# leo-stan/torch-points3d

Hardware: AMD Instinct MI355X
Metric: point-clouds/sec fwd+bwd PointNet++SSG B=32 N=16384 (higher is better)
Workload: dtype f32; 1 GPU; PointNet++ SSG (unet_3_ss) train step fwd+bwd+Adam, B=32 per GPU, N=16384, FEAT=3, 10 classes, pos~U[-1,1]^3 (BASELINE configs[1]); launch=hip-graph replay; geometry of step i+1 on a 2nd stream during step i, global_batch=32, points=16384, parallelism=dp1, whole clouds per rank, one flat gradient all-reduce (RCCL) per step

## Files before the change

include/tp3d_hip.h:

```cpp
#ifndef TP3D_HIP_H
#define TP3D_HIP_H

#include <stddef.h>
#include <stdint.h>

#ifdef __cplusplus
extern "C" {
#endif

#define TP3D_OK 0
#define TP3D_E_BADARG (-1)
#define TP3D_E_LAUNCH (-2)
#define TP3D_E_UNSORTED (-3)
#define TP3D_E_TOOBIG (-4)

#define TP3D_ABI_VERSION 39

int tp3d_abi_version(void);
const char *tp3d_strerror(int code);
int tp3d_last_hip_error(void);

#define TP3D_FPS_MAX_REG_POINTS 32768
int tp3d_fps_f32(const float *xyz, int B, int N, int npoint, float *scratch, int64_t *out_idx, void *stream);

int tp3d_fps_ragged_f32(const float *pos, const int64_t *seg_in, const int64_t *seg_out, int64_t M, int clouds,
                        int max_cloud_points, float *scratch, int64_t *out_idx, void *stream);

int tp3d_ball_query_dense_f32(const float *x, const float *y, int B, int N, int np, float radius, int nsample,
                              int sort, int64_t *idx, float *dist2, void *workspace, size_t workspace_bytes,
                              void *stream);
size_t tp3d_ball_query_workspace_bytes(int num_clouds, int64_t rows, int max_cloud_points);

int tp3d_ball_query_partial_dense_f32(const float *x, const float *y, const int64_t *batch_x,
                                      const int64_t *batch_y, int64_t M, int64_t Nq, float radius, int nsample,
                                      int sort, int64_t *idx, float *dist2, const int64_t *seg_x, int num_clouds,
                                      int max_cloud_points, void *workspace, size_t workspace_bytes, int reuse_grid,
                                      void *stream);

int tp3d_three_nn_f32(const float *unknown, const float *known, int B, int n, int m, float *dist, int64_t *idx,
                      void *stream);

int tp3d_three_interpolate_fwd_f32(const float *features, const int64_t *idx, const float *weight, int B, int C,
                                   int m, int n, float *out, void *stream);
int tp3d_three_interpolate_bwd_f32(const float *grad_out, const int64_t *idx, const float *weight, int B, int C,
                                   int m, int n, float *grad_features, void *workspace, size_t workspace_bytes,
                                   void *stream);

size_t tp3d_scatter_workspace_bytes(int B, int L, int nbins, int with_weights);

int tp3d_group_fwd_f32(const float *features, const int64_t *idx, int B, int C, int N, int np, int ns, float *out,
                       void *stream);
int tp3d_group_bwd_f32(const float *grad_out, const int64_t *idx, int B, int C, int N, int np, int ns,
                       float *grad_features, void *workspace, size_t workspace_bytes, void *stream);


int tp3d_group_concat_fwd_f32(const float *pos, const float *new_pos, const float *x_cl, const int64_t *idx, int B,
                              int N, int np, int ns, int C, int ld, float radius, int normalize, float *out,
                              void *stream);

int tp3d_rows_scatter_bwd_f32(const float *grad_rows, const int64_t *idx, const float *weight, int B, int L, int div,
                              int nbins, int ld, int col0, int C, float *grad_x_cl, void *workspace,
                              size_t workspace_bytes, void *stream);
int tp3d_rows_scatter_invert(const int64_t *idx, const float *weight, int B, int L, int div, int nbins, void *workspace,
                             size_t workspace_bytes, void *stream);
int tp3d_rows_scatter_apply_f32(const float *grad_rows, int B, int L, int div, int nbins, int ld, int col0, int C,
                                int with_weights, float *grad_x_cl, void *table, size_t table_bytes, void *stream);

size_t tp3d_bn_workspace_floats(int64_t M, int C);
int tp3d_bn_stats_f32(const float *Y, int64_t M, int C, float eps, float momentum, const float *gamma,
                      const float *beta, float *running_mean, float *running_var, int64_t *num_batches_tracked,
                      int training, float *mean, float *invstd, float *scale, float *shift, float *workspace,
                      void *stream);

int tp3d_bn_act_f32(const float *Y, const float *mean, const float *scale, const float *shift, float slope, int64_t M,
                    int C, float *out, void *stream);
int tp3d_bn_act_maxpool_f32(const float *Y, const float *mean, const float *scale, const float *shift, float slope,
                            int64_t G, int ns, int C, float *out, int *argmax, void *stream);

int tp3d_bn_act_bwd_f32(const float *dA, const int *argmax, const float *Y, const float *scale, const float *shift,
                        const float *mean, const float *invstd, float slope, int64_t M, int ns, int C, int training,
                        float *dbeta, float *dgamma, float *dY, float *workspace, void *stream);
int tp3d_bn_bwd_reduce_f32(const float *dA, const int *argmax, const float *Y, const float *scale, const float *shift,
                           const float *mean, const float *invstd, float slope, int64_t M, int ns, int C, int training,
                           float *dbeta, float *dgamma, float *c1, float *c2, float *workspace, int reverse,
                           void *stream);

int tp3d_interp_concat_fwd_f32(const float *feat_cl, const int64_t *idx, const float *weight, const float *skip_cl,
                               int B, int m, int n, int C1, int C2, int ld, float *out, void *stream);

size_t tp3d_gemm_rows_stat_floats(int64_t M, int N);
int tp3d_gemm_rows_stat_chunks(int64_t M, int N);
size_t tp3d_gemm_rows_workspace_floats(int64_t M, int N, int K);
int tp3d_gemm_rows_f32(const float *A, const float *Bt, int64_t M, int N, int K, float *C, float *stat_partial,
                       float *workspace, void *stream);
int tp3d_gemm_rows_epi_f32(const float *A, const float *Bt, int64_t M, int N, int K, const float *mean, const float *scale,
                           const float *beta, float slope, float *C, float *workspace, void *stream);
int tp3d_gemm_rows_sp_chunks(int64_t M, int N, int K, int with_act_out);
int tp3d_gemm_rows_bnact_sp_f32(const float *Y, const float *mean, const float *scale, const float *beta, float slope,
                                const float *Bt, int64_t M, int N, int K, float *C, float *stat_partial, float *act_out,
                                int reverse, void *stream);
int tp3d_gemm_rows_x3_chunks(int64_t M, int N, int K, int with_act_out);
int tp3d_gemm_rows_bnact_x3_f32(const float *Y, const float *mean, const float *scale, const float *beta, float slope,
                                const float *Bt, int64_t M, int N, int K, float *C, float *stat_partial, float *act_out,
                                int reverse, void *stream);

int tp3d_gemm_rows_bnbwd_sp_serves(int64_t M, int N, int K);
int tp3d_gemm_rows_bnbwd_sp_f32(const float *Y, const float *dA, const float *mean, const float *scale, const float *beta,
                                const float *c1, const float *c2, float slope, const float *Bt, int64_t M, int N, int K,
                                float *C, int ldc, int pad_lo, int pad_hi, float *dY_out, const int *argmax, int ns,
                                int reverse, void *stream);
int tp3d_bn_finalize_f32(float *partial, int chunks, int64_t M, int C, float eps, float momentum, const float *gamma,
                         const float *beta, float *running_mean, float *running_var, int64_t *num_batches_tracked,
                         float *mean, float *invstd, float *scale, float *shift, void *stream);

int tp3d_gemm_tn_bn_narrow_serves(int64_t M, int N, int K);
int tp3d_gemm_rows_narrow_chunks(int64_t M);
int tp3d_gemm_rows_narrow_f32(const float *A, const float *W, int64_t M, int N, int K, float *Y, float *stat_partial,
                              int reverse, void *stream);
size_t tp3d_gemm_tn_bn_narrow_workspace_floats(int64_t M, int N, int K);
int tp3d_gemm_tn_bn_narrow_f32(const float *Y, const float *dA, const float *mean_n, const float *scale_n,
                               const float *beta_n, const float *c1_n, const float *c2_n, float slope_n, const float *A,
                               int64_t M, int N, int K, float *out, float *workspace, int reverse, void *stream);

size_t tp3d_gemm_tn_workspace_floats(int64_t M, int N, int K);
int tp3d_gemm_tn_f32(const float *dY, const float *A, int64_t M, int N, int K, float *out, float *workspace,
                     void *stream);

int tp3d_gemm_tn_x3_serves(int64_t M, int N, int K);
size_t tp3d_gemm_tn_x3_workspace_floats(int64_t M, int N, int K);
int tp3d_gemm_tn_x3_f32(const float *dY, const float *A, int64_t M, int N, int K, int terms, float *out, float *workspace,
                        int reverse, void *stream);
int tp3d_gemm_tn_x3_act_f32(const float *dY, const float *Yp, const float *mean_k, const float *scale_k, const float *beta_k,
                            float slope_k, int64_t M, int N, int K, int terms, float *out, float *workspace, int reverse, void *stream);
int tp3d_gemm_tn_x3_red_chunks(int64_t M, int N, int K);
int tp3d_gemm_tn_x3_act_red_f32(const float *dY, const float *Yp, const float *mean_k, const float *scale_k,
                                const float *beta_k, const float *invstd_k, float slope_k, const float *dA_k, int training,
                                int64_t M, int N, int K, int terms, float *out, float *workspace, float *red_out,
                                float *red_workspace, int reverse, void *stream);

int tp3d_kpconv_weighted_f32(const float *query, const float *support, const int64_t *neighbors,
                             const float *features, const float *k_points, int64_t Nq, int64_t M, int Mn, int Cin,
                             int KP, float extent, int influence, int closest, float *weighted, void *stream);

size_t tp3d_kpconv_bwd_workspace_bytes(int64_t M, int64_t slots);
size_t tp3d_kpconv_grad_workspace_bytes(int64_t M, int64_t slots, int Cin);
int tp3d_kpconv_bwd_features_f32(const float *query, const float *support, const int64_t *neighbors,
                                 const float *k_points, const float *d_weighted, int64_t Nq, int64_t M, int Mn,
                                 int Cin, int KP, float extent, int influence, int closest, float *d_features,
                                 void *inverse, size_t inverse_bytes, int inverse_ready, void *workspace,
                                 size_t workspace_bytes, void *stream);

int tp3d_kpconv_deform_weighted_f32(const float *query, const float *support, const int64_t *neighbors,
                                    const float *features, const float *k_points, const float *offsets,
                                    const float *modulations, int64_t Nq, int64_t M, int Mn, int Cin, int KP, float extent,
                                    int influence, float *weighted, float *kp_min_d2, int32_t *kp_argmin, void *stream);

int tp3d_kpconv_deform_bwd_f32(const float *query, const float *support, const int64_t *neighbors, const float *features,
                               const float *k_points, const float *offsets, const float *modulations,
                               const float *d_weighted, const float *d_kp_min_d2, const int32_t *kp_argmin, int64_t Nq,
                               int64_t M, int Mn, int Cin, int KP, float extent, int influence, float *d_features,
                               float *d_offsets, float *d_modulations, void *inverse, size_t inverse_bytes,
                               int inverse_ready, void *workspace, size_t workspace_bytes, void *stream);

int tp3d_relation_rows_f32(const float *pos, const float *new_pos, const int64_t *idx, int B, int N, int np, int ns,
                           int ld, float *out, void *stream);

int tp3d_idw_weights_f32(const float *dist, int64_t rows, float *weight, void *stream);

int tp3d_voxel_bounds_f32(const float *pos, const int64_t *batch, int64_t N, float size, int32_t *bounds, void *stream);
size_t tp3d_voxel_workspace_bytes(int64_t N);
int tp3d_voxel_cluster_f32(const float *pos, const int64_t *batch, int64_t N, float size, const int32_t *bounds_host,
                           int64_t *cluster, int64_t *order, int64_t *cluster_start, int64_t *last, int64_t *meta,
                           void *workspace, size_t workspace_bytes, void *stream);
int tp3d_cluster_mean_f32(const float *x, const int64_t *order, const int64_t *cluster_start, int64_t K, int C,
                          float *out, void *stream);
int tp3d_cluster_majority_i64(const int64_t *labels, const int64_t *order, const int64_t *cluster_start, int64_t K,
                              int64_t min_label, int64_t num_classes, int64_t *out, void *stream);

size_t tp3d_knn_workspace_bytes(int num_clouds, int64_t rows, int max_cloud_points);
int tp3d_knn_partial_dense_f32(const float *x, const float *y, const int64_t *batch_y, const int64_t *seg_x,
                               int num_clouds, int max_cloud_points, int64_t M, int64_t Nq, int k, float cell,
                               int64_t *idx, float *dist2, void *workspace, size_t workspace_bytes, void *stream);
int tp3d_knn_dense_f32(const float *x, const float *y, int B, int N, int np, int k, float cell, int64_t *idx,
                       float *dist2, void *workspace, size_t workspace_bytes, void *stream);

int tp3d_knn_interpolate_fwd_f32(const float *x, const int64_t *idx, const float *dist2, const float *skip, int64_t Nq,
                                 int k, int C, int C2, int ld, float *out, float *wnorm, void *stream);

int tp3d_randla_relpos_f32(const float *q_pos, const float *s_pos, const int64_t *nbr, int64_t Nq, int k, int64_t M,
                           float *out, void *stream);

int tp3d_attn_pool_fwd_f32(const float *g, const float *f, const int64_t *nbr, int64_t Nq, int k, int C, int ldg, int ldf,
                           float *out, void *stream);
int tp3d_attn_pool_bwd_f32(const float *g, const float *f, const float *dout, const int64_t *nbr, int64_t Nq, int k, int C,
                           int ldg, int ldf, float *dg, float *df, void *stream);

int tp3d_gemm_skinny_f32(const float *A, const float *W, int64_t M, int N, int K, int lda, float *Y, void *stream);
int tp3d_gemm_skinny_bnact_f32(const float *A, const float *W, int64_t M, int N, int K, int lda, const float *mean,
                               const float *scale, const float *beta, float slope, float *out, void *stream);

int tp3d_nbr_maxpool_fwd_f32(const float *x, const int64_t *neighbors, int64_t Nq, int64_t M, int Mn, int C, float *out,
                             int32_t *argmax, void *stream);
int tp3d_nbr_maxpool_bwd_f32(const float *grad_out, const int32_t *argmax, const int64_t *neighbors, int64_t Nq,
                             int64_t M, int Mn, int C, float *d_x, void *inverse, size_t inverse_bytes,
                             int inverse_ready, void *stream);

int tp3d_pospool_padding_i64(const int64_t *neighbors, int64_t slots, int64_t M, int64_t *padding, void *stream);
int tp3d_pospool_fwd_f32(const float *query, const float *support, const int64_t *neighbors, const float *features,
                         const int64_t *padding, const float *dim_mat, int64_t Nq, int64_t M, int Mn, int C, float radius,
                         int embedding, int reduction, float *out, float *counts, void *stream);
int tp3d_pospool_bwd_f32(const float *query, const float *support, const int64_t *neighbors, const float *grad_out,
                         const float *counts, const float *dim_mat, int64_t Nq, int64_t M, int Mn, int C, float radius,
                         int embedding, int reduction, float *d_features, void *inverse, size_t inverse_bytes,
                         int inverse_ready, void *stream);


int tp3d_table_edge_start_i64(const int64_t *table, int64_t Nq, int max_num, int64_t *edge_start, void *stream);
int tp3d_table_edge_col_i64(const int64_t *table, const int64_t *edge_start, int64_t Nq, int max_num, int64_t E,
                            int64_t *col, void *stream);

int tp3d_pointconv_rows_f32(const float *x, const float *pos_s, const float *pos_q, const int64_t *edge_start,
                            const int64_t *col, int64_t Nq, int64_t M, int64_t E, int C, int ld, float *out,
                            void *stream);

int tp3d_segment_max_fwd_f32(const float *rows, const int64_t *seg, int64_t S, int64_t E, int C, int ld, float *out,
                             int64_t *argmax, void *stream);
int tp3d_segment_max_bwd_f32(const float *dout, const int64_t *argmax, const int64_t *seg, int64_t S, int64_t E, int C,
                             int ld, float *d_rows, void *stream);


int tp3d_rsconv_relation_rows_f32(const float *pos_s, const float *pos_q, const int64_t *edge_start, const int64_t *col,
                                  int64_t Nq, int64_t M, int64_t E, int ld, float *out, void *stream);

int tp3d_rsconv_msgmax_fwd_f32(const float *w, int ldw, const float *x, int ldx, const int64_t *col,
                               const int64_t *edge_start, int64_t Nq, int64_t M, int64_t E, int C, float *out,
                               int64_t *arg, void *stream);
int tp3d_rsconv_msgmax_bwd_f32(const float *dout, const int64_t *arg, const float *w, int ldw, const float *x, int ldx,
                               const int64_t *col, const int64_t *edge_start, int64_t Nq, int64_t M, int64_t E, int C,
                               float *d_w, float *g_x, void *stream);

int tp3d_gemm_tn_plan(int64_t M, int N, int K, int64_t *plan);
int tp3d_gemm_tn_x3_plan(int64_t M, int N, int K, int64_t *plan);
int tp3d_gemm_rows_plan(int64_t M, int N, int K, int64_t *plan);
int tp3d_bn_plan(int64_t M, int C, int pooled_ns, int64_t *plan);
int tp3d_scatter_plan(int B, int L, int nbins, int with_weights, int64_t *plan);

#ifdef __cplusplus
}
#endif
#endif
```

torch_points3d_amd/_lib.py:

```python
import collections
import ctypes
import os

import torch

from . import build as _build

_p = ctypes.c_void_p
_i = ctypes.c_int
_l = ctypes.c_int64
_f = ctypes.c_float

SIGNATURES = {
    "tp3d_fps_f32": [_p, _i, _i, _i, _p, _p, _p],
    "tp3d_ball_query_dense_f32": [_p, _p, _i, _i, _i, _f, _i, _i, _p, _p, _p, ctypes.c_size_t, _p],
    "tp3d_ball_query_partial_dense_f32": [_p, _p, _p, _p, _l, _l, _f, _i, _i, _p, _p, _p, _i, _i, _p, ctypes.c_size_t,
                                          _i, _p],
    "tp3d_three_nn_f32": [_p, _p, _i, _i, _i, _p, _p, _p],
    "tp3d_three_interpolate_fwd_f32": [_p, _p, _p, _i, _i, _i, _i, _p, _p],
    "tp3d_three_interpolate_bwd_f32": [_p, _p, _p, _i, _i, _i, _i, _p, _p, ctypes.c_size_t, _p],
    "tp3d_group_fwd_f32": [_p, _p, _i, _i, _i, _i, _i, _p, _p],
    "tp3d_group_bwd_f32": [_p, _p, _i, _i, _i, _i, _i, _p, _p, ctypes.c_size_t, _p],
    "tp3d_group_concat_fwd_f32": [_p, _p, _p, _p, _i, _i, _i, _i, _i, _i, _f, _i, _p, _p],
    "tp3d_rows_scatter_bwd_f32": [_p, _p, _p, _i, _i, _i, _i, _i, _i, _i, _p, _p, ctypes.c_size_t, _p],
    "tp3d_rows_scatter_invert": [_p, _p, _i, _i, _i, _i, _p, ctypes.c_size_t, _p],
    "tp3d_rows_scatter_apply_f32": [_p, _i, _i, _i, _i, _i, _i, _i, _i, _p, _p, ctypes.c_size_t, _p],
    "tp3d_bn_stats_f32": [_p, _l, _i, _f, _f, _p, _p, _p, _p, _p, _i, _p, _p, _p, _p, _p, _p],
    "tp3d_bn_act_f32": [_p, _p, _p, _p, _f, _l, _i, _p, _p],
    "tp3d_bn_act_maxpool_f32": [_p, _p, _p, _p, _f, _l, _i, _i, _p, _p, _p],
    "tp3d_bn_act_bwd_f32": [_p, _p, _p, _p, _p, _p, _p, _f, _l, _i, _i, _i, _p, _p, _p, _p, _p],
    "tp3d_interp_concat_fwd_f32": [_p, _p, _p, _p, _i, _i, _i, _i, _i, _i, _p, _p],
    "tp3d_idw_weights_f32": [_p, _l, _p, _p],
    "tp3d_gemm_tn_f32": [_p, _p, _l, _i, _i, _p, _p, _p],
    "tp3d_gemm_tn_x3_f32": [_p, _p, _l, _i, _i, _i, _p, _p, _i, _p],
    "tp3d_gemm_tn_x3_act_f32": [_p, _p, _p, _p, _p, _f, _l, _i, _i, _i, _p, _p, _i, _p],
    "tp3d_gemm_tn_x3_act_red_f32": [_p, _p, _p, _p, _p, _p, _f, _p, _i, _l, _i, _i, _i, _p, _p, _p, _p, _i, _p],
    "tp3d_gemm_rows_narrow_f32": [_p, _p, _l, _i, _i, _p, _p, _i, _p],
    "tp3d_gemm_tn_bn_narrow_f32": [_p, _p, _p, _p, _p, _p, _p, _f, _p, _l, _i, _i, _p, _p, _i, _p],
    "tp3d_bn_bwd_reduce_f32": [_p, _p, _p, _p, _p, _p, _p, _f, _l, _i, _i, _i, _p, _p, _p, _p, _p, _i, _p],
    "tp3d_gemm_rows_f32": [_p, _p, _l, _i, _i, _p, _p, _p, _p],
    "tp3d_gemm_rows_epi_f32": [_p, _p, _l, _i, _i, _p, _p, _p, _f, _p, _p, _p],
    "tp3d_gemm_rows_bnact_sp_f32": [_p, _p, _p, _p, _f, _p, _l, _i, _i, _p, _p, _p, _i, _p],
    "tp3d_gemm_rows_bnact_x3_f32": [_p, _p, _p, _p, _f, _p, _l, _i, _i, _p, _p, _p, _i, _p],
    "tp3d_gemm_rows_bnbwd_sp_f32": [_p, _p, _p, _p, _p, _p, _p, _f, _p, _l, _i, _i, _p, _i, _i, _i, _p, _p, _i, _i, _p],
    "tp3d_bn_finalize_f32": [_p, _i, _l, _i, _f, _f, _p, _p, _p, _p, _p, _p, _p, _p, _p, _p],
    "tp3d_kpconv_bwd_features_f32": [_p, _p, _p, _p, _p, _l, _l, _i, _i, _i, _f, _i, _i, _p, _p, ctypes.c_size_t, _i, _p,
                                     ctypes.c_size_t, _p],
    "tp3d_knn_partial_dense_f32": [_p, _p, _p, _p, _i, _i, _l, _l, _i, _f, _p, _p, _p, ctypes.c_size_t, _p],
    "tp3d_knn_dense_f32": [_p, _p, _i, _i, _i, _i, _f, _p, _p, _p, ctypes.c_size_t, _p],
    "tp3d_knn_interpolate_fwd_f32": [_p, _p, _p, _p, _l, _i, _i, _i, _i, _p, _p, _p],
    "tp3d_nbr_maxpool_fwd_f32": [_p, _p, _l, _l, _i, _i, _p, _p, _p],
    "tp3d_nbr_maxpool_bwd_f32": [_p, _p, _p, _l, _l, _i, _i, _p, _p, ctypes.c_size_t, _i, _p],
    "tp3d_pospool_padding_i64": [_p, _l, _l, _p, _p],
    "tp3d_pospool_fwd_f32": [_p, _p, _p, _p, _p, _p, _l, _l, _i, _i, _f, _i, _i, _p, _p, _p],
    "tp3d_pospool_bwd_f32": [_p, _p, _p, _p, _p, _p, _l, _l, _i, _i, _f, _i, _i, _p, _p, ctypes.c_size_t, _i, _p],
    "tp3d_voxel_bounds_f32": [_p, _p, _l, _f, _p, _p],
    "tp3d_voxel_cluster_f32": [_p, _p, _l, _f, _p, _p, _p, _p, _p, _p, _p, ctypes.c_size_t, _p],
    "tp3d_cluster_mean_f32": [_p, _p, _p, _l, _i, _p, _p],
    "tp3d_cluster_majority_i64": [_p, _p, _p, _l, _l, _l, _p, _p],
    "tp3d_kpconv_weighted_f32": [_p, _p, _p, _p, _p, _l, _l, _i, _i, _i, _f, _i, _i, _p, _p],
    "tp3d_kpconv_deform_weighted_f32": [_p, _p, _p, _p, _p, _p, _p, _l, _l, _i, _i, _i, _f, _i, _p, _p, _p, _p],
    "tp3d_kpconv_deform_bwd_f32": [_p, _p, _p, _p, _p, _p, _p, _p, _p, _p, _l, _l, _i, _i, _i, _f, _i, _p, _p, _p, _p,
                                   ctypes.c_size_t, _i, _p, ctypes.c_size_t, _p],
    "tp3d_gemm_skinny_f32": [_p, _p, _l, _i, _i, _i, _p, _p],
    "tp3d_gemm_skinny_bnact_f32": [_p, _p, _l, _i, _i, _i, _p, _p, _p, _f, _p, _p],
    "tp3d_randla_relpos_f32": [_p, _p, _p, _l, _i, _l, _p, _p],
    "tp3d_attn_pool_fwd_f32": [_p, _p, _p, _l, _i, _i, _i, _i, _p, _p],
    "tp3d_attn_pool_bwd_f32": [_p, _p, _p, _p, _l, _i, _i, _i, _i, _p, _p, _p],
    "tp3d_relation_rows_f32": [_p, _p, _p, _i, _i, _i, _i, _i, _p, _p],
    "tp3d_fps_ragged_f32": [_p, _p, _p, _l, _i, _i, _p, _p, _p],
    "tp3d_table_edge_start_i64": [_p, _l, _i, _p, _p],
    "tp3d_table_edge_col_i64": [_p, _p, _l, _i, _l, _p, _p],
    "tp3d_pointconv_rows_f32": [_p, _p, _p, _p, _p, _l, _l, _l, _i, _i, _p, _p],
    "tp3d_segment_max_fwd_f32": [_p, _p, _l, _l, _i, _i, _p, _p, _p],
    "tp3d_segment_max_bwd_f32": [_p, _p, _p, _l, _l, _i, _i, _p, _p],
    "tp3d_rsconv_relation_rows_f32": [_p, _p, _p, _p, _l, _l, _l, _i, _p, _p],
    "tp3d_rsconv_msgmax_fwd_f32": [_p, _i, _p, _i, _p, _p, _l, _l, _l, _i, _p, _p, _p],
    "tp3d_rsconv_msgmax_bwd_f32": [_p, _p, _p, _i, _p, _i, _p, _p, _l, _l, _l, _i, _p, _p, _p],
    "tp3d_gemm_tn_plan": [_l, _i, _i, _p],
    "tp3d_gemm_tn_x3_plan": [_l, _i, _i, _p],
    "tp3d_gemm_rows_plan": [_l, _i, _i, _p],
    "tp3d_bn_plan": [_l, _i, _i, _p],
    "tp3d_scatter_plan": [_i, _i, _i, _i, _p],
}
_z = ctypes.c_size_t
MISC = {
    "tp3d_abi_version": (_i, []),
    "tp3d_strerror": (ctypes.c_char_p, [_i]),
    "tp3d_last_hip_error": (_i, []),
    "tp3d_scatter_workspace_bytes": (_z, [_i, _i, _i, _i]),
    "tp3d_bn_workspace_floats": (_z, [_l, _i]),
    "tp3d_gemm_tn_workspace_floats": (_z, [_l, _i, _i]),
    "tp3d_gemm_tn_x3_workspace_floats": (_z, [_l, _i, _i]),
    "tp3d_gemm_tn_x3_serves": (_i, [_l, _i, _i]),
    "tp3d_gemm_tn_x3_red_chunks": (_i, [_l, _i, _i]),
    "tp3d_kpconv_bwd_workspace_bytes": (_z, [_l, _l]),
    "tp3d_gemm_rows_stat_floats": (_z, [_l, _i]),
    "tp3d_gemm_rows_stat_chunks": (_i, [_l, _i]),
    "tp3d_gemm_rows_narrow_chunks": (_i, [_l]),
    "tp3d_gemm_tn_bn_narrow_serves": (_i, [_l, _i, _i]),
    "tp3d_gemm_tn_bn_narrow_workspace_floats": (_z, [_l, _i, _i]),
    "tp3d_gemm_rows_bnbwd_sp_serves": (_i, [_l, _i, _i]),
    "tp3d_gemm_rows_x3_chunks": (_i, [_l, _i, _i, _i]),
    "tp3d_gemm_rows_sp_chunks": (_i, [_l, _i, _i, _i]),
    "tp3d_gemm_rows_workspace_floats": (_z, [_l, _i, _i]),
    "tp3d_kpconv_grad_workspace_bytes": (_z, [_l, _l, _i]),
    "tp3d_knn_workspace_bytes": (_z, [_i, _l, _i]),
    "tp3d_voxel_workspace_bytes": (_z, [_l]),
    "tp3d_ball_query_workspace_bytes": (_z, [_i, _l, _i]),
}
ABI_VERSION = 39

_handle = None


class Tp3dError(RuntimeError):
    pass


def library_path():
    return _build.LIB_PATH


def load():
    global _handle
    if _handle is not None:
        return _handle
    path = _build.LIB_PATH
    if not os.path.exists(path):
        _build.build_library()
    if not os.path.exists(path):
        raise Tp3dError("libtp3d_hip.so is missing at %s and could not be built" % path)
    h = ctypes.CDLL(path)
    for name, argtypes in SIGNATURES.items():
        fn = getattr(h, name)
        fn.argtypes = argtypes
        fn.restype = _i
    for name, (restype, argtypes) in MISC.items():
        fn = getattr(h, name)
        fn.restype = restype
        fn.argtypes = argtypes
    if h.tp3d_abi_version() != ABI_VERSION:
        raise Tp3dError("libtp3d_hip.so ABI %d != binding ABI %d" % (h.tp3d_abi_version(), ABI_VERSION))
    _handle = h
    return h


class KernelTimer(object):

    def __init__(self):
        self.records = []

    def summary(self):
        out = {}
        for tag, a, b in self.records:
            n, t = out.get(tag, (0, 0.0))
            out[tag] = (n + 1, t + a.elapsed_time(b))
        return out


_timer = None


def set_timer(timer):
    global _timer
    prev, _timer = _timer, timer
    return prev


_fn_cache = {}
_post_call_hook = None


def set_post_call_hook(hook):
    global _post_call_hook
    prev, _post_call_hook = _post_call_hook, hook
    return prev


def call(name, *args):
    fn = _fn_cache.get(name)
    if fn is None:
        fn = _fn_cache[name] = getattr(load(), name)
    if _timer is not None:
        a = torch.cuda.Event(enable_timing=True)
        b = torch.cuda.Event(enable_timing=True)
        torch.cuda.current_stream().synchronize()
        a.record()
        rc = fn(*args)
        b.record()
        _timer.records.append(((name, tuple(v for v in args if type(v) is int and v < (1 << 40))), a, b))
    else:
        rc = fn(*args)
    if rc != 0:
        h = load()
        raise Tp3dError("%s failed: %s (code %d, hipError %d)" % (
            name, h.tp3d_strerror(rc).decode(), rc, h.tp3d_last_hip_error()))
    if _post_call_hook is not None:
        _post_call_hook(name, args)


class on_device(object):

    __slots__ = ("idx", "prev")

    def __init__(self, dev):
        self.idx = dev.index if dev.index is not None else torch.cuda.current_device()
        self.prev = -1

    def __enter__(self):
        cur = torch.cuda.current_device()
        if cur != self.idx:
            self.prev = cur
            torch.cuda.set_device(self.idx)

    def __exit__(self, *exc):
        if self.prev >= 0:
            torch.cuda.set_device(self.prev)
        return False


_ws_cache = {}
_ws_retired = []


def workspace(tag, nbytes, device):
    key = (device.index, _raw_stream(device), tag)
    capturing = device.type == "cuda" and torch.cuda.is_current_stream_capturing()
    slot = _ws_cache.get(key)
    if slot is None or slot[0].numel() < nbytes:
        if slot is not None and slot[1]:
            _ws_retired.append(slot[0])
        slot = _ws_cache[key] = [torch.empty(max(int(nbytes), 256), dtype=torch.uint8, device=device), False]
    if capturing:
        slot[1] = True
    return slot[0]


def _raw_stream(device):
    idx = device.index if device.index is not None else torch.cuda.current_device()
    return torch._C._cuda_getCurrentRawStream(idx)


def scatter_workspace(B, L, nbins, with_weights, device):
    nbytes = load().tp3d_scatter_workspace_bytes(B, L, nbins, int(with_weights))
    return workspace("scatter", nbytes, device), nbytes


GRID_MIN_POINTS = 2048


def ball_query_workspace(num_clouds, rows, max_cloud_points, device):
    if max_cloud_points < GRID_MIN_POINTS:
        return None, 0
    nbytes = load().tp3d_ball_query_workspace_bytes(num_clouds, rows, max_cloud_points)
    if nbytes == 0:
        return None, 0
    return workspace("grid", nbytes, device), nbytes


_inverse_cache = collections.OrderedDict()
INVERSE_CACHE_ENTRIES = 48


def _evict_inverse():
    if len(_inverse_cache) < INVERSE_CACHE_ENTRIES:
        return
    for key in list(_inverse_cache):
        if len(_inverse_cache) < INVERSE_CACHE_ENTRIES:
            break
        if not _inverse_cache[key][5]:
            del _inverse_cache[key]


def neighbour_inverse(nbr, M, device):
    key = (nbr.data_ptr(), nbr._version, tuple(nbr.shape), int(M), device.index)
    hit = _inverse_cache.get(key)
    cur = _raw_stream(device)
    capturing = torch.cuda.is_current_stream_capturing()
    if hit is not None and hit[3] is not None:
        _inverse_cache.move_to_end(key)
        if capturing:
            hit[5] = True
        elif hit[4] != cur:
            torch.cuda.current_stream(device).wait_event(hit[3])
        return hit[1], hit[2], 1, None
    nbytes = load().tp3d_kpconv_bwd_workspace_bytes(int(M), nbr.numel())
    if capturing:
        return workspace("nbr_inverse", nbytes, device), nbytes, 0, None
    buf = torch.empty(max(int(nbytes), 256), dtype=torch.uint8, device=device)
    _evict_inverse()
    _inverse_cache[key] = [nbr, buf, nbytes, None, cur, False]
    return buf, nbytes, 0, key


def inverse_built(token, device):
    if token is None:
        return
    entry = _inverse_cache.get(token)
    if entry is not None:
        ev = torch.cuda.Event()
        ev.record(torch.cuda.current_stream(device))
        entry[3] = ev


def bn_workspace(M, C, device):
    n = load().tp3d_bn_workspace_floats(M, C)
    return workspace("bn", 4 * n, device)


def gemm_tn_workspace(M, N, K, device, x3=False):
    h = load()
    n = h.tp3d_gemm_tn_x3_workspace_floats(M, N, K) if x3 else h.tp3d_gemm_tn_workspace_floats(M, N, K)
    return workspace("gemm_tn", 4 * n, device)


def ptr(t):
    return None if t is None else t.data_ptr()


def stream_ptr(device):
    return _raw_stream(device)
```

torch_points3d_amd/csrc/gemm_tn.hip:

```cpp
#include <type_traits>

#include "tp3d_common.h"

namespace tp3d {

typedef float f32x16 __attribute__((ext_vector_type(16)));

constexpr int TN_BLOCK = 256;
constexpr int TN_BR_MAX = 64;

template <int WM, int WN, bool VECY, bool VECA, int GN = 2>
__global__ __launch_bounds__(TN_BLOCK) void gemm_tn_partial_kernel(const float *__restrict__ dY,
                                                                    const float *__restrict__ A, int64_t M, int N,
                                                                    int K, int64_t rows_per_split, int tiles_k,
                                                                    float *__restrict__ partial )
{
    constexpr int GK = 4 / GN;
    constexpr int TN = GN * WM * 32, TK = GK * WN * 32;
    constexpr int TN_BR = (WM * WN) % 3 == 0 ? 16 : 64 / (WM * WN);
    constexpr int LDN = TN + 4, LDK = TK + 4;
    __shared__ __attribute__((aligned(16))) float sY[TN_BR * LDN];
    __shared__ __attribute__((aligned(16))) float sA[TN_BR * LDK];

    const int tile = blockIdx.x;
    const int n0 = (tile / tiles_k) * TN, k0 = (tile % tiles_k) * TK;
    const int split = blockIdx.y;
    const int64_t r_begin = (int64_t)split * rows_per_split;
    const int64_t r_end = min(r_begin + rows_per_split, M);
    const int tid = threadIdx.x, lane = tid & 63, wave = tid >> 6;
    const int wr = wave / GK, wc = wave % GK;
    const int l31 = lane & 31, lh = lane >> 5;
    f32x16 acc[WM][WN];
#pragma unroll
    for (int i = 0; i < WM; ++i)
#pragma unroll
        for (int j = 0; j < WN; ++j)
#pragma unroll
            for (int e = 0; e < 16; ++e) acc[i][j][e] = 0.0f;


    auto load4 = [&](const float *base, int64_t r, int c, int ld, auto aligned_tag) __attribute__((always_inline)) -> float4 {
        constexpr bool aligned = decltype(aligned_tag)::value;
        float4 v = make_float4(0.f, 0.f, 0.f, 0.f);
        if (r < r_end) {
            const float *src = base + r * ld + c;
            if (aligned) {
                if (c < ld) v = *reinterpret_cast<const float4 *>(src);
            } else {
                if (c + 0 < ld) v.x = src[0];
                if (c + 1 < ld) v.y = src[1];
                if (c + 2 < ld) v.z = src[2];
                if (c + 3 < ld) v.w = src[3];
            }
        }
        return v;
    };

    constexpr int PY = TN_BR * (TN / 4) / TN_BLOCK, PA = TN_BR * (TK / 4) / TN_BLOCK;
    static_assert(PY >= 1 && PA >= 1 && PY * TN_BLOCK == TN_BR * (TN / 4) && PA * TN_BLOCK == TN_BR * (TK / 4),
                  "staged tile must be a whole number of float4 slots per thread");
    float4 ry[PY], ra[PA];
    auto fetch = [&](int64_t r0) __attribute__((always_inline)) {
#pragma unroll
        for (int i = 0; i < PY; ++i) {
            const int e = tid + i * TN_BLOCK;
            const int64_t r = r0 + e / (TN / 4);
            const int c = n0 + (e % (TN / 4)) * 4;
            ry[i] = load4(dY, r, c, N, std::integral_constant<bool, VECY>());
        }
#pragma unroll
        for (int i = 0; i < PA; ++i) {
            const int e = tid + i * TN_BLOCK;
            ra[i] = load4(A, r0 + e / (TK / 4), k0 + (e % (TK / 4)) * 4, K, std::integral_constant<bool, VECA>());
        }
    };
    if (r_begin < r_end) fetch(r_begin);
    for (int64_t r0 = r_begin; r0 < r_end; r0 += TN_BR) {
#pragma unroll
        for (int i = 0; i < PY; ++i) {
            const int e = tid + i * TN_BLOCK;
            *reinterpret_cast<float4 *>(&sY[(e / (TN / 4)) * LDN + (e % (TN / 4)) * 4]) = ry[i];
        }
#pragma unroll
        for (int i = 0; i < PA; ++i) {
            const int e = tid + i * TN_BLOCK;
            *reinterpret_cast<float4 *>(&sA[(e / (TK / 4)) * LDK + (e % (TK / 4)) * 4]) = ra[i];
        }
        __syncthreads();
        if (r0 + TN_BR < r_end) fetch(r0 + TN_BR);
#pragma unroll
        for (int rr = 0; rr < TN_BR; rr += 2) {
            float a[WM], b[WN];
#pragma unroll
            for (int i = 0; i < WM; ++i) a[i] = sY[(rr + lh) * LDN + (wr * WM + i) * 32 + l31];
#pragma unroll
            for (int j = 0; j < WN; ++j) b[j] = sA[(rr + lh) * LDK + (wc * WN + j) * 32 + l31];
#pragma unroll
            for (int i = 0; i < WM; ++i)
#pragma unroll
                for (int j = 0; j < WN; ++j) acc[i][j] = __builtin_amdgcn_mfma_f32_32x32x2f32(a[i], b[j], acc[i][j], 0, 0, 0);
        }
        __syncthreads();
    }

    float *out = partial + (size_t)split * N * K;
#pragma unroll
    for (int i = 0; i < WM; ++i)
#pragma unroll
        for (int j = 0; j < WN; ++j)
#pragma unroll
            for (int e = 0; e < 16; ++e) {
                const int n = n0 + (wr * WM + i) * 32 + (e & 3) + 8 * (e >> 2) + 4 * lh;
                const int k = k0 + (wc * WN + j) * 32 + l31;
                if (n < N && k < K) out[(size_t)n * K + k] = acc[i][j][e];
            }
}

constexpr int RD_E = 64, RD_S = 16;
__global__ __launch_bounds__(RD_E *RD_S) void gemm_tn_reduce_kernel(const float *__restrict__ partial, int S,
                                                                     int64_t NK, float *__restrict__ out)
{
    __shared__ float sm[RD_S][RD_E];
    const int tx = threadIdx.x % RD_E, ty = threadIdx.x / RD_E;
    const int64_t e = (int64_t)blockIdx.x * RD_E + tx;
    float acc = 0.0f;
    if (e < NK)
        for (int s = ty; s < S; s += RD_S) acc += partial[(size_t)s * NK + e];
    sm[ty][tx] = acc;
    __syncthreads();
    if (ty == 0 && e < NK) {
        float t = 0.0f;
#pragma unroll
        for (int k = 0; k < RD_S; ++k) t += sm[k][tx];
        out[e] = t;
    }
}

int tn_reduce_splits(const float *partial, int splits, int64_t NK, float *out, hipStream_t s)
{
    hipLaunchKernelGGL(gemm_tn_reduce_kernel, dim3((unsigned)((NK + RD_E - 1) / RD_E)), dim3(RD_E * RD_S), 0, s, partial, splits,
                       NK, out);
    return check_launch();
}

struct TnPlan {
    int wm, wn, gn, tn, tk, tiles_n, tiles_k, splits;
    int64_t rows_per_split;
};

static TnPlan plan_tn(int64_t M, int N, int K)
{
    TnPlan p;
    p.wm = N > 64 ? 2 : 1;
    if (K <= 64) p.wn = 1;
    else if (K <= 128) p.wn = 2;
    else if (K <= 192) p.wn = 3;
    else p.wn = ((K + 191) / 192) * 192 < ((K + 127) / 128) * 128 ? 3 : 2;
    p.gn = 2;
    if (N <= 32 && K >= 128) {
        p.gn = 1;
        p.wm = 1;
        p.wn = 1;
    }
    p.tn = 32 * p.gn * p.wm;
    p.tk = 32 * (4 / p.gn) * p.wn;
    p.tiles_n = (N + p.tn - 1) / p.tn;
    p.tiles_k = (K + p.tk - 1) / p.tk;
    const int tiles = p.tiles_n * p.tiles_k;
    int64_t want = (1024 + tiles - 1) / tiles;
    const int min_rows = 256;
    int64_t max_by_rows = (M + min_rows - 1) / min_rows;
    int64_t s = want < max_by_rows ? want : max_by_rows;
    if (s < 1) s = 1;
    if (s > 512) s = 512;
    p.rows_per_split = ((M + s - 1) / s + TN_BR_MAX - 1) / TN_BR_MAX * TN_BR_MAX;
    p.splits = (int)((M + p.rows_per_split - 1) / p.rows_per_split);
    return p;
}

static int launch_tn(const float *dY, const float *A, int64_t M, int N, int K, float *out, float *workspace, hipStream_t s)
{
    const TnPlan p = plan_tn(M, N, K);
    if (p.splits > 65535) return TP3D_E_TOOBIG;
    dim3 grid(p.tiles_n * p.tiles_k, p.splits);
    const bool vy = (N & 3) == 0, va = (K & 3) == 0;
#define TP3D_TN_LAUNCH(WM_, WN_, VY_, VA_)                                                                          \
    hipLaunchKernelGGL((gemm_tn_partial_kernel<WM_, WN_, VY_, VA_>), grid, dim3(TN_BLOCK), 0, s, dY, A, M, N, K,        \
                       p.rows_per_split, p.tiles_k, workspace)
#define TP3D_TN_ALIGN(WM_, WN_)                                                                                     \
    do {                                                                                                            \
        if (vy && va) TP3D_TN_LAUNCH(WM_, WN_, true, true);                                                         \
        else if (vy) TP3D_TN_LAUNCH(WM_, WN_, true, false);                                                         \
        else if (va) TP3D_TN_LAUNCH(WM_, WN_, false, true);                                                         \
        else TP3D_TN_LAUNCH(WM_, WN_, false, false);                                                                \
    } while (0)
    if (p.gn == 1) {
        if (vy && va) hipLaunchKernelGGL((gemm_tn_partial_kernel<1, 1, true, true, 1>), grid, dim3(TN_BLOCK), 0, s, dY, A, M, N, K,
                                         p.rows_per_split, p.tiles_k, workspace);
        else if (va) hipLaunchKernelGGL((gemm_tn_partial_kernel<1, 1, false, true, 1>), grid, dim3(TN_BLOCK), 0, s, dY, A, M, N, K,
                                        p.rows_per_split, p.tiles_k, workspace);
        else if (vy) hipLaunchKernelGGL((gemm_tn_partial_kernel<1, 1, true, false, 1>), grid, dim3(TN_BLOCK), 0, s, dY, A, M, N, K,
                                        p.rows_per_split, p.tiles_k, workspace);
        else hipLaunchKernelGGL((gemm_tn_partial_kernel<1, 1, false, false, 1>), grid, dim3(TN_BLOCK), 0, s, dY, A, M, N, K,
                                p.rows_per_split, p.tiles_k, workspace);
    } else if (p.wm == 2 && p.wn == 3) TP3D_TN_ALIGN(2, 3);
    else if (p.wn == 3) TP3D_TN_ALIGN(1, 3);
    else if (p.wm == 2 && p.wn == 2) TP3D_TN_ALIGN(2, 2);
    else if (p.wm == 2) TP3D_TN_ALIGN(2, 1);
    else if (p.wn == 2) TP3D_TN_ALIGN(1, 2);
    else TP3D_TN_ALIGN(1, 1);
#undef TP3D_TN_ALIGN
#undef TP3D_TN_LAUNCH
    if (int rc = check_launch()) return rc;
    return tn_reduce_splits(workspace, p.splits, (int64_t)N * K, out, s);
}

}

using namespace tp3d;

TP3D_EXPORT size_t tp3d_gemm_tn_workspace_floats(int64_t M, int N, int K)
{
    if (M <= 0 || N <= 0 || K <= 0) return 0;
    const TnPlan p = plan_tn(M, N, K);
    return (size_t)p.splits * (size_t)N * (size_t)K;
}

TP3D_EXPORT int tp3d_gemm_tn_plan(int64_t M, int N, int K, int64_t *plan)
{
    if (M <= 0 || N <= 0 || K <= 0 || !plan) return TP3D_E_BADARG;
    const TnPlan p = plan_tn(M, N, K);
    plan[0] = p.splits;
    plan[1] = p.rows_per_split;
    plan[2] = p.tn;
    plan[3] = p.tk;
    plan[4] = (int64_t)p.tiles_n * p.tiles_k;
    plan[5] = (p.wm * p.wn) % 3 == 0 ? 16 : 64 / (p.wm * p.wn);
    plan[6] = (int64_t)p.splits * N * K;
    plan[7] = (int64_t)(p.splits - 1) * p.rows_per_split;
    return TP3D_OK;
}

TP3D_EXPORT int tp3d_gemm_tn_f32(const float *dY, const float *A, int64_t M, int N, int K, float *out,
                                 float *workspace, void *stream)
{
    if (M < 0 || N <= 0 || K <= 0 || !out) return TP3D_E_BADARG;
    hipStream_t s = (hipStream_t)stream;
    if (M == 0) return zero_async(out, (size_t)N * K * sizeof(float), s);
    if (!dY || !A || !workspace) return TP3D_E_BADARG;
    return launch_tn(dY, A, M, N, K, out, workspace, s);
}
```

torch_points3d_amd/csrc/gemm_tn_x3.hip:

```cpp
#include "tp3d_common.h"
#include "x3_split.h"

namespace tp3d {

typedef float f32x16 __attribute__((ext_vector_type(16)));
typedef __bf16 bf16x8 __attribute__((ext_vector_type(8)));
typedef short s16x4 __attribute__((ext_vector_type(4)));
typedef short s16x8 __attribute__((ext_vector_type(8)));

constexpr int X3_BLOCK = 512;

__host__ __device__ constexpr int x3_pitch(int cols) { return cols % 64 == 0 ? cols + 32 : cols; }

__device__ __forceinline__ bf16x8 x3_frag(const unsigned short *plane, int pitch, int row0, int col0, int lane)
{
    const int grp = lane >> 4, q = (lane & 15) >> 2, p = lane & 3;
    const unsigned short *a = plane + (row0 + 8 * (grp >> 1) + q) * pitch + col0 + 16 * (grp & 1) + 4 * p;
    typedef s16x4 __attribute__((address_space(3))) *lds_ptr;
    const s16x4 lo = __builtin_amdgcn_ds_read_tr16_b64_v4i16((lds_ptr)(a));
    const s16x4 hi = __builtin_amdgcn_ds_read_tr16_b64_v4i16((lds_ptr)(a + 4 * pitch));
    const s16x8 both = {lo[0], lo[1], lo[2], lo[3], hi[0], hi[1], hi[2], hi[3]};
    return __builtin_bit_cast(bf16x8, both);
}

struct X3Prologue {
    const float *mean, *scale, *beta;
    float slope;
    int reverse;
    const float *dA, *invstd;
    float *red_partial;
};

template <int WM, int WN, bool STRIP, int BR, int TERMS, bool RED = false>
__global__ __launch_bounds__(X3_BLOCK) void gemm_tn_x3_kernel(const float *__restrict__ dY, const float *__restrict__ A,
                                                              int64_t M, int N, int K, int64_t rows_per_split,
                                                              int tiles_k, float *__restrict__ partial ,
                                                              X3Prologue pro)
{
    static_assert(!STRIP || WM == 2, "the strip is one block per wave of a 128-row tile");
    static_assert(!(RED && STRIP), "the reductions ride on the plain tiles (one tile column: every workgroup sees all K columns)");
    constexpr int TN = 64 * WM, TK = 64 * WN, TKS = TK + (STRIP ? 32 : 0);
    constexpr int PN = x3_pitch(TN), PK = x3_pitch(TKS);
    constexpr int PLANE_N = BR * PN, PLANE_K = BR * PK;
    constexpr int BUF = 3 * PLANE_N + 3 * PLANE_K;
    extern __shared__ __attribute__((aligned(16))) unsigned short smem[];
    __shared__ __attribute__((aligned(16))) float sK[RED ? 4 : 3][TKS];

    const int tid = threadIdx.x, lane = tid & 63, wave = tid >> 6;
    const int tile = blockIdx.x;
    const int n0 = (tile / tiles_k) * TN, k0 = (tile % tiles_k) * TK;
    const bool prologue = pro.mean != nullptr;
    if (prologue) {
        for (int c = tid; c < TKS; c += X3_BLOCK) {
            const bool in = k0 + c < K;
            sK[0][c] = in ? pro.mean[k0 + c] : 0.0f;
            sK[1][c] = in ? pro.scale[k0 + c] : 0.0f;
            sK[2][c] = in ? pro.beta[k0 + c] : 0.0f;
            if (RED) sK[3][c] = in ? pro.invstd[k0 + c] : 0.0f;
        }
        __syncthreads();
    }
    const int64_t r_end = M;
    const int64_t blocks = (M + BR - 1) / BR;
    const int S = gridDim.y;
    const int steps = (int)(((int64_t)blocks - blockIdx.y + S - 1) / S);
    (void)rows_per_split;

    if (__builtin_amdgcn_readfirstlane(tid) >= 256) {
        __builtin_amdgcn_s_setprio(3);
        const int lt = tid - 256;
        constexpr int SY = BR * (TN / 4) / 256, SA = BR * (TK / 4) / 256, SS = STRIP ? BR * 8 / 256 : 0;
        static_assert(SY >= 1 && SA >= 1 && SY * 256 == BR * (TN / 4) && SA * 256 == BR * (TK / 4), "whole float4 slots per thread");
        static_assert(!STRIP || SS * 256 == BR * 8, "whole strip slots per thread");
        float4 ry0[SY], ra0[SA], rs0[STRIP ? SS : 1], ry1[SY], ra1[SA], rs1[STRIP ? SS : 1], ry2[SY], ra2[SA], rs2[STRIP ? SS : 1];
        float4 rd0[RED ? SA : 1], rd1[RED ? SA : 1], rd2[RED ? SA : 1];
        float red1[4] = {0.f, 0.f, 0.f, 0.f}, red2[4] = {0.f, 0.f, 0.f, 0.f};
        const int red_tiles = (int)gridDim.x;
        auto mine = [&](int t) __attribute__((always_inline)) -> bool { return RED && (t % red_tiles) == tile; };
        const float4 zero = make_float4(0.f, 0.f, 0.f, 0.f);
        const bool cols_full = n0 + TN <= N && k0 + TK <= K;
        unsigned oy[SY], oa[SA], os[STRIP ? SS : 1];
#pragma unroll
        for (int i = 0; i < SY; ++i) oy[i] = (unsigned)((((lt + i * 256) / (TN / 4)) * N + n0 + ((lt + i * 256) % (TN / 4)) * 4) * 4);
#pragma unroll
        for (int i = 0; i < SA; ++i) oa[i] = (unsigned)((((lt + i * 256) / (TK / 4)) * K + k0 + ((lt + i * 256) % (TK / 4)) * 4) * 4);
        if (STRIP) {
#pragma unroll
            for (int i = 0; i < SS; ++i) os[i] = (unsigned)((((lt + i * 256) / 8) * K + k0 + TK + ((lt + i * 256) % 8) * 4) * 4);
        }
        auto fetch = [&](int t, float4 *ry, float4 *ra, float4 *rs, float4 *rd) __attribute__((always_inline)) {
            const int64_t r0 = ((int64_t)(pro.reverse ? steps - 1 - t : t) * S + blockIdx.y) * BR;
            const char *by_ = reinterpret_cast<const char *>(dY) + r0 * N * 4;
            const char *ba_ = reinterpret_cast<const char *>(A) + r0 * K * 4;
            if (r0 + BR <= M && cols_full) {
#pragma unroll
                for (int i = 0; i < SY; ++i) ry[i] = *reinterpret_cast<const float4 *>(by_ + oy[i]);
#pragma unroll
                for (int i = 0; i < SA; ++i) ra[i] = *reinterpret_cast<const float4 *>(ba_ + oa[i]);
                if (mine(t)) {
                    const char *bd_ = reinterpret_cast<const char *>(pro.dA) + r0 * K * 4;
#pragma unroll
                    for (int i = 0; i < SA; ++i) rd[i] = *reinterpret_cast<const float4 *>(bd_ + oa[i]);
                }
                if (STRIP) {
#pragma unroll
                    for (int i = 0; i < SS; ++i) {
                        rs[i] = zero;
                        if (k0 + TK + ((lt + i * 256) % 8) * 4 < K) rs[i] = *reinterpret_cast<const float4 *>(ba_ + os[i]);
                    }
                }
                return;
            }
#pragma unroll
            for (int i = 0; i < SY; ++i) {
                const int e = lt + i * 256;
                const int64_t r = r0 + e / (TN / 4);
                const int c = n0 + (e % (TN / 4)) * 4;
                ry[i] = zero;
                if (r < r_end && c < N) ry[i] = *reinterpret_cast<const float4 *>(dY + r * N + c);
            }
#pragma unroll
            for (int i = 0; i < SA; ++i) {
                const int e = lt + i * 256;
                const int64_t r = r0 + e / (TK / 4);
                const int c = k0 + (e % (TK / 4)) * 4;
                ra[i] = zero;
                if (r < r_end && c < K) ra[i] = *reinterpret_cast<const float4 *>(A + r * K + c);
                if (mine(t)) {
                    rd[i] = zero;
                    if (r < r_end && c < K) rd[i] = *reinterpret_cast<const float4 *>(pro.dA + r * K + c);
                }
            }
            if (STRIP) {
#pragma unroll
                for (int i = 0; i < SS; ++i) {
                    const int e = lt + i * 256;
                    const int64_t r = r0 + e / 8;
                    const int c = k0 + TK + (e % 8) * 4;
                    rs[i] = zero;
                    if (r < r_end && c < K) rs[i] = *reinterpret_cast<const float4 *>(A + r * K + c);
                }
            }
        };
        auto put = [&](unsigned short *plane0, int plane_len, int pitch, int row, int col, float4 v) __attribute__((always_inline)) {
            uint2 h, m, l;
            x3_split(v, h, m, l);
            unsigned short *dst = plane0 + row * pitch + col;
            *reinterpret_cast<uint2 *>(dst) = h;
            *reinterpret_cast<uint2 *>(dst + plane_len) = m;
            *reinterpret_cast<uint2 *>(dst + 2 * plane_len) = l;
        };
        auto act4 = [&](float4 v, int col) __attribute__((always_inline)) -> float4 {
            const float4 mu = *reinterpret_cast<const float4 *>(&sK[0][col]);
            const float4 sc = *reinterpret_cast<const float4 *>(&sK[1][col]);
            const float4 be = *reinterpret_cast<const float4 *>(&sK[2][col]);
            const float z0 = (v.x - mu.x) * sc.x + be.x, z1 = (v.y - mu.y) * sc.y + be.y;
            const float z2 = (v.z - mu.z) * sc.z + be.z, z3 = (v.w - mu.w) * sc.w + be.w;
            return make_float4(z0 > 0.0f ? z0 : z0 * pro.slope, z1 > 0.0f ? z1 : z1 * pro.slope, z2 > 0.0f ? z2 : z2 * pro.slope,
                               z3 > 0.0f ? z3 : z3 * pro.slope);
        };
        auto store = [&](int t, const float4 *ry, const float4 *ra, const float4 *rs, const float4 *rd) __attribute__((always_inline)) {
            unsigned short *by = smem + (t & 1) * BUF, *ba = by + 3 * PLANE_N;
            if (mine(t)) {
                const int col = ((lt % (TK / 4))) * 4;
                const float4 mu = *reinterpret_cast<const float4 *>(&sK[0][col]), sc = *reinterpret_cast<const float4 *>(&sK[1][col]);
                const float4 be = *reinterpret_cast<const float4 *>(&sK[2][col]), is = *reinterpret_cast<const float4 *>(&sK[3][col]);
#pragma unroll
                for (int i = 0; i < SA; ++i) {
                    const float y[4] = {ra[i].x, ra[i].y, ra[i].z, ra[i].w}, d[4] = {rd[i].x, rd[i].y, rd[i].z, rd[i].w};
                    const float m4[4] = {mu.x, mu.y, mu.z, mu.w}, s4[4] = {sc.x, sc.y, sc.z, sc.w};
                    const float b4[4] = {be.x, be.y, be.z, be.w}, i4[4] = {is.x, is.y, is.z, is.w};
#pragma unroll
                    for (int c = 0; c < 4; ++c) {
                        const float yc = y[c] - m4[c];
                        const float dz = d[c] * (yc * s4[c] + b4[c] > 0.0f ? 1.0f : pro.slope);
                        red1[c] += dz;
                        red2[c] += dz * (yc * i4[c]);
                    }
                }
            }
#pragma unroll
            for (int i = 0; i < SY; ++i) {
                const int e = lt + i * 256;
                put(by, PLANE_N, PN, e / (TN / 4), (e % (TN / 4)) * 4, ry[i]);
            }
#pragma unroll
            for (int i = 0; i < SA; ++i) {
                const int e = lt + i * 256;
                const int col = (e % (TK / 4)) * 4;
                put(ba, PLANE_K, PK, e / (TK / 4), col, prologue ? act4(ra[i], col) : ra[i]);
            }
            if (STRIP) {
#pragma unroll
                for (int i = 0; i < SS; ++i) {
                    const int e = lt + i * 256;
                    const int col = TK + (e % 8) * 4;
                    put(ba, PLANE_K, PK, e / 8, col, prologue ? act4(rs[i], col) : rs[i]);
                }
            }
        };
        if (steps > 0) fetch(0, ry0, ra0, rs0, rd0);
        if (steps > 1) fetch(1, ry1, ra1, rs1, rd1);
        if (steps > 2) fetch(2, ry2, ra2, rs2, rd2);
        auto iter = [&](int t, float4 *ry, float4 *ra, float4 *rs, float4 *rd) __attribute__((always_inline)) {
            store(t, ry, ra, rs, rd);
            if (t + 3 < steps) fetch(t + 3, ry, ra, rs, rd);
            __syncthreads();
        };
        for (int t = 0; t < steps; t += 3) {
            iter(t, ry0, ra0, rs0, rd0);
            if (t + 1 < steps) iter(t + 1, ry1, ra1, rs1, rd1);
            if (t + 2 < steps) iter(t + 2, ry2, ra2, rs2, rd2);
        }
        if (RED) {
            float *scr = reinterpret_cast<float *>(smem + (steps & 1) * BUF);
#pragma unroll
            for (int c = 0; c < 4; ++c) {
                scr[lt * 8 + c] = red1[c];
                scr[lt * 8 + 4 + c] = red2[c];
            }
            __syncthreads();
            constexpr int CG = TK / 4, PER = 256 / CG;
            if (lt < CG) {
                float a1[4] = {0.f, 0.f, 0.f, 0.f}, a2[4] = {0.f, 0.f, 0.f, 0.f};
                for (int x = 0; x < PER; ++x)
#pragma unroll
                    for (int c = 0; c < 4; ++c) {
                        a1[c] += scr[(lt + x * CG) * 8 + c];
                        a2[c] += scr[(lt + x * CG) * 8 + 4 + c];
                    }
                float *pr = pro.red_partial + ((size_t)blockIdx.y * gridDim.x + blockIdx.x) * 2 * K;
#pragma unroll
                for (int c = 0; c < 4; ++c) {
                    const int k = k0 + lt * 4 + c;
                    if (k < K) {
                        pr[k] = a1[c];
                        pr[K + k] = a2[c];
                    }
                }
            }
        }
        return;
    }

    const int wr = wave >> 1, wc = wave & 1;
    const int l31 = lane & 31, lh = lane >> 5;
    f32x16 acc[WM][WN], low[WM][WN], accs, lows;
#pragma unroll
    for (int i = 0; i < WM; ++i)
#pragma unroll
        for (int j = 0; j < WN; ++j)
#pragma unroll
            for (int e = 0; e < 16; ++e) acc[i][j][e] = low[i][j][e] = 0.0f;
#pragma unroll
    for (int e = 0; e < 16; ++e) accs[e] = lows[e] = 0.0f;

    for (int t = 0; t < steps; ++t) {
        __syncthreads();
        const unsigned short *by = smem + (t & 1) * BUF, *ba = by + 3 * PLANE_N;
#pragma unroll
        for (int s = 0; s < BR; s += 16) {
            bf16x8 a[WM][3], b[WN][3], bs[3], as[3];
#pragma unroll
            for (int p = 0; p < 3; ++p) {
#pragma unroll
                for (int i = 0; i < WM; ++i) a[i][p] = x3_frag(by + p * PLANE_N, PN, s, (wr * WM + i) * 32, lane);
#pragma unroll
                for (int j = 0; j < WN; ++j) b[j][p] = x3_frag(ba + p * PLANE_K, PK, s, (wc * WN + j) * 32, lane);
                if (STRIP) {
                    bs[p] = x3_frag(ba + p * PLANE_K, PK, s, TK, lane);
                    as[p] = x3_frag(by + p * PLANE_N, PN, s, (wr * WM + wc) * 32, lane);
                }
            }
            constexpr int PA_[9] = {2, 2, 1, 2, 0, 1, 1, 0, 0};
            constexpr int PB_[9] = {2, 1, 2, 0, 2, 1, 0, 1, 0};
#pragma unroll
            for (int u = 9 - TERMS; u < 8; ++u) {
#pragma unroll
                for (int i = 0; i < WM; ++i)
#pragma unroll
                    for (int j = 0; j < WN; ++j)
                        low[i][j] = __builtin_amdgcn_mfma_f32_32x32x16_bf16(a[i][PA_[u]], b[j][PB_[u]], low[i][j], 0, 0, 0);
                if (STRIP) lows = __builtin_amdgcn_mfma_f32_32x32x16_bf16(as[PA_[u]], bs[PB_[u]], lows, 0, 0, 0);
            }
#pragma unroll
            for (int i = 0; i < WM; ++i)
#pragma unroll
                for (int j = 0; j < WN; ++j)
                    acc[i][j] = __builtin_amdgcn_mfma_f32_32x32x16_bf16(a[i][0], b[j][0], acc[i][j], 0, 0, 0);
            if (STRIP) accs = __builtin_amdgcn_mfma_f32_32x32x16_bf16(as[0], bs[0], accs, 0, 0, 0);
        }
    }
    if (RED) __syncthreads();

    float *out = partial + (size_t)blockIdx.y * N * K;
#pragma unroll
    for (int i = 0; i < WM; ++i)
#pragma unroll
        for (int j = 0; j < WN; ++j)
#pragma unroll
            for (int e = 0; e < 16; ++e) {
                const int n = n0 + (wr * WM + i) * 32 + (e & 3) + 8 * (e >> 2) + 4 * lh;
                const int k = k0 + (wc * WN + j) * 32 + l31;
                if (n < N && k < K) out[(size_t)n * K + k] = acc[i][j][e] + low[i][j][e];
            }
    if (STRIP) {
#pragma unroll
        for (int e = 0; e < 16; ++e) {
            const int n = n0 + (wr * WM + wc) * 32 + (e & 3) + 8 * (e >> 2) + 4 * lh;
            const int k = k0 + TK + l31;
            if (n < N && k < K) out[(size_t)n * K + k] = accs[e] + lows[e];
        }
    }
}

struct X3Plan {
    int wm, wn, strip, br, tiles_n, tiles_k, splits, lds_bytes;
    int64_t rows_per_split;
};

static X3Plan x3_plan(int64_t M, int N, int K);

static bool x3_serves(int64_t M, int N, int K)
{
    if (!(M >= 131072 && N >= 64 && K >= 64 && (N & 3) == 0 && (K & 3) == 0 &&
          M * (int64_t)(N > K ? N : K) < ((int64_t)1 << 30)))
        return false;
    const X3Plan p = x3_plan(M, N, K);
    const int tiles = p.tiles_n * p.tiles_k;
    const int64_t padded = (int64_t)p.tiles_n * 64 * p.wm * ((int64_t)p.tiles_k * 64 * p.wn + (p.strip ? 32 : 0));
    return tiles <= 2 && (int64_t)N * K * 5 >= padded * 4;
}

static X3Plan x3_plan(int64_t M, int N, int K)
{
    X3Plan p;
    p.wm = N <= 64 ? 1 : 2;
    const int rem128 = K % 128, rem64 = K % 64;
    p.strip = 0;
    if (K <= 64) p.wn = 1;
    else if (K > 128 && K <= 160 && p.wm == 2) p.wn = 2, p.strip = 1;
    else if (K <= 128) p.wn = 2;
    else p.wn = 2;
    (void)rem128;
    (void)rem64;
    p.br = (p.wm == 1 && p.wn == 1) ? 64 : 32;
    const int tn = 64 * p.wm, tk = 64 * p.wn;
    p.tiles_n = (N + tn - 1) / tn;
    p.tiles_k = p.strip ? 1 : (K + tk - 1) / tk;
    const int tiles = p.tiles_n * p.tiles_k;
    int64_t s = (256 + tiles - 1) / tiles;
    const int64_t max_by_rows = (M + 1023) / 1024;
    if (s > max_by_rows) s = max_by_rows;
    if (s < 1) s = 1;
    p.rows_per_split = ((M + s - 1) / s + p.br - 1) / p.br * p.br;
    p.splits = (int)((M + p.rows_per_split - 1) / p.rows_per_split);
    const int pn = x3_pitch(tn), pk = x3_pitch(tk + (p.strip ? 32 : 0));
    p.lds_bytes = 2 * 3 * p.br * (pn + pk) * 2;
    return p;
}

template <int WM, int WN, bool STRIP, int BR, int TERMS, bool RED = false>
static void x3_launch(const X3Plan &p, const float *dY, const float *A, int64_t M, int N, int K, float *ws, X3Prologue pro,
                      hipStream_t s)
{
    static bool allowed[64] = {};
    auto kern = gemm_tn_x3_kernel<WM, WN, STRIP, BR, TERMS, RED>;
    allow_large_dynamic_lds(reinterpret_cast<const void *>(kern), p.lds_bytes, allowed);
    hipLaunchKernelGGL(kern, dim3(p.tiles_n * p.tiles_k, p.splits), dim3(X3_BLOCK), p.lds_bytes, s, dY, A, M, N, K,
                       p.rows_per_split, p.tiles_k, ws, pro);
}

}

using namespace tp3d;

TP3D_EXPORT int tp3d_gemm_tn_x3_serves(int64_t M, int N, int K) { return x3_serves(M, N, K) ? 1 : 0; }

TP3D_EXPORT size_t tp3d_gemm_tn_x3_workspace_floats(int64_t M, int N, int K)
{
    if (!x3_serves(M, N, K)) return 0;
    return (size_t)x3_plan(M, N, K).splits * (size_t)N * (size_t)K;
}

TP3D_EXPORT int tp3d_gemm_tn_x3_plan(int64_t M, int N, int K, int64_t *plan)
{
    if (!plan || !x3_serves(M, N, K)) return TP3D_E_BADARG;
    const X3Plan p = x3_plan(M, N, K);
    plan[0] = p.splits;
    plan[1] = p.rows_per_split;
    plan[2] = 64 * p.wm;
    plan[3] = 64 * p.wn + (p.strip ? 32 : 0);
    plan[4] = (int64_t)p.tiles_n * p.tiles_k;
    plan[5] = p.br;
    plan[6] = (int64_t)p.splits * N * K;
    plan[7] = p.lds_bytes;
    return TP3D_OK;
}

static int x3_run(const float *dY, const float *A, int64_t M, int N, int K, int terms, float *out, float *workspace,
                  X3Prologue pro, void *stream)
{
    if (!x3_serves(M, N, K) || !dY || !A || !out || !workspace || (terms != 9 && terms != 6 && terms != 1)) return TP3D_E_BADARG;
    hipStream_t s = (hipStream_t)stream;
    const X3Plan p = x3_plan(M, N, K);
    if (p.splits > 65535) return TP3D_E_TOOBIG;
#define TP3D_X3(WM_, WN_, ST_, BR_)                                                                 \
    do {                                                                                            \
        if (terms == 9) x3_launch<WM_, WN_, ST_, BR_, 9>(p, dY, A, M, N, K, workspace, pro, s);     \
        else if (terms == 6) x3_launch<WM_, WN_, ST_, BR_, 6>(p, dY, A, M, N, K, workspace, pro, s); \
        else x3_launch<WM_, WN_, ST_, BR_, 1>(p, dY, A, M, N, K, workspace, pro, s);                \
    } while (0)
    if (p.wm == 2 && p.wn == 2 && p.strip) TP3D_X3(2, 2, true, 32);
    else if (p.wm == 2 && p.wn == 2) TP3D_X3(2, 2, false, 32);
    else if (p.wm == 2) TP3D_X3(2, 1, false, 32);
    else if (p.wn == 2) TP3D_X3(1, 2, false, 32);
    else TP3D_X3(1, 1, false, 64);
#undef TP3D_X3
    if (int rc = check_launch()) return rc;
    return tn_reduce_splits(workspace, p.splits, (int64_t)N * K, out, s);
}

TP3D_EXPORT int tp3d_gemm_tn_x3_f32(const float *dY, const float *A, int64_t M, int N, int K, int terms, float *out,
                                    float *workspace, int reverse, void *stream)
{
    const X3Prologue none = {nullptr, nullptr, nullptr, 1.0f, reverse, nullptr, nullptr, nullptr};
    return x3_run(dY, A, M, N, K, terms, out, workspace, none, stream);
}

TP3D_EXPORT int tp3d_gemm_tn_x3_act_f32(const float *dY, const float *Yp, const float *mean_k, const float *scale_k,
                                        const float *beta_k, float slope_k, int64_t M, int N, int K, int terms, float *out,
                                        float *workspace, int reverse, void *stream)
{
    if (!mean_k || !scale_k || !beta_k) return TP3D_E_BADARG;
    const X3Prologue pro = {mean_k, scale_k, beta_k, slope_k, reverse, nullptr, nullptr, nullptr};
    return x3_run(dY, Yp, M, N, K, terms, out, workspace, pro, stream);
}

static bool x3_red_serves(int64_t M, int N, int K)
{
    if (!x3_serves(M, N, K)) return false;
    const X3Plan p = x3_plan(M, N, K);
    return p.tiles_k == 1 && !p.strip && (p.wm == 2 || p.wn == 1);
}

TP3D_EXPORT int tp3d_gemm_tn_x3_red_chunks(int64_t M, int N, int K)
{
    if (!x3_red_serves(M, N, K)) return 0;
    const X3Plan p = x3_plan(M, N, K);
    return p.tiles_n * p.splits;
}

TP3D_EXPORT int tp3d_gemm_tn_x3_act_red_f32(const float *dY, const float *Yp, const float *mean_k, const float *scale_k,
                                            const float *beta_k, const float *invstd_k, float slope_k, const float *dA_k,
                                            int training, int64_t M, int N, int K, int terms, float *out, float *workspace,
                                            float *red_out, float *red_workspace, int reverse, void *stream)
{
    if (!mean_k || !scale_k || !beta_k || !invstd_k || !dA_k || !red_out || !red_workspace || terms != 6) return TP3D_E_BADARG;
    if (!x3_red_serves(M, N, K) || !dY || !Yp || !out || !workspace) return TP3D_E_BADARG;
    hipStream_t s = (hipStream_t)stream;
    const X3Plan p = x3_plan(M, N, K);
    if (p.splits > 65535) return TP3D_E_TOOBIG;
    const X3Prologue pro = {mean_k, scale_k, beta_k, slope_k, reverse, dA_k, invstd_k, red_workspace};
    if (p.wm == 2 && p.wn == 2) x3_launch<2, 2, false, 32, 6, true>(p, dY, Yp, M, N, K, workspace, pro, s);
    else if (p.wm == 2) x3_launch<2, 1, false, 32, 6, true>(p, dY, Yp, M, N, K, workspace, pro, s);
    else x3_launch<1, 1, false, 64, 6, true>(p, dY, Yp, M, N, K, workspace, pro, s);
    if (int rc = check_launch()) return rc;
    if (int rc = tn_reduce_splits(workspace, p.splits, (int64_t)N * K, out, s)) return rc;
    return bn_bwd_finalize_launch(red_workspace, p.tiles_n * p.splits, K, red_out, red_out + K, invstd_k, M, training,
                                  red_out + 2 * (size_t)K, red_out + 3 * (size_t)K, s);
}
```

torch_points3d_amd/csrc/rows.hip:

```cpp
#include <type_traits>

#include "tp3d_common.h"

namespace tp3d {

constexpr int RW_BLOCK = 256;

__global__ __launch_bounds__(RW_BLOCK) void group_concat_fwd_kernel(const float *__restrict__ pos,
                                                                     const float *__restrict__ new_pos,
                                                                     const float *__restrict__ x_cl,
                                                                     const int64_t *__restrict__ idx, int N, int np,
                                                                     int ns, int C, int ld, float radius,
                                                                     int normalize, int64_t total,
                                                                     float *__restrict__ out)
{
    const int Cw = C + 3;
    for (int64_t e = (int64_t)blockIdx.x * RW_BLOCK + threadIdx.x; e < total; e += (int64_t)gridDim.x * RW_BLOCK) {
        const int64_t row = e / ld;
        const int c = (int)(e - row * ld);
        if (c >= Cw) {
            out[e] = 0.0f;
            continue;
        }
        const int64_t bj = row / ns;
        const int b = (int)(bj / np);
        const int k = min(max((int)idx[row], 0), N - 1);
        float v;
        if (c < 3) {
            v = pos[((size_t)b * N + k) * 3 + c] - new_pos[bj * 3 + c];
            if (normalize) v = v / radius;
        } else {
            v = x_cl[((size_t)b * N + k) * C + (c - 3)];
        }
        out[e] = v;
    }
}

struct __attribute__((packed, aligned(4))) f4u {
    float v[4];
};
__global__ __launch_bounds__(RW_BLOCK) void group_concat_fwd4_kernel(const float *__restrict__ pos,
                                                                      const float *__restrict__ new_pos,
                                                                      const float *__restrict__ x_cl,
                                                                      const int64_t *__restrict__ idx, int N, int np,
                                                                      int ns, int C, int ld, float radius,
                                                                      int normalize, int64_t total4,
                                                                      float *__restrict__ out)
{
    const int Cw = C + 3, q = ld >> 2;
    for (int64_t e4 = (int64_t)blockIdx.x * RW_BLOCK + threadIdx.x; e4 < total4; e4 += (int64_t)gridDim.x * RW_BLOCK) {
        const int64_t row = e4 / q;
        const int c = (int)(e4 - row * q) * 4;
        const int64_t bj = row / ns;
        const int b = (int)(bj / np);
        const int k = min(max((int)idx[row], 0), N - 1);
        float t[4];
        if (c == 0) {
#pragma unroll
            for (int j = 0; j < 3; ++j) {
                float v = pos[((size_t)b * N + k) * 3 + j] - new_pos[bj * 3 + j];
                if (normalize) v = v / radius;
                t[j] = v;
            }
            t[3] = C > 0 ? x_cl[((size_t)b * N + k) * C] : 0.0f;
        } else if (c + 3 < Cw) {
            const f4u f = *reinterpret_cast<const f4u *>(x_cl + ((size_t)b * N + k) * C + (c - 3));
#pragma unroll
            for (int j = 0; j < 4; ++j) t[j] = f.v[j];
        } else {
#pragma unroll
            for (int j = 0; j < 4; ++j) t[j] = (c + j < Cw) ? x_cl[((size_t)b * N + k) * C + (c + j - 3)] : 0.0f;
        }
        *reinterpret_cast<float4 *>(out + e4 * 4) = make_float4(t[0], t[1], t[2], t[3]);
    }
}

__device__ __forceinline__ float rl_f(float x, int lane)
{
    return __builtin_bit_cast(float, __builtin_amdgcn_readlane(__builtin_bit_cast(int, x), lane));
}

template <int NP>
__device__ __forceinline__ void gather_run(const float *__restrict__ base, const int *__restrict__ od,
                                           const float *__restrict__ ws, int lo, int hi, int ld, const int (&c)[NP],
                                           float (&acc)[NP], int lane)
{
    for (int j0 = lo; j0 < hi; j0 += 64) {
        const int cnt = min(64, hi - j0);
        const int my_r = (lane < cnt) ? od[j0 + lane] : 0;
        const float my_w = (ws && lane < cnt) ? ws[j0 + lane] : 1.0f;
        int t = 0;
        auto take = [&](auto utag) {
            constexpr int U = decltype(utag)::value;
            int r[U];
            float wv[U], v[U][NP];
#pragma unroll
            for (int u = 0; u < U; ++u) {
                r[u] = __builtin_amdgcn_readlane(my_r, t + u);
                wv[u] = ws ? rl_f(my_w, t + u) : 1.0f;
            }
#pragma unroll
            for (int u = 0; u < U; ++u)
#pragma unroll
                for (int p = 0; p < NP; ++p) v[u][p] = base[(size_t)r[u] * ld + c[p]];
#pragma unroll
            for (int u = 0; u < U; ++u)
#pragma unroll
                for (int p = 0; p < NP; ++p) acc[p] = acc[p] + (ws ? wv[u] * v[u][p] : v[u][p]);
            t += U;
        };
        while (t + 8 <= cnt) take(std::integral_constant<int, 8>());
        if (t + 4 <= cnt) take(std::integral_constant<int, 4>());
        const int rem = cnt - t;
        if (rem > 0) {
            const int r0 = __builtin_amdgcn_readlane(my_r, t);
            const int r1 = __builtin_amdgcn_readlane(my_r, min(t + 1, cnt - 1));
            const int r2 = __builtin_amdgcn_readlane(my_r, min(t + 2, cnt - 1));
            const float w0 = ws ? rl_f(my_w, t) : 1.0f, w1 = ws ? rl_f(my_w, min(t + 1, cnt - 1)) : 1.0f,
                        w2 = ws ? rl_f(my_w, min(t + 2, cnt - 1)) : 1.0f;
#pragma unroll
            for (int p = 0; p < NP; ++p) {
                const float v0 = base[(size_t)r0 * ld + c[p]], v1 = base[(size_t)r1 * ld + c[p]],
                            v2 = base[(size_t)r2 * ld + c[p]];
                acc[p] = acc[p] + (ws ? w0 * v0 : v0);
                if (rem > 1) acc[p] = acc[p] + (ws ? w1 * v1 : v1);
                if (rem > 2) acc[p] = acc[p] + (ws ? w2 * v2 : v2);
            }
        }
    }
}

constexpr int HUB_MIN = 128;
constexpr int HUB_BLOCK = 1024;

template <int NP>
__global__ __launch_bounds__(RW_BLOCK) void rows_gather_sum_kernel(const float *__restrict__ grad_rows,
                                                                    const int *__restrict__ start,
                                                                    const int *__restrict__ order,
                                                                    const float *__restrict__ wsorted, int nbins,
                                                                    int L, int rows_per_cloud, int ld, int col0,
                                                                    int C, float *__restrict__ out, int flat, int hub_min)
{
    const int lane = threadIdx.x & 63;
    const int64_t dest = (int64_t)blockIdx.x * (RW_BLOCK / 64) + (threadIdx.x >> 6);
    const int b = blockIdx.y;
    if (dest >= nbins) return;
    const int *st = flat ? start + (size_t)b * nbins : start + (size_t)b * (nbins + 1);
    const int *od = flat ? order : order + (size_t)b * L;
    const float *ws = wsorted ? (flat ? wsorted : wsorted + (size_t)b * L) : nullptr;
    const int lo = st[dest], hi = st[dest + 1];
    if (hub_min > 0 && hi - lo > hub_min) return;
    const float *base = grad_rows + (flat ? (size_t)0 : (size_t)b * rows_per_cloud * ld) + col0;
    for (int c0 = 0; c0 < C; c0 += 64 * NP) {
        int c[NP];
        float acc[NP];
#pragma unroll
        for (int p = 0; p < NP; ++p) {
            c[p] = min(c0 + p * 64 + lane, C - 1);
            acc[p] = 0.0f;
        }
        gather_run<NP>(base, od, ws, lo, hi, ld, c, acc, lane);
#pragma unroll
        for (int p = 0; p < NP; ++p)
            if (c0 + p * 64 + lane < C) out[((size_t)b * nbins + dest) * C + c0 + p * 64 + lane] = acc[p];
    }
}

__global__ __launch_bounds__(256) void find_hubs_kernel(const int *__restrict__ start, int B, int nbins, int flat,
                                                        int *__restrict__ hubs)
{
    const int64_t e = (int64_t)blockIdx.x * 256 + threadIdx.x;
    if (e >= (int64_t)B * nbins) return;
    const int b = (int)(e / nbins), k = (int)(e - (int64_t)b * nbins);
    const int *st = flat ? start + (size_t)b * nbins : start + (size_t)b * (nbins + 1);
    if (st[k + 1] - st[k] > HUB_MIN) hubs[1 + atomicAdd(&hubs[0], 1)] = (int)e;
}

template <int NP>
__global__ __launch_bounds__(HUB_BLOCK) void rows_gather_hub_kernel(const float *__restrict__ grad_rows,
                                                                     const int *__restrict__ start,
                                                                     const int *__restrict__ order,
                                                                     const float *__restrict__ wsorted,
                                                                     const int *__restrict__ hubs, int nbins, int L,
                                                                     int rows_per_cloud, int ld, int col0, int C,
                                                                     float *__restrict__ out, int flat)
{
    constexpr int NW = HUB_BLOCK / 64;
    __shared__ float part[NW][64 * NP];
    const int lane = threadIdx.x & 63, wave = threadIdx.x >> 6;
    const int count = hubs[0];
    for (int h = blockIdx.x; h < count; h += gridDim.x) {
        const int e = hubs[1 + h];
        const int b = e / nbins, dest = e - b * nbins;
        const int *st = flat ? start + (size_t)b * nbins : start + (size_t)b * (nbins + 1);
        const int *od = flat ? order : order + (size_t)b * L;
        const float *ws = wsorted ? (flat ? wsorted : wsorted + (size_t)b * L) : nullptr;
        const int lo = st[dest], hi = st[dest + 1];
        const int per = ((hi - lo + NW - 1) / NW + 7) & ~7;
        const int wlo = min(lo + wave * per, hi), whi = min(wlo + per, hi);
        const float *base = grad_rows + (flat ? (size_t)0 : (size_t)b * rows_per_cloud * ld) + col0;
        for (int c0 = 0; c0 < C; c0 += 64 * NP) {
            int c[NP];
            float acc[NP];
#pragma unroll
            for (int p = 0; p < NP; ++p) {
                c[p] = min(c0 + p * 64 + lane, C - 1);
                acc[p] = 0.0f;
            }
            gather_run<NP>(base, od, ws, wlo, whi, ld, c, acc, lane);
#pragma unroll
            for (int p = 0; p < NP; ++p) part[wave][p * 64 + lane] = acc[p];
            __syncthreads();
            for (int x = threadIdx.x; x < 64 * NP; x += HUB_BLOCK) {
                float sum = part[0][x];
                for (int w = 1; w < NW; ++w) sum = sum + part[w][x];
                const int cc = c0 + x;
                if (cc < C) out[((size_t)b * nbins + dest) * C + cc] = sum;
            }
            __syncthreads();
        }
    }
}

constexpr int ST_ROWS = 256;
constexpr int ST_ROWS_SMALL = 32;
constexpr int64_t ST_SMALL_BELOW = 131072;
static inline int stat_rows(int64_t R) { return R >= ST_SMALL_BELOW ? ST_ROWS : ST_ROWS_SMALL; }

struct StatTile {
    int colthreads, rowlanes, gridx;
};
static inline StatTile stat_tile(int C, int V)
{
    int cols = (C + V - 1) / V;
    int ct = 1;
    while (ct < cols && ct < 64) ct <<= 1;
    StatTile t;
    t.colthreads = ct;
    t.rowlanes = RW_BLOCK / ct;
    t.gridx = (cols + ct - 1) / ct;
    return t;
}

template <int V, int MODE>
__global__ __launch_bounds__(RW_BLOCK) void colreduce_partial_kernel(
    const float *__restrict__ Y, const float *__restrict__ dA, const float *__restrict__ scale,
    const float *__restrict__ shift, const float *__restrict__ mean, const float *__restrict__ invstd, float slope,
    int64_t M, int C, int colthreads, int chunk_rows, float *__restrict__ partial , int reverse = 0)
{
    __shared__ float s1[RW_BLOCK * V], s2[RW_BLOCK * V];
    const int ct = threadIdx.x % colthreads, rl = threadIdx.x / colthreads;
    const int rowlanes = RW_BLOCK / colthreads;
    const int c = (blockIdx.x * colthreads + ct) * V;
    const int chunk = (MODE == 1 && reverse) ? (int)(gridDim.y - 1 - blockIdx.y) : (int)blockIdx.y;
    const int64_t r0 = (int64_t)chunk * chunk_rows;
    const int64_t r1 = min(r0 + chunk_rows, M);
    float a[V], q[V], sc[V], sh[V], mu[V], is[V];
#pragma unroll
    for (int v = 0; v < V; ++v) {
        a[v] = 0.0f;
        q[v] = 0.0f;
        if (MODE == 0) mu[v] = (c + v < C && r0 < M) ? Y[r0 * C + c + v] : 0.0f;
        if (MODE == 1 && c + v < C) {
            sc[v] = scale[c + v];
            sh[v] = shift[c + v];
            mu[v] = mean[c + v];
            is[v] = invstd[c + v];
        }
    }
    if (c < C) {
        constexpr int U = 4;
        for (int64_t r = r0 + rl; r < r1; r += (int64_t)rowlanes * U) {
            float y[U][V], d[U][V];
#pragma unroll
            for (int u = 0; u < U; ++u) {
                const int64_t rr = r + (int64_t)u * rowlanes;
                if (rr < r1) {
                    if (V == 4) {
                        *reinterpret_cast<float4 *>(y[u]) = *reinterpret_cast<const float4 *>(Y + rr * C + c);
                        if (MODE == 1) *reinterpret_cast<float4 *>(d[u]) = *reinterpret_cast<const float4 *>(dA + rr * C + c);
                    } else {
                        y[u][0] = Y[rr * C + c];
                        if (MODE == 1) d[u][0] = dA[rr * C + c];
                    }
                } else {
#pragma unroll
                    for (int v = 0; v < V; ++v) {
                        y[u][v] = mu[v];
                        d[u][v] = 0.0f;
                    }
                }
            }
#pragma unroll
            for (int u = 0; u < U; ++u)
#pragma unroll
                for (int v = 0; v < V; ++v) {
                    if (MODE == 0) {
                        const float dd = y[u][v] - mu[v];
                        a[v] += dd;
                        q[v] += dd * dd;
                    } else {
                        const float z = (y[u][v] - mu[v]) * sc[v] + sh[v];
                        const float dz = d[u][v] * (z > 0.0f ? 1.0f : slope);
                        a[v] += dz;
                        q[v] += dz * ((y[u][v] - mu[v]) * is[v]);
                    }
                }
        }
    }
#pragma unroll
    for (int v = 0; v < V; ++v) {
        s1[(rl * colthreads + ct) * V + v] = a[v];
        s2[(rl * colthreads + ct) * V + v] = q[v];
    }
    __syncthreads();
    if (rl == 0 && c < C) {
#pragma unroll
        for (int v = 0; v < V; ++v) {
            if (c + v < C) {
                float sa = 0.0f, sq = 0.0f;
                for (int k = 0; k < rowlanes; ++k) {
                    sa += s1[(k * colthreads + ct) * V + v];
                    sq += s2[(k * colthreads + ct) * V + v];
                }
                if (MODE == 0) {
                    partial[((size_t)chunk * 4 + 0) * C + c + v] = sa;
                    partial[((size_t)chunk * 4 + 1) * C + c + v] = sq;
                    partial[((size_t)chunk * 4 + 2) * C + c + v] = mu[v];
                    partial[((size_t)chunk * 4 + 3) * C + c + v] = (float)(r1 - r0);
                } else {
                    partial[((size_t)chunk * 2 + 0) * C + c + v] = sa;
                    partial[((size_t)chunk * 2 + 1) * C + c + v] = sq;
                }
            }
        }
    }
}

__device__ __forceinline__ void sum_partials(const float *__restrict__ partial, int chunks, int C, int c, double &a,
                                             double &q)
{
    __shared__ double r1[RW_BLOCK], r2[RW_BLOCK];
    double la = 0.0, lq = 0.0;
    for (int k = threadIdx.x; k < chunks; k += RW_BLOCK) {
        la += (double)partial[((size_t)k * 2 + 0) * C + c];
        lq += (double)partial[((size_t)k * 2 + 1) * C + c];
    }
    r1[threadIdx.x] = la;
    r2[threadIdx.x] = lq;
    __syncthreads();
    for (int off = RW_BLOCK / 2; off > 0; off >>= 1) {
        if ((int)threadIdx.x < off) {
            r1[threadIdx.x] += r1[threadIdx.x + off];
            r2[threadIdx.x] += r2[threadIdx.x + off];
        }
        __syncthreads();
    }
    a = r1[0];
    q = r2[0];
}

constexpr int BM_COLS = 32, BM_LANES = RW_BLOCK / BM_COLS;
__global__ __launch_bounds__(RW_BLOCK) void bn_merge_slices_kernel(float *__restrict__ partial, int chunks, int per, int C)
{
    __shared__ double rn[BM_LANES][BM_COLS], rm[BM_LANES][BM_COLS], r2[BM_LANES][BM_COLS];
    const int cx = threadIdx.x % BM_COLS, ry = threadIdx.x / BM_COLS;
    const int c = blockIdx.x * BM_COLS + cx;
    const int k0 = blockIdx.y * per, k1 = min(k0 + per, chunks);
    double n = 0.0, mu = 0.0, m2 = 0.0;
    if (c < C)
        for (int k = k0 + ry; k < k1; k += BM_LANES) {
            const float *pk = partial + (size_t)k * 4 * C + c;
            const double nb = (double)pk[(size_t)3 * C];
            if (nb > 0.0) {
                const double S = (double)pk[0], Q = (double)pk[(size_t)C];
                const double mb = (double)pk[(size_t)2 * C] + S / nb, m2b = Q - S * S / nb;
                const double tot = n + nb, dm = mb - mu;
                mu += dm * (nb / tot);
                m2 += m2b + dm * dm * (n * nb / tot);
                n = tot;
            }
        }
    rn[ry][cx] = n;
    rm[ry][cx] = mu;
    r2[ry][cx] = m2;
    __syncthreads();
    for (int off = BM_LANES / 2; off > 0; off >>= 1) {
        if (ry < off) {
            const double na = rn[ry][cx], nb = rn[ry + off][cx];
            const double tot = na + nb;
            if (nb > 0.0) {
                const double dm = rm[ry + off][cx] - rm[ry][cx];
                rm[ry][cx] += dm * (nb / tot);
                r2[ry][cx] += r2[ry + off][cx] + dm * dm * (na * nb / tot);
                rn[ry][cx] = tot;
            }
        }
        __syncthreads();
    }
    if (ry == 0 && c < C && k0 < k1) {
        float *pk = partial + (size_t)k0 * 4 * C + c;
        const double nn = rn[0][cx];
        const float kf = (float)rm[0][cx];
        const double sres = nn * (rm[0][cx] - (double)kf);
        pk[0] = (float)sres;
        pk[(size_t)C] = (float)(r2[0][cx] + (nn > 0.0 ? sres * sres / nn : 0.0));
        pk[(size_t)2 * C] = kf;
        pk[(size_t)3 * C] = (float)nn;
    }
}

__global__ __launch_bounds__(RW_BLOCK) void bn_finalize_kernel(
    const float *__restrict__ partial, int chunks, int chunk_stride, int64_t M, int C, float eps, float momentum,
    const float *__restrict__ gamma, const float *__restrict__ beta, float *__restrict__ running_mean,
    float *__restrict__ running_var, int64_t *__restrict__ batches, int training, float *__restrict__ mean_out,
    float *__restrict__ invstd_out, float *__restrict__ scale_out, float *__restrict__ shift_out)
{
    __shared__ double rn[RW_BLOCK], rm[RW_BLOCK], r2[RW_BLOCK];
    const int c = blockIdx.x;
    float mean, var;
    if (training) {
        if (batches && c == 0 && threadIdx.x == 0) *batches += 1;
        double n = 0.0, mu = 0.0, m2 = 0.0;
        for (int k = threadIdx.x; k < chunks; k += RW_BLOCK) {
            const float *pk = partial + (size_t)k * chunk_stride * 4 * C + c;
            const double nb = (double)pk[(size_t)3 * C];
            if (nb > 0.0) {
                const double S = (double)pk[0], Q = (double)pk[(size_t)C];
                const double mb = (double)pk[(size_t)2 * C] + S / nb, m2b = Q - S * S / nb;
                const double tot = n + nb, dm = mb - mu;
                mu += dm * (nb / tot);
                m2 += m2b + dm * dm * (n * nb / tot);
                n = tot;
            }
        }
        rn[threadIdx.x] = n;
        rm[threadIdx.x] = mu;
        r2[threadIdx.x] = m2;
        __syncthreads();
        for (int off = RW_BLOCK / 2; off > 0; off >>= 1) {
            if ((int)threadIdx.x < off) {
                const double na = rn[threadIdx.x], nb = rn[threadIdx.x + off];
                const double tot = na + nb;
                if (nb > 0.0) {
                    const double dm = rm[threadIdx.x + off] - rm[threadIdx.x];
                    rm[threadIdx.x] += dm * (nb / tot);
                    r2[threadIdx.x] += r2[threadIdx.x + off] + dm * dm * (na * nb / tot);
                    rn[threadIdx.x] = tot;
                }
            }
            __syncthreads();
        }
        double v = r2[0] / (double)M;
        if (v < 0.0) v = 0.0;
        mean = (float)rm[0];
        var = (float)v;
        if (running_mean && threadIdx.x == 0) {
            const double unb = M > 1 ? v * ((double)M / (double)(M - 1)) : v;
            running_mean[c] = (1.0f - momentum) * running_mean[c] + momentum * mean;
            running_var[c] = (1.0f - momentum) * running_var[c] + momentum * (float)unb;
        }
    } else {
        mean = running_mean[c];
        var = running_var[c];
    }
    if (threadIdx.x != 0) return;
    const float invstd = 1.0f / sqrtf(var + eps);
    const float g = gamma ? gamma[c] : 1.0f;
    mean_out[c] = mean;
    invstd_out[c] = invstd;
    scale_out[c] = g * invstd;
    shift_out[c] = beta ? beta[c] : 0.0f;
}

struct ChanWalk {
    int c, step, C;
    __device__ ChanWalk(int64_t e0, int64_t stride, int C_) : C(C_)
    {
        c = (int)(e0 % C_);
        step = (int)(stride % C_);
    }
    __device__ __forceinline__ void next()
    {
        c += step;
        if (c >= C) c -= C;
    }
};

__device__ __forceinline__ float leaky(float z, float slope) { return z > 0.0f ? z : z * slope; }

template <int V>
__global__ __launch_bounds__(RW_BLOCK) void bn_act_kernel(const float *__restrict__ Y, const float *__restrict__ mean,
                                                           const float *__restrict__ scale,
                                                           const float *__restrict__ shift, float slope,
                                                           int64_t total, int C, float *__restrict__ out)
{
    const int64_t stride = (int64_t)gridDim.x * RW_BLOCK * V;
    int64_t e = ((int64_t)blockIdx.x * RW_BLOCK + threadIdx.x) * V;
    ChanWalk cw(e, stride, C);
    for (; e < total; e += stride, cw.next()) {
        if (V == 4) {
            const float4 y = *reinterpret_cast<const float4 *>(Y + e);
            const float4 mu = *reinterpret_cast<const float4 *>(mean + cw.c);
            const float4 sc = *reinterpret_cast<const float4 *>(scale + cw.c);
            const float4 sh = *reinterpret_cast<const float4 *>(shift + cw.c);
            float4 o;
            o.x = leaky((y.x - mu.x) * sc.x + sh.x, slope);
            o.y = leaky((y.y - mu.y) * sc.y + sh.y, slope);
            o.z = leaky((y.z - mu.z) * sc.z + sh.z, slope);
            o.w = leaky((y.w - mu.w) * sc.w + sh.w, slope);
            *reinterpret_cast<float4 *>(out + e) = o;
        } else {
            out[e] = leaky((Y[e] - mean[cw.c]) * scale[cw.c] + shift[cw.c], slope);
        }
    }
}

__global__ __launch_bounds__(RW_BLOCK) void bn_act_maxpool_kernel(const float *__restrict__ Y,
                                                                   const float *__restrict__ mean,
                                                                   const float *__restrict__ scale,
                                                                   const float *__restrict__ shift, float slope,
                                                                   int64_t G, int ns, int C,
                                                                   float *__restrict__ out, int *__restrict__ arg)
{
    const int64_t total = G * C;
    for (int64_t e = (int64_t)blockIdx.x * RW_BLOCK + threadIdx.x; e < total; e += (int64_t)gridDim.x * RW_BLOCK) {
        const int64_t g = e / C;
        const int c = (int)(e - g * C);
        const float mu = mean[c], sc = scale[c], sh = shift[c];
        const float *y = Y + (size_t)g * ns * C + c;
        float best = -INFINITY;
        int bs = 0;
        int s = 0;
        auto take = [&](float a, int row) {
            const bool is_nan = (__float_as_uint(a) & 0x7fffffffu) > 0x7f800000u;
            const bool have_nan = (__float_as_uint(best) & 0x7fffffffu) > 0x7f800000u;
            if (!have_nan && (is_nan || a > best)) {
                best = a;
                bs = row;
            }
        };
        for (; s + 8 <= ns; s += 8) {
            float v[8];
#pragma unroll
            for (int u = 0; u < 8; ++u) v[u] = y[(size_t)(s + u) * C];
#pragma unroll
            for (int u = 0; u < 8; ++u) {
                const float z = (v[u] - mu) * sc + sh;
                take(z > 0.0f ? z : z * slope, s + u);
            }
        }
        for (; s < ns; ++s) {
            const float z = (y[(size_t)s * C] - mu) * sc + sh;
            take(z > 0.0f ? z : z * slope, s);
        }
        out[e] = best;
        arg[e] = bs;
    }
}

__global__ __launch_bounds__(RW_BLOCK) void bn_pool_bwd_partial_kernel(const float *__restrict__ dP,
                                                                        const int *__restrict__ arg,
                                                                        const float *__restrict__ Y,
                                                                        const float *__restrict__ scale,
                                                                        const float *__restrict__ shift,
                                                                        const float *__restrict__ mean,
                                                                        const float *__restrict__ invstd, float slope,
                                                                        int64_t G, int ns, int C, int chunk_rows,
                                                                        float *__restrict__ partial)
{
    __shared__ float s1[4][64], s2[4][64];
    const int tc = threadIdx.x & 63, tr = threadIdx.x >> 6;
    const int c = blockIdx.x * 64 + tc;
    const int64_t g0 = (int64_t)blockIdx.y * chunk_rows;
    const int64_t g1 = min(g0 + chunk_rows, G);
    float a = 0.0f, q = 0.0f;
    if (c < C) {
        const float sc = scale[c], sh = shift[c], mu = mean[c], is = invstd[c];
        for (int64_t g = g0 + tr; g < g1; g += 4) {
            const int s = arg[g * C + c];
            const float y = Y[((size_t)g * ns + s) * C + c];
            const float z = (y - mu) * sc + sh;
            const float dz = dP[g * C + c] * (z > 0.0f ? 1.0f : slope);
            a += dz;
            q += dz * ((y - mu) * is);
        }
    }
    s1[tr][tc] = a;
    s2[tr][tc] = q;
    __syncthreads();
    if (tr == 0 && c < C) {
        a = (s1[0][tc] + s1[1][tc]) + (s1[2][tc] + s1[3][tc]);
        q = (s2[0][tc] + s2[1][tc]) + (s2[2][tc] + s2[3][tc]);
        partial[((size_t)blockIdx.y * 2 + 0) * C + c] = a;
        partial[((size_t)blockIdx.y * 2 + 1) * C + c] = q;
    }
}

__global__ __launch_bounds__(RW_BLOCK) void bn_bwd_finalize_kernel(const float *__restrict__ partial, int chunks,
                                                                    int C, float *__restrict__ dbeta,
                                                                    float *__restrict__ dgamma,
                                                                    const float *__restrict__ invstd, int64_t M,
                                                                    int training, float *__restrict__ c1,
                                                                    float *__restrict__ c2)
{
    double a, q;
    sum_partials(partial, chunks, C, blockIdx.x, a, q);
    if (threadIdx.x == 0) {
        dbeta[blockIdx.x] = (float)a;
        dgamma[blockIdx.x] = (float)q;
        if (c1) {
            const float invM = 1.0f / (float)M;
            c1[blockIdx.x] = training ? (float)a * invM : 0.0f;
            c2[blockIdx.x] = training ? invstd[blockIdx.x] * ((float)q * invM) : 0.0f;
        }
    }
}

__device__ __forceinline__ float bn_bwd_elem(float da, float y, float sc, float sh, float mu, float is, float db,
                                             float dg, float slope, float invM, int training)
{
    const float z = (y - mu) * sc + sh;
    const float dz = da * (z > 0.0f ? 1.0f : slope);
    float v = dz;
    if (training) v = dz - db * invM - ((y - mu) * is) * (dg * invM);
    return sc * v;
}

template <int V>
__global__ __launch_bounds__(RW_BLOCK) void bn_act_bwd_apply_kernel(
    const float *__restrict__ dA, const float *__restrict__ Y, const float *__restrict__ scale,
    const float *__restrict__ shift, const float *__restrict__ mean, const float *__restrict__ invstd,
    const float *__restrict__ dbeta, const float *__restrict__ dgamma, float slope, int64_t M, int C, int training,
    float *__restrict__ dY)
{
    const int64_t total = M * C;
    const float invM = 1.0f / (float)M;
    const int64_t stride = (int64_t)gridDim.x * RW_BLOCK * V;
    int64_t e = ((int64_t)blockIdx.x * RW_BLOCK + threadIdx.x) * V;
    ChanWalk cw(e, stride, C);
    if (cw.step == 0 && e < total) {
        float sc[V], sh[V], mu[V], is[V], k1[V], k2[V];
#pragma unroll
        for (int v = 0; v < V; ++v) {
            const int c = cw.c + v;
            sc[v] = scale[c], sh[v] = shift[c], mu[v] = mean[c], is[v] = invstd[c];
            k1[v] = dbeta[c] * invM, k2[v] = dgamma[c] * invM;
        }
        for (; e < total; e += stride) {
            float y[V], d[V], o[V];
            if (V == 4) {
                *reinterpret_cast<float4 *>(y) = *reinterpret_cast<const float4 *>(Y + e);
                *reinterpret_cast<float4 *>(d) = *reinterpret_cast<const float4 *>(dA + e);
            } else {
                y[0] = Y[e];
                d[0] = dA[e];
            }
#pragma unroll
            for (int v = 0; v < V; ++v) {
                const float z = (y[v] - mu[v]) * sc[v] + sh[v];
                const float dz = d[v] * (z > 0.0f ? 1.0f : slope);
                float t = dz;
                if (training) t = dz - k1[v] - ((y[v] - mu[v]) * is[v]) * k2[v];
                o[v] = sc[v] * t;
            }
            if (V == 4) *reinterpret_cast<float4 *>(dY + e) = *reinterpret_cast<float4 *>(o);
            else dY[e] = o[0];
        }
        return;
    }
    for (; e < total; e += stride, cw.next()) {
        float y[V], d[V], o[V];
        if (V == 4) {
            *reinterpret_cast<float4 *>(y) = *reinterpret_cast<const float4 *>(Y + e);
            *reinterpret_cast<float4 *>(d) = *reinterpret_cast<const float4 *>(dA + e);
        } else {
            y[0] = Y[e];
            d[0] = dA[e];
        }
#pragma unroll
        for (int v = 0; v < V; ++v) {
            const int c = cw.c + v;
            o[v] = bn_bwd_elem(d[v], y[v], scale[c], shift[c], mean[c], invstd[c], dbeta[c], dgamma[c], slope, invM,
                               training);
        }
        if (V == 4) *reinterpret_cast<float4 *>(dY + e) = *reinterpret_cast<float4 *>(o);
        else dY[e] = o[0];
    }
}

__global__ __launch_bounds__(RW_BLOCK) void bn_pool_bwd_apply_kernel(
    const float *__restrict__ dP, const int *__restrict__ arg, const float *__restrict__ Y,
    const float *__restrict__ scale, const float *__restrict__ shift, const float *__restrict__ mean,
    const float *__restrict__ invstd, const float *__restrict__ dbeta, const float *__restrict__ dgamma, float slope,
    int64_t G, int ns, int C, int split, int training, float *__restrict__ dY)
{
    const int64_t GC = G * C, total = GC * split;
    const int seg_len = (ns + split - 1) / split;
    const float invM = 1.0f / (float)(G * ns);
    for (int64_t w = (int64_t)blockIdx.x * RW_BLOCK + threadIdx.x; w < total; w += (int64_t)gridDim.x * RW_BLOCK) {
        const int seg = (int)(w / GC);
        const int64_t e = w - (int64_t)seg * GC;
        const int64_t g = e / C;
        const int c = (int)(e - g * C);
        const float sc = scale[c], sh = shift[c], mu = mean[c], is = invstd[c], db = dbeta[c], dg = dgamma[c];
        const float dp = dP[e];
        const int sa = arg[e];
        const size_t base = (size_t)g * ns * C + c;
        const int s_end = min(ns, (seg + 1) * seg_len);
        int s = seg * seg_len;
        for (; s + 8 <= s_end; s += 8) {
            float y[8];
#pragma unroll
            for (int u = 0; u < 8; ++u) y[u] = Y[base + (size_t)(s + u) * C];
#pragma unroll
            for (int u = 0; u < 8; ++u)
                dY[base + (size_t)(s + u) * C] =
                    bn_bwd_elem(s + u == sa ? dp : 0.0f, y[u], sc, sh, mu, is, db, dg, slope, invM, training);
        }
        for (; s < s_end; ++s) {
            const float y = Y[base + (size_t)s * C];
            dY[base + (size_t)s * C] = bn_bwd_elem(s == sa ? dp : 0.0f, y, sc, sh, mu, is, db, dg, slope, invM, training);
        }
    }
}

__global__ __launch_bounds__(RW_BLOCK) void interp_concat_fwd_kernel(const float *__restrict__ feat_cl,
                                                                      const int64_t *__restrict__ idx,
                                                                      const float *__restrict__ w,
                                                                      const float *__restrict__ skip_cl, int m, int n,
                                                                      int C1, int C2, int ld, int64_t total,
                                                                      float *__restrict__ out)
{
    const int Cw = C1 + C2;
    for (int64_t e = (int64_t)blockIdx.x * RW_BLOCK + threadIdx.x; e < total; e += (int64_t)gridDim.x * RW_BLOCK) {
        const int64_t row = e / ld;
        const int c = (int)(e - row * ld);
        if (c >= Cw) {
            out[e] = 0.0f;
            continue;
        }
        float v;
        if (c < C1) {
            const int b = (int)(row / n);
            const int64_t *ip = idx + row * 3;
            const float *wp = w + row * 3;
            const int k0 = min(max((int)ip[0], 0), m - 1), k1 = min(max((int)ip[1], 0), m - 1),
                      k2 = min(max((int)ip[2], 0), m - 1);
            const float *fb = feat_cl + (size_t)b * m * C1 + c;
            const float a0 = wp[0] * fb[(size_t)k0 * C1];
            const float a1 = wp[1] * fb[(size_t)k1 * C1];
            const float a2 = wp[2] * fb[(size_t)k2 * C1];
            v = (a0 + a1) + a2;
        } else {
            v = skip_cl[row * C2 + (c - C1)];
        }
        out[e] = v;
    }
}

__global__ __launch_bounds__(RW_BLOCK) void interp_concat_fwd4_kernel(const float *__restrict__ feat_cl,
                                                                       const int64_t *__restrict__ idx,
                                                                       const float *__restrict__ w,
                                                                       const float *__restrict__ skip_cl, int m, int n,
                                                                       int C1, int C2, int ld, int64_t total4,
                                                                       float *__restrict__ out)
{
    const int Cw = C1 + C2, q = ld >> 2;
    for (int64_t e4 = (int64_t)blockIdx.x * RW_BLOCK + threadIdx.x; e4 < total4; e4 += (int64_t)gridDim.x * RW_BLOCK) {
        const int64_t row = e4 / q;
        const int c = (int)(e4 - row * q) * 4;
        float4 v;
        if (c < C1) {
            const int b = (int)(row / n);
            const int64_t *ip = idx + row * 3;
            const float *wp = w + row * 3;
            const int k0 = min(max((int)ip[0], 0), m - 1), k1 = min(max((int)ip[1], 0), m - 1),
                      k2 = min(max((int)ip[2], 0), m - 1);
            const float w0 = wp[0], w1 = wp[1], w2 = wp[2];
            const float *fb = feat_cl + (size_t)b * m * C1 + c;
            const float4 f0 = *reinterpret_cast<const float4 *>(fb + (size_t)k0 * C1);
            const float4 f1 = *reinterpret_cast<const float4 *>(fb + (size_t)k1 * C1);
            const float4 f2 = *reinterpret_cast<const float4 *>(fb + (size_t)k2 * C1);
            v.x = (w0 * f0.x + w1 * f1.x) + w2 * f2.x;
            v.y = (w0 * f0.y + w1 * f1.y) + w2 * f2.y;
            v.z = (w0 * f0.z + w1 * f1.z) + w2 * f2.z;
            v.w = (w0 * f0.w + w1 * f1.w) + w2 * f2.w;
        } else {
            float t[4];
#pragma unroll
            for (int j = 0; j < 4; ++j) t[j] = (c + j < Cw) ? skip_cl[row * C2 + (c + j - C1)] : 0.0f;
            v = make_float4(t[0], t[1], t[2], t[3]);
        }
        *reinterpret_cast<float4 *>(out + e4 * 4) = v;
    }
}

__global__ void idw_weights_kernel(const float *__restrict__ dist, int64_t rows, float *__restrict__ w)
{
    const int64_t r = (int64_t)blockIdx.x * blockDim.x + threadIdx.x;
    if (r >= rows) return;
    const float r0 = 1.0f / (dist[r * 3 + 0] + 1e-8f);
    const float r1 = 1.0f / (dist[r * 3 + 1] + 1e-8f);
    const float r2 = 1.0f / (dist[r * 3 + 2] + 1e-8f);
    const float norm = (r0 + r1) + r2;
    w[r * 3 + 0] = r0 / norm;
    w[r * 3 + 1] = r1 / norm;
    w[r * 3 + 2] = r2 / norm;
}

static inline unsigned grid_for(int64_t total)
{
    int64_t g = (total + RW_BLOCK - 1) / RW_BLOCK;
    return (unsigned)(g < 1 ? 1 : (g > 8192 ? 8192 : g));
}

}

using namespace tp3d;

TP3D_EXPORT int tp3d_group_concat_fwd_f32(const float *pos, const float *new_pos, const float *x_cl,
                                          const int64_t *idx, int B, int N, int np, int ns, int C, int ld,
                                          float radius, int normalize, float *out, void *stream)
{
    if (B < 0 || N <= 0 || np < 0 || ns < 0 || C < 0 || ld < C + 3) return TP3D_E_BADARG;
    const int64_t total = (int64_t)B * np * ns * ld;
    if (total == 0) return TP3D_OK;
    if (!pos || !new_pos || !idx || !out || (C > 0 && !x_cl)) return TP3D_E_BADARG;
    if ((ld & 3) == 0 && ((uintptr_t)out & 15) == 0)
        hipLaunchKernelGGL(group_concat_fwd4_kernel, dim3(grid_for(total / 4)), dim3(RW_BLOCK), 0, (hipStream_t)stream,
                           pos, new_pos, x_cl, idx, N, np, ns, C, ld, radius, normalize, total / 4, out);
    else
        hipLaunchKernelGGL(group_concat_fwd_kernel, dim3(grid_for(total)), dim3(RW_BLOCK), 0, (hipStream_t)stream, pos,
                           new_pos, x_cl, idx, N, np, ns, C, ld, radius, normalize, total, out);
    return check_launch();
}

namespace tp3d {
__global__ void slots_to_rows_kernel(int *__restrict__ order, const float *__restrict__ weight, int div, int L,
                                     const int *__restrict__ start, int nbins, float *__restrict__ wsorted)
{
    const int j = blockIdx.x * blockDim.x + threadIdx.x;
    if (j >= L || j >= start[nbins]) return;
    const int slot = order[j];
    if (wsorted) wsorted[j] = weight[slot];
    order[j] = slot / div;
}
}

namespace tp3d {
static bool scatter_goes_flat(int B, int L, int nbins)
{
    return L >= 2 * nbins && (int64_t)B * L < 0x7fffffff && (int64_t)B * nbins < 0x3fffffff &&
           ((B == 1 && L >= 16384) || !csr_fits_lds(L, nbins));
}
}

TP3D_EXPORT int tp3d_scatter_plan(int B, int L, int nbins, int with_weights, int64_t *plan)
{
    if (B <= 0 || L <= 0 || nbins <= 0 || !plan) return TP3D_E_BADARG;
    const ScatterWorkspace w = carve_scatter_workspace(nullptr, B, L, nbins, with_weights != 0);
    plan[0] = (char *)w.start - (char *)nullptr;
    plan[1] = (char *)w.order - (char *)nullptr;
    plan[2] = (char *)w.scratch - (char *)nullptr;
    plan[3] = w.wsorted ? (char *)w.wsorted - (char *)nullptr : -1;
    plan[4] = (char *)w.merge_tmp - (char *)nullptr;
    plan[5] = (int64_t)w.bytes;
    plan[6] = scatter_goes_flat(B, L, nbins) ? 1 : 0;
    plan[7] = plan[6] ? 2 * (int64_t)B * nbins : 0;
    plan[8] = (char *)w.hubs - (char *)nullptr;
    return TP3D_OK;
}

TP3D_EXPORT int tp3d_rows_scatter_invert(const int64_t *idx, const float *weight, int B, int L, int div, int nbins,
                                         void *workspace, size_t workspace_bytes, void *stream)
{
    if (B < 0 || L < 0 || div <= 0 || nbins <= 0) return TP3D_E_BADARG;
    if (B == 0 || L == 0) return TP3D_OK;
    if (!idx || !workspace || B > 65535) return TP3D_E_BADARG;
    hipStream_t s = (hipStream_t)stream;
    ScatterWorkspace w = carve_scatter_workspace(workspace, B, L, nbins, weight != nullptr);
    if (workspace_bytes < w.bytes) return TP3D_E_BADARG;
    const bool flat = scatter_goes_flat(B, L, nbins);
    if (flat) {
        const int64_t slots = (int64_t)B * L, bins = (int64_t)B * nbins;
        if (int rc = invert_table(idx, slots, bins, w.scratch, w.start, w.scratch + bins, w.order, s, L, nbins, w.merge_tmp))
            return rc;
        hipLaunchKernelGGL(slots_to_rows_kernel, dim3((unsigned)((slots + 255) / 256)), dim3(256), 0, s, w.order, weight, div,
                           (int)slots, w.start, (int)bins, w.wsorted);
        if (int rc = check_launch()) return rc;
    } else if (int rc = csr_transpose(idx, B, L, nbins, div, weight, w.start, w.order, w.wsorted, w.scratch, s)) {
        return rc;
    }
    if (int rc = zero_async(w.hubs, sizeof(int), s)) return rc;
    hipLaunchKernelGGL(find_hubs_kernel, dim3((unsigned)(((int64_t)B * nbins + 255) / 256)), dim3(256), 0, s, w.start, B, nbins,
                       flat ? 1 : 0, w.hubs);
    return check_launch();
}

TP3D_EXPORT int tp3d_rows_scatter_apply_f32(const float *grad_rows, int B, int L, int div, int nbins, int ld, int col0,
                                            int C, int with_weights, float *grad_x_cl, void *table, size_t table_bytes,
                                            void *stream)
{
    if (B < 0 || L < 0 || div <= 0 || nbins <= 0 || ld <= 0 || col0 < 0 || C < 0 || col0 + C > ld) return TP3D_E_BADARG;
    if (B == 0 || C == 0) return TP3D_OK;
    if (!grad_x_cl) return TP3D_E_BADARG;
    hipStream_t s = (hipStream_t)stream;
    if (L == 0) return zero_async(grad_x_cl, (size_t)B * nbins * C * sizeof(float), s);
    if (!grad_rows || !table || B > 65535) return TP3D_E_BADARG;
    ScatterWorkspace w = carve_scatter_workspace(table, B, L, nbins, with_weights != 0);
    if (table_bytes < w.bytes) return TP3D_E_BADARG;
    const bool flat = scatter_goes_flat(B, L, nbins);
    dim3 grid((nbins + RW_BLOCK / 64 - 1) / (RW_BLOCK / 64), B);
    const dim3 hub_grid(256);
    const int fl = flat ? 1 : 0;
    if (C > 128) {
        hipLaunchKernelGGL(rows_gather_sum_kernel<4>, grid, dim3(RW_BLOCK), 0, s, grad_rows, w.start, w.order, w.wsorted,
                           nbins, L, L / div, ld, col0, C, grad_x_cl, fl, HUB_MIN);
        hipLaunchKernelGGL(rows_gather_hub_kernel<4>, hub_grid, dim3(HUB_BLOCK), 0, s, grad_rows, w.start, w.order, w.wsorted,
                           w.hubs, nbins, L, L / div, ld, col0, C, grad_x_cl, fl);
    } else if (C > 64) {
        hipLaunchKernelGGL(rows_gather_sum_kernel<2>, grid, dim3(RW_BLOCK), 0, s, grad_rows, w.start, w.order, w.wsorted,
                           nbins, L, L / div, ld, col0, C, grad_x_cl, fl, HUB_MIN);
        hipLaunchKernelGGL(rows_gather_hub_kernel<2>, hub_grid, dim3(HUB_BLOCK), 0, s, grad_rows, w.start, w.order, w.wsorted,
                           w.hubs, nbins, L, L / div, ld, col0, C, grad_x_cl, fl);
    } else {
        hipLaunchKernelGGL(rows_gather_sum_kernel<1>, grid, dim3(RW_BLOCK), 0, s, grad_rows, w.start, w.order, w.wsorted,
                           nbins, L, L / div, ld, col0, C, grad_x_cl, fl, HUB_MIN);
        hipLaunchKernelGGL(rows_gather_hub_kernel<1>, hub_grid, dim3(HUB_BLOCK), 0, s, grad_rows, w.start, w.order, w.wsorted,
                           w.hubs, nbins, L, L / div, ld, col0, C, grad_x_cl, fl);
    }
    return check_launch();
}

TP3D_EXPORT int tp3d_rows_scatter_bwd_f32(const float *grad_rows, const int64_t *idx, const float *weight, int B,
                                          int L, int div, int nbins, int ld, int col0, int C, float *grad_x_cl,
                                          void *workspace, size_t workspace_bytes, void *stream)
{
    if (B < 0 || L < 0 || div <= 0 || nbins <= 0 || ld <= 0 || col0 < 0 || C < 0 || col0 + C > ld) return TP3D_E_BADARG;
    if (B == 0 || C == 0) return TP3D_OK;
    if (!grad_x_cl) return TP3D_E_BADARG;
    if (L == 0) return zero_async(grad_x_cl, (size_t)B * nbins * C * sizeof(float), (hipStream_t)stream);
    if (!grad_rows || !idx || !workspace || B > 65535) return TP3D_E_BADARG;
    if (int rc = tp3d_rows_scatter_invert(idx, weight, B, L, div, nbins, workspace, workspace_bytes, stream)) return rc;
    return tp3d_rows_scatter_apply_f32(grad_rows, B, L, div, nbins, ld, col0, C, weight != nullptr, grad_x_cl, workspace,
                                       workspace_bytes, stream);
}

TP3D_EXPORT size_t tp3d_bn_workspace_floats(int64_t M, int C)
{
    if (M < 0 || C < 0) return 0;
    int64_t chunks = M >= ST_SMALL_BELOW ? (M + ST_ROWS - 1) / ST_ROWS : (M + ST_ROWS_SMALL - 1) / ST_ROWS_SMALL;
    if (M >= ST_SMALL_BELOW && chunks < ST_SMALL_BELOW / ST_ROWS_SMALL) chunks = ST_SMALL_BELOW / ST_ROWS_SMALL;
    return (size_t)chunks * 4 * (size_t)C;
}

TP3D_EXPORT int tp3d_bn_plan(int64_t M, int C, int pooled_ns, int64_t *plan)
{
    if (M <= 0 || C <= 0 || pooled_ns < 0 || !plan) return TP3D_E_BADARG;
    const int64_t R = pooled_ns > 1 ? M / pooled_ns : M;
    const int crow = stat_rows(R);
    plan[0] = crow;
    plan[1] = (R + crow - 1) / crow;
    plan[2] = plan[1] * (pooled_ns == 0 ? 4 : 2) * C;
    return TP3D_OK;
}

constexpr int BN_DIRECT_CHUNKS = 64, BN_SLICES = 32;
static int launch_bn_finalize(float *partial, int chunks, int64_t M, int C, float eps, float momentum, const float *gamma,
                              const float *beta, float *running_mean, float *running_var, int64_t *batches, int training,
                              float *mean, float *invstd, float *scale, float *shift, hipStream_t s)
{
    int n = chunks, stride = 1;
    if (training && chunks > BN_DIRECT_CHUNKS) {
        stride = (chunks + BN_SLICES - 1) / BN_SLICES;
        n = (chunks + stride - 1) / stride;
        hipLaunchKernelGGL(bn_merge_slices_kernel, dim3((C + BM_COLS - 1) / BM_COLS, n), dim3(RW_BLOCK), 0, s, partial, chunks,
                           stride, C);
        if (int rc = check_launch()) return rc;
    }
    hipLaunchKernelGGL(bn_finalize_kernel, dim3(C), dim3(RW_BLOCK), 0, s, partial, n, stride, M, C, eps, momentum, gamma, beta,
                       running_mean, running_var, batches, training, mean, invstd, scale, shift);
    return check_launch();
}

TP3D_EXPORT int tp3d_bn_stats_f32(const float *Y, int64_t M, int C, float eps, float momentum, const float *gamma,
                                  const float *beta, float *running_mean, float *running_var,
                                  int64_t *num_batches_tracked, int training, float *mean, float *invstd, float *scale,
                                  float *shift, float *workspace, void *stream)
{
    if (M <= 0 || C <= 0 || !mean || !invstd || !scale || !shift) return TP3D_E_BADARG;
    if (!training && (!running_mean || !running_var)) return TP3D_E_BADARG;
    hipStream_t s = (hipStream_t)stream;
    const int crow = stat_rows(M);
    const int chunks = (int)((M + crow - 1) / crow);
    if (training) {
        if (!Y || !workspace) return TP3D_E_BADARG;
        if (chunks > 65535) return TP3D_E_TOOBIG;
        if ((C & 3) == 0) {
            const StatTile t = stat_tile(C, 4);
            hipLaunchKernelGGL((colreduce_partial_kernel<4, 0>), dim3(t.gridx, chunks), dim3(RW_BLOCK), 0, s, Y,
                               (const float *)nullptr, (const float *)nullptr, (const float *)nullptr,
                               (const float *)nullptr, (const float *)nullptr, 0.0f, M, C, t.colthreads, crow, workspace);
        } else {
            const StatTile t = stat_tile(C, 1);
            hipLaunchKernelGGL((colreduce_partial_kernel<1, 0>), dim3(t.gridx, chunks), dim3(RW_BLOCK), 0, s, Y,
                               (const float *)nullptr, (const float *)nullptr, (const float *)nullptr,
                               (const float *)nullptr, (const float *)nullptr, 0.0f, M, C, t.colthreads, crow, workspace);
        }
        if (int rc = check_launch()) return rc;
    }
    return launch_bn_finalize(workspace, chunks, M, C, eps, momentum, gamma, beta, running_mean, running_var,
                              num_batches_tracked, training, mean, invstd, scale, shift, s);
}

TP3D_EXPORT int tp3d_bn_finalize_f32(float *partial, int chunks, int64_t M, int C, float eps, float momentum,
                                     const float *gamma, const float *beta, float *running_mean, float *running_var,
                                     int64_t *num_batches_tracked, float *mean, float *invstd, float *scale, float *shift,
                                     void *stream)
{
    if (M <= 0 || C <= 0 || chunks <= 0 || !partial || !mean || !invstd || !scale || !shift) return TP3D_E_BADARG;
    return launch_bn_finalize(partial, chunks, M, C, eps, momentum, gamma, beta, running_mean, running_var,
                              num_batches_tracked, 1, mean, invstd, scale, shift, (hipStream_t)stream);
}

TP3D_EXPORT int tp3d_bn_act_f32(const float *Y, const float *mean, const float *scale, const float *shift, float slope,
                                int64_t M, int C, float *out, void *stream)
{
    if (M < 0 || C <= 0) return TP3D_E_BADARG;
    if (M == 0) return TP3D_OK;
    if (!Y || !mean || !scale || !shift || !out) return TP3D_E_BADARG;
    const int64_t total = M * C;
    if ((C & 3) == 0)
        hipLaunchKernelGGL(bn_act_kernel<4>, dim3(grid_for(total / 4)), dim3(RW_BLOCK), 0, (hipStream_t)stream, Y, mean,
                           scale, shift, slope, total, C, out);
    else
        hipLaunchKernelGGL(bn_act_kernel<1>, dim3(grid_for(total)), dim3(RW_BLOCK), 0, (hipStream_t)stream, Y, mean,
                           scale, shift, slope, total, C, out);
    return check_launch();
}

TP3D_EXPORT int tp3d_bn_act_maxpool_f32(const float *Y, const float *mean, const float *scale, const float *shift,
                                        float slope, int64_t G, int ns, int C, float *out, int *argmax, void *stream)
{
    if (G < 0 || ns <= 0 || C <= 0) return TP3D_E_BADARG;
    if (G == 0) return TP3D_OK;
    if (!Y || !mean || !scale || !shift || !out || !argmax) return TP3D_E_BADARG;
    hipLaunchKernelGGL(bn_act_maxpool_kernel, dim3(grid_for(G * C)), dim3(RW_BLOCK), 0, (hipStream_t)stream, Y, mean, scale,
                       shift, slope, G, ns, C, out, argmax);
    return check_launch();
}

namespace tp3d {
int bn_bwd_finalize_launch(const float *partial, int chunks, int C, float *dbeta, float *dgamma, const float *invstd, int64_t M,
                           int training, float *c1, float *c2, hipStream_t s)
{
    hipLaunchKernelGGL(bn_bwd_finalize_kernel, dim3(C), dim3(RW_BLOCK), 0, s, partial, chunks, C, dbeta, dgamma, invstd, M,
                       training, c1, c2);
    return check_launch();
}

static int bn_bwd_reduce(const float *dA, const int *argmax, const float *Y, const float *scale, const float *shift,
                         const float *mean, const float *invstd, float slope, int64_t M, int ns, int C, int training,
                         float *dbeta, float *dgamma, float *c1, float *c2, float *workspace, int reverse, hipStream_t s)
{
    const int64_t R = argmax ? M / ns : M;
    const int crow = stat_rows(R);
    const int chunks = (int)((R + crow - 1) / crow);
    if (chunks > 65535) return TP3D_E_TOOBIG;
    if (argmax) {
        hipLaunchKernelGGL(bn_pool_bwd_partial_kernel, dim3((C + 63) / 64, chunks), dim3(RW_BLOCK), 0, s, dA, argmax, Y,
                           scale, shift, mean, invstd, slope, R, ns, C, crow, workspace);
    } else if ((C & 3) == 0) {
        const StatTile t = stat_tile(C, 4);
        hipLaunchKernelGGL((colreduce_partial_kernel<4, 1>), dim3(t.gridx, chunks), dim3(RW_BLOCK), 0, s, Y, dA, scale,
                           shift, mean, invstd, slope, M, C, t.colthreads, crow, workspace, reverse);
    } else {
        const StatTile t = stat_tile(C, 1);
        hipLaunchKernelGGL((colreduce_partial_kernel<1, 1>), dim3(t.gridx, chunks), dim3(RW_BLOCK), 0, s, Y, dA, scale,
                           shift, mean, invstd, slope, M, C, t.colthreads, crow, workspace);
    }
    if (int rc = check_launch()) return rc;
    hipLaunchKernelGGL(bn_bwd_finalize_kernel, dim3(C), dim3(RW_BLOCK), 0, s, workspace, chunks, C, dbeta, dgamma, invstd, M,
                       training, c1, c2);
    return check_launch();
}
}

TP3D_EXPORT int tp3d_bn_bwd_reduce_f32(const float *dA, const int *argmax, const float *Y, const float *scale,
                                       const float *shift, const float *mean, const float *invstd, float slope,
                                       int64_t M, int ns, int C, int training, float *dbeta, float *dgamma, float *c1,
                                       float *c2, float *workspace, int reverse, void *stream)
{
    if (M <= 0 || C <= 0 || ns <= 0 || (argmax && M % ns)) return TP3D_E_BADARG;
    if (!dA || !Y || !scale || !shift || !mean || !invstd || !dbeta || !dgamma || !c1 || !c2 || !workspace)
        return TP3D_E_BADARG;
    return bn_bwd_reduce(dA, argmax, Y, scale, shift, mean, invstd, slope, M, ns, C, training, dbeta, dgamma, c1, c2,
                         workspace, reverse, (hipStream_t)stream);
}

TP3D_EXPORT int tp3d_bn_act_bwd_f32(const float *dA, const int *argmax, const float *Y, const float *scale,
                                    const float *shift, const float *mean, const float *invstd, float slope,
                                    int64_t M, int ns, int C, int training, float *dbeta, float *dgamma, float *dY,
                                    float *workspace, void *stream)
{
    if (M <= 0 || C <= 0 || ns <= 0 || (argmax && M % ns)) return TP3D_E_BADARG;
    if (!dA || !Y || !scale || !shift || !mean || !invstd || !dbeta || !dgamma || !dY || !workspace)
        return TP3D_E_BADARG;
    hipStream_t s = (hipStream_t)stream;
    const int64_t R = argmax ? M / ns : M;
    if (int rc = bn_bwd_reduce(dA, argmax, Y, scale, shift, mean, invstd, slope, M, ns, C, training, dbeta, dgamma, nullptr,
                               nullptr, workspace, 0, s))
        return rc;
    if (argmax) {
        int split = (int)((262144 + R * C - 1) / (R * C));
        split = split < 1 ? 1 : (split > ns ? ns : split);
        hipLaunchKernelGGL(bn_pool_bwd_apply_kernel, dim3(grid_for(R * C * split)), dim3(RW_BLOCK), 0, s, dA, argmax, Y,
                           scale, shift, mean, invstd, dbeta, dgamma, slope, R, ns, C, split, training, dY);
    }
    else if ((C & 3) == 0)
        hipLaunchKernelGGL(bn_act_bwd_apply_kernel<4>, dim3(grid_for(M * C / 4)), dim3(RW_BLOCK), 0, s, dA, Y, scale,
                           shift, mean, invstd, dbeta, dgamma, slope, M, C, training, dY);
    else
        hipLaunchKernelGGL(bn_act_bwd_apply_kernel<1>, dim3(grid_for(M * C)), dim3(RW_BLOCK), 0, s, dA, Y, scale,
                           shift, mean, invstd, dbeta, dgamma, slope, M, C, training, dY);
    return check_launch();
}

TP3D_EXPORT int tp3d_interp_concat_fwd_f32(const float *feat_cl, const int64_t *idx, const float *weight,
                                           const float *skip_cl, int B, int m, int n, int C1, int C2, int ld,
                                           float *out, void *stream)
{
    if (B < 0 || m <= 0 || n < 0 || C1 < 0 || C2 < 0 || ld < C1 + C2) return TP3D_E_BADARG;
    const int64_t total = (int64_t)B * n * ld;
    if (total == 0) return TP3D_OK;
    if (!out || (C1 > 0 && (!feat_cl || !idx || !weight)) || (C2 > 0 && !skip_cl)) return TP3D_E_BADARG;
    if ((ld & 3) == 0 && (C1 & 3) == 0 && (((uintptr_t)feat_cl | (uintptr_t)out) & 15) == 0)
        hipLaunchKernelGGL(interp_concat_fwd4_kernel, dim3(grid_for(total / 4)), dim3(RW_BLOCK), 0, (hipStream_t)stream,
                           feat_cl, idx, weight, skip_cl, m, n, C1, C2, ld, total / 4, out);
    else
        hipLaunchKernelGGL(interp_concat_fwd_kernel, dim3(grid_for(total)), dim3(RW_BLOCK), 0, (hipStream_t)stream,
                           feat_cl, idx, weight, skip_cl, m, n, C1, C2, ld, total, out);
    return check_launch();
}

namespace tp3d {
__global__ __launch_bounds__(RW_BLOCK) void relation_rows_kernel(const float *__restrict__ pos,
                                                                  const float *__restrict__ new_pos,
                                                                  const int64_t *__restrict__ idx, int N, int np, int ns,
                                                                  int ld, int64_t rows, float *__restrict__ out)
{
    for (int64_t row = (int64_t)blockIdx.x * RW_BLOCK + threadIdx.x; row < rows; row += (int64_t)gridDim.x * RW_BLOCK) {
        const int64_t bj = row / ns;
        const int b = (int)(bj / np);
        const int k = min(max((int)idx[row], 0), N - 1);
        const float *p = pos + ((size_t)b * N + k) * 3, *c = new_pos + bj * 3;
        const float px = p[0], py = p[1], pz = p[2], cx = c[0], cy = c[1], cz = c[2];
        const float dx = px - cx, dy = py - cy, dz = pz - cz;
        float v[12] = {sqrtf((dx * dx + dy * dy) + dz * dz), cx, cy, cz, px, py, pz, dx, dy, dz, 0.0f, 0.0f};
        float *o = out + row * ld;
        if (ld == 12 && ((uintptr_t)out & 15) == 0) {
#pragma unroll
            for (int q = 0; q < 3; ++q) reinterpret_cast<float4 *>(o)[q] = make_float4(v[4 * q], v[4 * q + 1], v[4 * q + 2], v[4 * q + 3]);
        } else {
            for (int q = 0; q < ld; ++q) o[q] = q < 10 ? v[q] : 0.0f;
        }
    }
}
}

TP3D_EXPORT int tp3d_relation_rows_f32(const float *pos, const float *new_pos, const int64_t *idx, int B, int N, int np,
                                       int ns, int ld, float *out, void *stream)
{
    if (B < 0 || N <= 0 || np < 0 || ns < 0 || ld < 10) return TP3D_E_BADARG;
    const int64_t rows = (int64_t)B * np * ns;
    if (rows == 0) return TP3D_OK;
    if (!pos || !new_pos || !idx || !out) return TP3D_E_BADARG;
    hipLaunchKernelGGL(relation_rows_kernel, dim3(grid_for(rows)), dim3(RW_BLOCK), 0, (hipStream_t)stream, pos, new_pos, idx,
                       N, np, ns, ld, rows, out);
    return check_launch();
}

TP3D_EXPORT int tp3d_idw_weights_f32(const float *dist, int64_t rows, float *weight, void *stream)
{
    if (rows < 0) return TP3D_E_BADARG;
    if (rows == 0) return TP3D_OK;
    if (!dist || !weight) return TP3D_E_BADARG;
    hipLaunchKernelGGL(idw_weights_kernel, dim3((unsigned)((rows + 255) / 256)), dim3(256), 0, (hipStream_t)stream,
                       dist, rows, weight);
    return check_launch();
}
```

torch_points3d_amd/csrc/tp3d_common.h:

```cpp
#pragma once
#include <hip/hip_runtime.h>
#include <stdint.h>

#include "tp3d_hip.h"

#define TP3D_EXPORT extern "C" __attribute__((visibility("default")))

namespace tp3d {

constexpr int kWave = 64;

void set_last_hip_error(hipError_t e);

inline int check_launch()
{
    hipError_t e = hipGetLastError();
    if (e != hipSuccess) {
        set_last_hip_error(e);
        return TP3D_E_LAUNCH;
    }
    return TP3D_OK;
}

inline void allow_large_dynamic_lds(const void *func, int bytes, bool *done_per_device )
{
    int dev = 0;
    if (hipGetDevice(&dev) != hipSuccess || dev < 0 || dev >= 64) dev = 0;
    if (!done_per_device[dev]) {
        (void)hipFuncSetAttribute(func, hipFuncAttributeMaxDynamicSharedMemorySize, bytes);
        done_per_device[dev] = true;
    }
}

inline int zero_async(void *ptr, size_t bytes, hipStream_t s)
{
    if (bytes == 0) return TP3D_OK;
    hipError_t e = hipMemsetAsync(ptr, 0, bytes, s);
    if (e != hipSuccess) {
        set_last_hip_error(e);
        return TP3D_E_LAUNCH;
    }
    return TP3D_OK;
}

__device__ __forceinline__ float sqdist3(float ax, float ay, float az, float bx, float by, float bz)
{
    float dx = ax - bx;
    float dy = ay - by;
    float dz = az - bz;
    return (dx * dx + dy * dy) + dz * dz;
}

struct ScatterWorkspace {
    int *start;
    int *order;
    int *scratch;
    float *wsorted;
    int *merge_tmp;
    int *hubs;
    size_t bytes;
};
ScatterWorkspace carve_scatter_workspace(void *ws, int B, int L, int nbins, bool with_weights);
int csr_transpose(const int64_t *idx, int B, int L, int nbins, int div, const float *weight, int *start, int *order,
                  float *wsorted, int *scratch_ord, hipStream_t s);
int gather_sum(const float *rows, const int *start, const int *order, const float *wsorted, int B, int C, int nbins,
               int Lrow, int Lslots, float *out, hipStream_t s);

int invert_table(const int64_t *idx, int64_t slots, int64_t M, int *cnt, int *start, int *cursor, int *order,
                 hipStream_t s, int64_t per_cloud_slots = 0, int64_t per_cloud_bins = 0, int *merge_tmp = nullptr);
int invert_neighbors(const int64_t *neighbors, int64_t slots, int64_t M, void *workspace, int **start_out,
                     int **order_out, hipStream_t s, bool ready = false);
int gather_slot_rows(const float *g, const int *start, const int *order, int64_t M, int Cin, float *d_x, hipStream_t s);
bool csr_fits_lds(int L, int nbins);

int bn_bwd_finalize_launch(const float *partial, int chunks, int C, float *dbeta, float *dgamma, const float *invstd, int64_t M,
                           int training, float *c1, float *c2, hipStream_t s);
int tn_reduce_splits(const float *partial, int splits, int64_t NK, float *out, hipStream_t s);

int grid_ball_query(const float *x, const float *y, const int64_t *seg, const int64_t *batch_y, int num_clouds,
                    int64_t rows, int N, int np, int64_t total_q, int Lmax, float radius, int nsample, int sort,
                    int64_t *idx, float *dist2, void *workspace, size_t workspace_bytes, bool reuse_grid, hipStream_t s);

__device__ __forceinline__ int lane_id() { return threadIdx.x & (kWave - 1); }

__device__ __forceinline__ int lanes_below(unsigned long long mask)
{
    return __builtin_amdgcn_mbcnt_hi((unsigned)(mask >> 32), __builtin_amdgcn_mbcnt_lo((unsigned)mask, 0));
}


template <int NU, typename OrdT>
__device__ __forceinline__ void wave_sort_bin(OrdT *__restrict__ bin, int n, int lane)
{
    int e[NU];
#pragma unroll
    for (int u = 0; u < NU; ++u) e[u] = (lane + 64 * u < n) ? (int)bin[lane + 64 * u] : 0x7fffffff;
#pragma unroll
    for (int size = 2; size <= 64 * NU; size <<= 1) {
#pragma unroll
        for (int stride = size >> 1; stride >= 1; stride >>= 1) {
            if (stride >= 64) {
#pragma unroll
                for (int u = 0; u < NU; ++u) {
                    const int pu = u ^ (stride >> 6);
                    if (pu > u) {
                        const bool up = (((u << 6) | lane) & size) == 0;
                        const int a = e[u], b = e[pu];
                        const bool swap = up ? a > b : a < b;
                        e[u] = swap ? b : a;
                        e[pu] = swap ? a : b;
                    }
                }
            } else {
#pragma unroll
                for (int u = 0; u < NU; ++u) {
                    const int other = __shfl_xor(e[u], stride);
                    const bool up = (((u << 6) | lane) & size) == 0;
                    const bool lower = (lane & stride) == 0;
                    e[u] = (lower == up) ? min(e[u], other) : max(e[u], other);
                }
            }
        }
    }
    __builtin_amdgcn_fence(__ATOMIC_RELEASE, "workgroup");
    __builtin_amdgcn_wave_barrier();
#pragma unroll
    for (int u = 0; u < NU; ++u)
        if (lane + 64 * u < n) bin[lane + 64 * u] = (OrdT)e[u];
}

}
```

torch_points3d_amd/fused.py:

```python
import collections

import torch
import torch.nn as nn

from . import _lib


USE_ROWS_GEMM = True


def _cl(x):
    return x.transpose(1, 2).contiguous()


def _pad4(c):
    return (c + 3) & ~3


def _slope_of(act):
    if act is None:
        return 1.0
    if isinstance(act, nn.LeakyReLU):
        return float(act.negative_slope)
    if isinstance(act, nn.ReLU):
        return 0.0
    return None


def layer_parts(block):
    mods = list(block.children())
    if not mods or not isinstance(mods[0], (nn.Conv2d, nn.Conv1d)):
        return None
    conv = mods[0]
    if conv.bias is not None or any(k != 1 for k in conv.kernel_size):
        return None
    bn, act = None, None
    for m in mods[1:]:
        if isinstance(m, (nn.BatchNorm2d, nn.BatchNorm1d)) and bn is None and act is None:
            bn = m
        elif act is None:
            act = m
        else:
            return None
    if bn is None or not bn.affine or not bn.track_running_stats or bn.momentum is None:
        return None
    slope = _slope_of(act)
    if slope is None:
        return None
    return conv, bn, slope


def mlp_parts(mlp):
    parts = [layer_parts(b) for b in mlp.children()]
    return None if (not parts or any(p is None for p in parts)) else parts


FWD_X3 = True
WGRAD_X3_ACT = True
WGRAD_X3 = 6


_ident = {}


def _identity_stats(K, dev):
    key = (dev.index, K)
    hit = _ident.get(key)
    if hit is None:
        hit = _ident[key] = (torch.zeros(K, dtype=torch.float32, device=dev), torch.ones(K, dtype=torch.float32, device=dev))
    return hit


def _chain_wgrad(b, dY, l, A0, acts, Ys, stats, slopes, dA_prev=None, training=True):
    if b.wgrad not in ("x3_act", "x3_act_red"):
        return _gemm_tn_launch(b.wgrad, dY, A0 if l == 0 else acts[l - 1], b.terms, None, b.wgrad_rev), None
    ps = stats[l - 1]
    if b.wgrad == "x3_act":
        return _gemm_tn_launch("x3_act", dY, Ys[l - 1], b.terms, (ps[0], ps[2], ps[3], slopes[l - 1]), b.wgrad_rev), None
    dev = dY.device
    M, N = dY.shape
    K = Ys[l - 1].shape[1]
    out = torch.empty((N, K), dtype=torch.float32, device=dev)
    red = torch.empty((4, K), dtype=torch.float32, device=dev)
    ws = _lib.gemm_tn_workspace(M, N, K, dev, x3=True)
    rws = _lib.workspace("gemm_tn_red", 4 * 2 * b.wgrad_chunks * K, dev)
    with _lib.on_device(dev):
        _lib.call("tp3d_gemm_tn_x3_act_red_f32", _lib.ptr(dY), _lib.ptr(Ys[l - 1]), _lib.ptr(ps[0]), _lib.ptr(ps[2]), _lib.ptr(ps[3]),
                  _lib.ptr(ps[1]), float(slopes[l - 1]), _lib.ptr(dA_prev), int(training), M, N, K, 6, _lib.ptr(out), _lib.ptr(ws),
                  _lib.ptr(red), _lib.ptr(rws), int(b.wgrad_rev), _lib.stream_ptr(dev))
    return out, red


def _chain_wgrad_narrow(dY_src, Y, ls, red, slope, A0, reverse, st):
    dev = Y.device
    M, C = Y.shape
    Kp = A0.shape[1]
    dW = torch.empty((C, Kp), dtype=torch.float32, device=dev)
    nws = _lib.workspace("gemm_tn_narrow", 4 * _lib.load().tp3d_gemm_tn_bn_narrow_workspace_floats(M, C, Kp), dev)
    _lib.call("tp3d_gemm_tn_bn_narrow_f32", _lib.ptr(Y), _lib.ptr(dY_src), _lib.ptr(ls[0]), _lib.ptr(ls[2]),
              _lib.ptr(ls[3]), _lib.ptr(red[2]), _lib.ptr(red[3]), slope, _lib.ptr(A0), M, C, Kp, _lib.ptr(dW),
              _lib.ptr(nws), reverse, st)
    return dW


def gemm_tn(dY, A, x3=None, act=None, reverse=0):
    dY, A = dY.contiguous(), A.contiguous()
    M, N = dY.shape
    K = A.shape[1]
    terms = WGRAD_X3 if x3 is None else x3
    kernel = "x3" if terms and M > 0 and _lib.load().tp3d_gemm_tn_x3_serves(M, N, K) else "tn"
    if act is not None:
        if kernel != "x3":
            raise ValueError("gemm_tn(act=): only the bf16-pipe contraction forms its A operand (shape %s x %s x %s)" % (M, N, K))
        kernel = "x3_act"
    return _gemm_tn_launch(kernel, dY, A, terms, act, reverse)


def _gemm_tn_launch(kernel, dY, A, terms, act, reverse):
    dev = dY.device
    M, N = dY.shape
    K = A.shape[1]
    out = torch.empty((N, K), dtype=torch.float32, device=dev)
    ws = _lib.gemm_tn_workspace(M, N, K, dev, x3=kernel != "tn")
    with _lib.on_device(dev):
        if kernel == "x3_act":
            _lib.call("tp3d_gemm_tn_x3_act_f32", _lib.ptr(dY), _lib.ptr(A), _lib.ptr(act[0]), _lib.ptr(act[1]), _lib.ptr(act[2]),
                      float(act[3]), M, N, K, int(terms), _lib.ptr(out), _lib.ptr(ws), int(reverse), _lib.stream_ptr(dev))
        elif kernel == "x3":
            _lib.call("tp3d_gemm_tn_x3_f32", _lib.ptr(dY), _lib.ptr(A), M, N, K, int(terms), _lib.ptr(out), _lib.ptr(ws), int(reverse),
                      _lib.stream_ptr(dev))
        else:
            _lib.call("tp3d_gemm_tn_f32", _lib.ptr(dY), _lib.ptr(A), M, N, K, _lib.ptr(out), _lib.ptr(ws),
                      _lib.stream_ptr(dev))
    return out


SKINNY_MAX = 32
SKINNY_MIN_ROWS = 32768


def gemm_skinny(A, W):
    dev = A.device
    A, W = A.contiguous(), W.contiguous()
    M, K = A.shape
    N = W.shape[0]
    Y = torch.empty((M, N), dtype=torch.float32, device=dev)
    with _lib.on_device(dev):
        _lib.call("tp3d_gemm_skinny_f32", _lib.ptr(A), _lib.ptr(W), M, N, K, K, _lib.ptr(Y), _lib.stream_ptr(dev))
    return Y


def _is_skinny(M, a, b):
    return M >= SKINNY_MIN_ROWS and a <= SKINNY_MAX and b <= SKINNY_MAX


def gemm_rows(A, Bt, want_stats=False):
    dev = A.device
    M, K = A.shape
    N = Bt.shape[0]
    Bm = Bt.contiguous()
    C = torch.empty((M, N), dtype=torch.float32, device=dev)
    part, slabs = None, None
    h = _lib.load()
    if want_stats:
        part = _lib.workspace("gemm_rows_stats", 4 * h.tp3d_gemm_rows_stat_floats(M, N), dev)
    else:
        n = h.tp3d_gemm_rows_workspace_floats(M, N, K)
        if n:
            slabs = _lib.workspace("gemm_rows_slabs", 4 * n, dev)
    with _lib.on_device(dev):
        _lib.call("tp3d_gemm_rows_f32", _lib.ptr(A), _lib.ptr(Bm), M, N, K, _lib.ptr(C), _lib.ptr(part), _lib.ptr(slabs),
                  _lib.stream_ptr(dev))
    return C, part


def _finalize_stats(part, M, C, gamma, beta, bn, dev, st, chunks=None):
    stats = torch.empty((4, C), dtype=torch.float32, device=dev)
    if chunks is None:
        chunks = _lib.load().tp3d_gemm_rows_stat_chunks(M, C)
    _lib.call("tp3d_bn_finalize_f32", _lib.ptr(part), chunks, M, C, float(bn.eps),
              float(bn.momentum), _lib.ptr(gamma), _lib.ptr(beta), _lib.ptr(bn.running_mean), _lib.ptr(bn.running_var),
              _lib.ptr(bn.num_batches_tracked), _lib.ptr(stats[0]), _lib.ptr(stats[1]), _lib.ptr(stats[2]), _lib.ptr(stats[3]), st)
    _note_training_pass(bn)
    return stats


def _note_training_pass(bn):
    bn._tp3d_train_passes = getattr(bn, "_tp3d_train_passes", 0) + 1


_replay_epoch = 0


def note_graph_replay():
    global _replay_epoch
    _replay_epoch += 1


ROWS_GEMM_MIN_COLS = 32
ROWS_GEMM_WITHOUT_STATS = True
ROWS_GEMM_EPILOGUE = True
ROWS_GEMM_NARROW = True
CHAIN_MIN_ROWS = 32768


def _rows_gemm_serves(cout):
    if not USE_ROWS_GEMM or cout < ROWS_GEMM_MIN_COLS:
        return False
    return ROWS_GEMM_NARROW or not (0 < cout % 128 <= 64)


def _bn_stats(Y, M, C, gamma, beta, bn, training, dev, st, bias=None):
    key = None
    if not training:
        key = tuple((t.data_ptr(), t._version) for t in (gamma, beta, bn.running_mean, bn.running_var)
                    + ((bias,) if bias is not None else ())) + (getattr(bn, "_tp3d_train_passes", 0), _replay_epoch)
        hit = getattr(bn, "_tp3d_eval_stats", None)
        if hit is not None and hit[0] == key:
            return hit[1]
    stats = torch.empty((4, C), dtype=torch.float32, device=dev)
    ws = _lib.bn_workspace(M, C, dev)
    _lib.call("tp3d_bn_stats_f32", _lib.ptr(Y), M, C, float(bn.eps), float(bn.momentum), _lib.ptr(gamma), _lib.ptr(beta),
              _lib.ptr(bn.running_mean), _lib.ptr(bn.running_var), _lib.ptr(bn.num_batches_tracked) if training else None,
              int(training), _lib.ptr(stats[0]), _lib.ptr(stats[1]), _lib.ptr(stats[2]), _lib.ptr(stats[3]), _lib.ptr(ws), st)
    if training:
        _note_training_pass(bn)
    if key is not None:
        if bias is not None:
            stats[0].sub_(bias.detach())
        bn._tp3d_eval_stats = (key, stats)
    return stats


def _bn_act_out(Y, stats, slope, pool_ns, st):
    dev = Y.device
    M, C = Y.shape
    if pool_ns:
        G = M // pool_ns
        out = torch.empty((G, C), dtype=torch.float32, device=dev)
        arg = torch.empty((G, C), dtype=torch.int32, device=dev)
        _lib.call("tp3d_bn_act_maxpool_f32", _lib.ptr(Y), _lib.ptr(stats[0]), _lib.ptr(stats[2]), _lib.ptr(stats[3]), slope, G,
                  pool_ns, C, _lib.ptr(out), _lib.ptr(arg), st)
        return out, arg
    out = torch.empty((M, C), dtype=torch.float32, device=dev)
    _lib.call("tp3d_bn_act_f32", _lib.ptr(Y), _lib.ptr(stats[0]), _lib.ptr(stats[2]), _lib.ptr(stats[3]), slope, M, C,
              _lib.ptr(out), st)
    return out, None


def _bn_act_bwd(grad_out, arg, Y, stats, slope, pool_ns, training, st):
    dev = Y.device
    M, C = Y.shape
    dY = torch.empty_like(Y)
    dgb = torch.empty((2, C), dtype=torch.float32, device=dev)
    ws = _lib.bn_workspace(M, C, dev)
    _lib.call("tp3d_bn_act_bwd_f32", _lib.ptr(grad_out), _lib.ptr(arg), _lib.ptr(Y), _lib.ptr(stats[2]),
              _lib.ptr(stats[3]), _lib.ptr(stats[0]), _lib.ptr(stats[1]), slope, M, max(pool_ns, 1), C,
              int(training), _lib.ptr(dgb[0]), _lib.ptr(dgb[1]), _lib.ptr(dY), _lib.ptr(ws), st)
    return dY, dgb


def _layer_route(M, Kp, Cout, training, pool_ns, want_grad):
    skinny = _is_skinny(M, Kp, Cout)
    if not training and skinny and not want_grad:
        return "skinny_bnact", False
    few_tiles = ((M + 127) // 128) * ((Cout + 127) // 128) < 128 and 512 <= Kp < 1024
    rows = _rows_gemm_serves(Cout) and Kp % 4 == 0 and not few_tiles
    want_stats = training and _lib.load().tp3d_gemm_rows_workspace_floats(M, Cout, Kp) == 0
    if rows and ROWS_GEMM_EPILOGUE and not training and not pool_ns and ROWS_GEMM_WITHOUT_STATS and not want_grad:
        return "rows_epi", False
    if rows and (want_stats or ROWS_GEMM_WITHOUT_STATS):
        return "rows", want_stats
    if skinny:
        return "skinny", False
    return "library", False


class _LinearBNAct(torch.autograd.Function):

    @staticmethod
    def forward(ctx, A, weight, gamma, beta, bn, slope, pool_ns, grad_enabled, bias=None):
        dev = A.device
        A = A.contiguous()
        M, Kp = A.shape
        Cout = weight.shape[0]
        W2 = weight.reshape(Cout, -1)
        Cin = W2.shape[1]
        if Kp != Cin:
            W2 = torch.nn.functional.pad(W2, (0, Kp - Cin))
        training = bn.training
        st = _lib.stream_ptr(dev)
        path, want_stats = _layer_route(M, Kp, Cout, training, pool_ns, grad_enabled and any(ctx.needs_input_grad))
        if path in ("skinny_bnact", "rows_epi"):
            with _lib.on_device(dev):
                stats = _bn_stats(A, M, Cout, gamma, beta, bn, False, dev, st, bias)
                out = torch.empty((M, Cout), dtype=torch.float32, device=dev)
                if path == "skinny_bnact":
                    _lib.call("tp3d_gemm_skinny_bnact_f32", _lib.ptr(A), _lib.ptr(W2.contiguous()), M, Cout, Kp, Kp,
                              _lib.ptr(stats[0]), _lib.ptr(stats[2]), _lib.ptr(stats[3]), slope, _lib.ptr(out), st)
                else:
                    n = _lib.load().tp3d_gemm_rows_workspace_floats(M, Cout, Kp)
                    slabs = _lib.workspace("gemm_rows_slabs", 4 * n, dev) if n else None
                    _lib.call("tp3d_gemm_rows_epi_f32", _lib.ptr(A), _lib.ptr(W2.contiguous()), M, Cout, Kp, _lib.ptr(stats[0]),
                              _lib.ptr(stats[2]), _lib.ptr(stats[3]), slope, _lib.ptr(out), _lib.ptr(slabs), st)
            return out.view(M // pool_ns, pool_ns, Cout).max(1)[0] if pool_ns else out
        part = None
        if path == "rows":
            Y, part = gemm_rows(A, W2, want_stats=want_stats)
        elif path == "skinny":
            Y = gemm_skinny(A, W2)
        else:
            Y = torch.mm(A, W2.t())
        with _lib.on_device(dev):
            if part is not None:
                stats = _finalize_stats(part, M, Cout, gamma, beta, bn, dev, st)
            else:
                stats = _bn_stats(Y, M, Cout, gamma, beta, bn, training, dev, st, bias)
            out, arg = _bn_act_out(Y, stats, slope, pool_ns, st)
        if training and bias is not None:
            bn.running_mean.add_(bias.detach(), alpha=float(bn.momentum))
        ctx.save_for_backward(A, W2, Y, stats, arg)
        ctx.cfg = (slope, pool_ns, training, tuple(weight.shape), Cin, bias is not None)
        return out

    @staticmethod
    def backward(ctx, grad_out):
        A, W2, Y, stats, arg = ctx.saved_tensors
        slope, pool_ns, training, wshape, Cin, has_bias = ctx.cfg
        dev = grad_out.device
        grad_out = grad_out.contiguous()
        M, Cout = Y.shape
        need_A, need_W, need_bias = ctx.needs_input_grad[0], ctx.needs_input_grad[1], ctx.needs_input_grad[-1]
        with _lib.on_device(dev):
            dY, dgb = _bn_act_bwd(grad_out, arg, Y, stats, slope, pool_ns, training, _lib.stream_ptr(dev))
        dW = None
        if need_W:
            dW = gemm_tn(dY, A)[:, :Cin].reshape(wshape)
        dA = None
        if need_A:
            if _is_skinny(M, W2.shape[1], Cout):
                dA = gemm_skinny(dY, W2.t())
            else:
                dA = torch.mm(dY, W2)
        dbias = None
        if has_bias and need_bias:
            dbias = torch.zeros(Y.shape[1], dtype=torch.float32, device=dev) if training else dY.sum(0)
        return dA, dW, dgb[1], dgb[0], None, None, None, None, dbias


class _MLPChain(torch.autograd.Function):

    @staticmethod
    def forward(ctx, A0, pool_ns, layers, grad_cols, grad_enabled, *params):
        dev = A0.device
        A0 = A0.contiguous()
        M, K0 = A0.shape
        st = _lib.stream_ptr(dev)
        L = len(layers)
        training = layers[0][0].training
        need = ctx.needs_input_grad
        first = len(need) - len(params)
        plan = _plan_chain(M, K0, [params[3 * l].shape[0] for l in range(L)], pool_ns, grad_enabled and any(need), need[0],
                           need[first::3], grad_cols)
        Ys, stats, W2s, cins, acts = [], [], [], [], [None] * (L - 1)
        with _lib.on_device(dev):
            for l, ((bn, slope), p) in enumerate(zip(layers, plan)):
                weight, gamma, beta = params[3 * l], params[3 * l + 1], params[3 * l + 2]
                Cout = weight.shape[0]
                W2 = weight.reshape(Cout, -1)
                Kp = K0 if l == 0 else Ys[-1].shape[1]
                cins.append(W2.shape[1])
                if W2.shape[1] != Kp:
                    W2 = torch.nn.functional.pad(W2, (0, Kp - W2.shape[1]))
                W2 = W2.contiguous()
                Y = torch.empty((M, Cout), dtype=torch.float32, device=dev)
                part = None
                if training:
                    nbytes = 16 * p.chunks * Cout if p.reverse is not None else 4 * _lib.load().tp3d_gemm_rows_stat_floats(M, Cout)
                    part = _lib.workspace("gemm_rows_stats", nbytes, dev)
                if p.kernel == "narrow":
                    _lib.call("tp3d_gemm_rows_narrow_f32", _lib.ptr(A0), _lib.ptr(W2), M, Cout, Kp, _lib.ptr(Y), _lib.ptr(part), p.reverse, st)
                elif p.kernel in ("rows", "bn_act_rows"):
                    src = A0
                    if l:
                        src = _bn_act_out(Ys[-1], stats[-1], layers[l - 1][1], 0, st)[0]
                        acts[l - 1] = src if p.keep_act else None
                    _lib.call("tp3d_gemm_rows_f32", _lib.ptr(src), _lib.ptr(W2), M, Cout, Kp, _lib.ptr(Y), _lib.ptr(part), None, st)
                else:
                    if l == 0:
                        ident = _identity_stats(Kp, dev)
                        src, mean, scale, shift, pslope = A0, ident[0], ident[1], ident[0], 1.0
                    else:
                        ps = stats[-1]
                        src, mean, scale, shift, pslope = Ys[-1], ps[0], ps[2], ps[3], layers[l - 1][1]
                        acts[l - 1] = torch.empty((M, Kp), dtype=torch.float32, device=dev) if p.keep_act else None
                    _lib.call("tp3d_gemm_rows_bnact_sp_f32" if p.kernel == "sp" else "tp3d_gemm_rows_bnact_x3_f32", _lib.ptr(src),
                              _lib.ptr(mean), _lib.ptr(scale), _lib.ptr(shift), pslope, _lib.ptr(W2), M, Cout, Kp, _lib.ptr(Y),
                              _lib.ptr(part), _lib.ptr(acts[l - 1]) if l else None, p.reverse, st)
                if training:
                    stats.append(_finalize_stats(part, M, Cout, gamma, beta, bn, dev, st, p.chunks))
                else:
                    stats.append(_bn_stats(Y, M, Cout, gamma, beta, bn, False, dev, st))
                Ys.append(Y)
                W2s.append(W2)
            out, arg = _bn_act_out(Ys[-1], stats[-1], layers[-1][1], pool_ns, st)
        ctx.save_for_backward(A0, arg, *Ys, *stats, *W2s, *(acts if plan[0].bwd else []))
        ctx.cfg = (L, pool_ns, training, [s_ for _, s_ in layers], [tuple(params[3 * l].shape) for l in range(L)], cins)
        ctx.plan = plan
        return out

    @staticmethod
    def backward(ctx, grad_out):
        L, pool_ns, training, slopes, wshapes, cins = ctx.cfg
        saved = ctx.saved_tensors
        A0, arg = saved[0], saved[1]
        Ys, stats, W2s = saved[2:2 + L], saved[2 + L:2 + 2 * L], saved[2 + 2 * L:2 + 3 * L]
        dev = grad_out.device
        st = _lib.stream_ptr(dev)
        M = A0.shape[0]
        dcur = grad_out.contiguous()
        grads = [None] * (3 * L)
        if not ctx.plan[0].bwd:
            raise RuntimeError("_MLPChain.backward: the forward pass ran without a gradient request (grad mode off at the call site)")
        acts = saved[2 + 3 * L:2 + 3 * L + (L - 1)]
        red_next = None
        with _lib.on_device(dev):
            for l in range(L - 1, -1, -1):
                Y, ls, W2, slope, b = Ys[l], stats[l], W2s[l], slopes[l], ctx.plan[l].bwd
                C, Kp = W2.shape
                pooled_arg, ns = (arg, pool_ns) if (pool_ns and l == L - 1) else (None, 0)
                if b.kind == "passes":
                    dY, dgb = _bn_act_bwd(dcur, pooled_arg, Y, ls, slope, ns, training, st)
                    grads[3 * l + 1], grads[3 * l + 2] = dgb[1], dgb[0]
                    if b.wgrad:
                        grads[3 * l] = _chain_wgrad(b, dY, l, A0, acts, Ys, stats, slopes)[0][:, :cins[l]].reshape(wshapes[l])
                    if b.dx:
                        dcur = torch.mm(dY, W2)
                    continue
                red, red_next = red_next, None
                if b.reduce_rev is not None:
                    red = torch.empty((4, C), dtype=torch.float32, device=dev)
                    _lib.call("tp3d_bn_bwd_reduce_f32", _lib.ptr(dcur), _lib.ptr(pooled_arg), _lib.ptr(Y), _lib.ptr(ls[2]), _lib.ptr(ls[3]),
                              _lib.ptr(ls[0]), _lib.ptr(ls[1]), slope, M, max(ns, 1), C, int(training), _lib.ptr(red[0]),
                              _lib.ptr(red[1]), _lib.ptr(red[2]), _lib.ptr(red[3]), _lib.ptr(_lib.bn_workspace(M, C, dev)), b.reduce_rev, st)
                grads[3 * l + 1], grads[3 * l + 2] = red[1], red[0]
                if b.kind == "narrow":
                    dW = _chain_wgrad_narrow(dcur, Y, ls, red, slope, A0, b.wgrad_rev, st)
                    grads[3 * l] = dW[:, :cins[l]].reshape(wshapes[l])
                    continue
                dY = torch.empty_like(Y) if b.write_dY else None
                dprev = torch.empty((M, Kp), dtype=torch.float32, device=dev)
                c0, ncol = b.cols if b.cols else (0, Kp)
                pad_hi = Kp - c0 - ncol
                Wt = W2.t()[c0:c0 + ncol].contiguous()
                pad_lo_k, pad_hi_k = c0, pad_hi
                if c0 > 32 or pad_hi > 32:
                    dprev.zero_()
                    pad_lo_k = pad_hi_k = 0
                _lib.call("tp3d_gemm_rows_bnbwd_sp_f32", _lib.ptr(Y), _lib.ptr(dcur), _lib.ptr(ls[0]), _lib.ptr(ls[2]),
                          _lib.ptr(ls[3]), _lib.ptr(red[2]), _lib.ptr(red[3]), slope, _lib.ptr(Wt), M, ncol, C,
                          _lib.ptr(dprev) + 4 * c0, Kp, pad_lo_k, pad_hi_k, _lib.ptr(dY), _lib.ptr(pooled_arg), max(ns, 1), b.dx_rev, st)
                if b.wgrad:
                    dW, red_next = _chain_wgrad(b, dY, l, A0, acts, Ys, stats, slopes, dprev, training)
                    grads[3 * l] = dW[:, :cins[l]].reshape(wshapes[l])
                dcur = dprev
        return (dcur if ctx.plan[0].bwd.dx else None, None, None, None, None) + tuple(grads)


def _chain_ok(rows, parts):
    if not USE_MLP_CHAIN or rows.shape[0] < CHAIN_MIN_ROWS or rows.shape[1] % 4:
        return False
    for conv, bn, slope in parts:
        cout = conv.weight.shape[0]
        if getattr(conv, "bias", None) is not None or cout % 4 or cout < ROWS_GEMM_MIN_COLS or cout > 1536:
            return False
    return True


USE_MLP_CHAIN = True
CHAIN_BWD_LOADER = True
CHAIN_BWD_POOLED = True
ROW_ORDER_ALTERNATE = True
WGRAD_NARROW = True
FWD_NARROW = True
WGRAD_RED = True

_ChainLayer = collections.namedtuple("_ChainLayer", "kernel chunks reverse keep_act bwd")
_ChainLayerBwd = collections.namedtuple("_ChainLayerBwd", "kind cols reduce_rev dx dx_rev write_dY wgrad wgrad_rev wgrad_chunks terms")


def _plan_chain(M, K0, widths, pool_ns, want_grad, need_in, need_w, grad_cols):
    h = _lib.load()
    L = len(widths)
    Ks = [K0] + list(widths[:-1])
    alt = bool(ROW_ORDER_ALTERNATE)
    tn = ["x3" if WGRAD_X3 and h.tp3d_gemm_tn_x3_serves(M, widths[l], Ks[l]) else "tn" for l in range(L)]
    keep = [bool(want_grad and l > 0 and not (WGRAD_X3_ACT and need_w[l] and tn[l] == "x3")) for l in range(L)]

    fwd, prev = [], 0
    for l in range(L):
        Cout, Kp, side = widths[l], Ks[l], int(keep[l])
        sp = h.tp3d_gemm_rows_sp_chunks(M, Cout, Kp, side) if l else 0
        x3 = h.tp3d_gemm_rows_x3_chunks(M, Cout, Kp, side) if (FWD_X3 and (sp or not l)) else 0
        if x3:
            kernel, chunks = "x3" if l else "x3_identity", x3
        elif sp:
            kernel, chunks = "sp", sp
        elif not l and FWD_NARROW and h.tp3d_gemm_tn_bn_narrow_serves(M, Cout, Kp):
            kernel, chunks = "narrow", h.tp3d_gemm_rows_narrow_chunks(M)
        else:
            kernel, chunks = "bn_act_rows" if l else "rows", h.tp3d_gemm_rows_stat_chunks(M, Cout)
        directed = kernel not in ("rows", "bn_act_rows")
        prev = int(directed and alt and not prev)
        fwd.append((kernel, chunks, prev if directed else None, keep[l]))
    if not want_grad:
        return tuple(_ChainLayer(*f, bwd=None) for f in fwd)

    kinds, cols = [], []
    for l in range(L):
        C, Kp = widths[l], Ks[l]
        pooled = bool(pool_ns) and l == L - 1
        want_prev = l > 0 or need_in
        cols.append(grad_cols if (l == 0 and grad_cols is not None and grad_cols[1] >= ROWS_GEMM_MIN_COLS) else None)
        pow2 = pooled and pool_ns >= 64 and (pool_ns & (pool_ns - 1)) == 0
        if (CHAIN_BWD_LOADER and (not pooled or (CHAIN_BWD_POOLED and pow2)) and want_prev
                and h.tp3d_gemm_rows_bnbwd_sp_serves(M, cols[l][1] if cols[l] else Kp, C)):
            kinds.append("loader")
        elif (WGRAD_NARROW and not pooled and not want_prev and need_w[l] and l == 0
                and h.tp3d_gemm_tn_bn_narrow_serves(M, C, Kp)):
            kinds.append("narrow")
        else:
            kinds.append("passes")

    rev = (int(alt), 0)
    bwd, turn = [None] * L, 0
    red_above = False
    for l in range(L - 1, -1, -1):
        plain = "x3_act" if (l > 0 and not keep[l]) else tn[l]
        if kinds[l] == "passes":
            wgrad = plain if need_w[l] else None
            bwd[l] = _ChainLayerBwd("passes", cols[l], None, l > 0 or need_in, None, True, wgrad, 0 if wgrad in ("x3", "x3_act") else None,
                                    0, WGRAD_X3)
            continue
        reduce_rev = None
        if not red_above:
            reduce_rev, turn = rev[turn % 2], turn + 1
        red_above = False
        if kinds[l] == "narrow":
            bwd[l] = _ChainLayerBwd("narrow", cols[l], reduce_rev, False, None, False, "narrow", rev[turn % 2], 0, WGRAD_X3)
            turn += 1
            continue
        dx_rev, turn = rev[turn % 2], turn + 1
        wgrad, wgrad_rev, chunks = None, None, 0
        if need_w[l] and WGRAD_RED and l > 0 and not keep[l] and kinds[l - 1] != "passes":
            chunks = h.tp3d_gemm_tn_x3_red_chunks(M, widths[l], Ks[l]) if WGRAD_X3 == 6 else 0
            if chunks:
                wgrad, wgrad_rev, red_above = "x3_act_red", rev[turn % 2], True
            turn += 1
        if need_w[l] and not chunks:
            wgrad, wgrad_rev, turn = plain, (rev[turn % 2] if plain != "tn" else None), turn + 1
        bwd[l] = _ChainLayerBwd("loader", cols[l], reduce_rev, True, dx_rev, need_w[l], wgrad, wgrad_rev, chunks, WGRAD_X3)
    return tuple(_ChainLayer(*f, bwd=b) for f, b in zip(fwd, bwd))


class _BNAct(torch.autograd.Function):

    @staticmethod
    def forward(ctx, Y, gamma, beta, bn, slope, pool_ns=0):
        dev = Y.device
        Y = Y.contiguous()
        M, C = Y.shape
        training = bn.training
        st = _lib.stream_ptr(dev)
        with _lib.on_device(dev):
            stats = _bn_stats(Y, M, C, gamma, beta, bn, training, dev, st)
            out, arg = _bn_act_out(Y, stats, slope, pool_ns, st)
        ctx.save_for_backward(Y, stats, arg)
        ctx.cfg = (slope, training, pool_ns)
        return out

    @staticmethod
    def backward(ctx, grad_out):
        Y, stats, arg = ctx.saved_tensors
        slope, training, pool_ns = ctx.cfg
        dev = grad_out.device
        with _lib.on_device(dev):
            dY, dgb = _bn_act_bwd(grad_out.contiguous(), arg, Y, stats, slope, pool_ns, training, _lib.stream_ptr(dev))
        return dY, dgb[1], dgb[0], None, None, None


def bn_act(Y, bn, slope, pool_ns=0):
    return _BNAct.apply(Y, bn.weight, bn.bias, bn, slope, pool_ns)


def relation_rows(pos, new_pos, idx):
    dev = pos.device
    B, N, _ = pos.shape
    _, npnt, ns = idx.shape
    out = torch.empty((B * npnt * ns, 12), dtype=torch.float32, device=dev)
    with _lib.on_device(dev):
        _lib.call("tp3d_relation_rows_f32", _lib.ptr(pos.contiguous()), _lib.ptr(new_pos.contiguous()),
                  _lib.ptr(idx.contiguous()), B, N, npnt, ns, 12, _lib.ptr(out), _lib.stream_ptr(dev))
    return out


class _NbrMaxPool(torch.autograd.Function):

    @staticmethod
    def forward(ctx, x, nbr):
        dev = x.device
        xf = x.contiguous()
        Nq, Mn = nbr.shape
        M, C = xf.shape
        out = torch.empty((Nq, C), dtype=torch.float32, device=dev)
        need = ctx.needs_input_grad[0]
        arg = torch.empty((Nq, C), dtype=torch.int32, device=dev) if need else None
        with _lib.on_device(dev):
            _lib.call("tp3d_nbr_maxpool_fwd_f32", _lib.ptr(xf), _lib.ptr(nbr), Nq, M, Mn, C, _lib.ptr(out), _lib.ptr(arg),
                      _lib.stream_ptr(dev))
        ctx.save_for_backward(nbr, arg)
        ctx.cfg = (M, C)
        return out

    @staticmethod
    def backward(ctx, g):
        nbr, arg = ctx.saved_tensors
        M, C = ctx.cfg
        dev = g.device
        g = g.contiguous()
        Nq, Mn = nbr.shape
        dx = torch.empty((M, C), dtype=torch.float32, device=dev)
        with _lib.on_device(dev):
            inv, inv_bytes, ready, token = _lib.neighbour_inverse(nbr, M, dev)
            _lib.call("tp3d_nbr_maxpool_bwd_f32", _lib.ptr(g), _lib.ptr(arg), _lib.ptr(nbr), Nq, M, Mn, C, _lib.ptr(dx),
                      _lib.ptr(inv), inv_bytes, ready, _lib.stream_ptr(dev))
            _lib.inverse_built(token, dev)
        return dx, None


def nbr_maxpool(x, nbr):
    return _NbrMaxPool.apply(x.float(), nbr)


def linear_bn_act(A, conv, bn, slope, pool_ns=0):
    return _LinearBNAct.apply(A, conv.weight, bn.weight, bn.bias, bn, slope, pool_ns, torch.is_grad_enabled(), getattr(conv, "bias", None))


def _bn1d_of(m):
    inner = getattr(m, "batch_norm", m)
    if isinstance(inner, nn.BatchNorm1d) and inner.affine and inner.track_running_stats and inner.momentum is not None:
        return inner
    return None


def seq_parts(seq):
    mods = list(seq.children()) if isinstance(seq, nn.Sequential) else []
    if len(mods) not in (2, 3) or not isinstance(mods[0], nn.Linear):
        return None
    bn = _bn1d_of(mods[1])
    slope = _slope_of(mods[2] if len(mods) == 3 else None)
    if bn is None or slope is None:
        return None
    return mods[0], bn, slope


def rows_seq(seq, x):
    parts = seq_parts(seq) if x.is_cuda else None
    if parts is None:
        return seq(x)
    lin, bn, slope = parts
    return linear_bn_act(x.float(), lin, bn, slope)


def rows_mlp(mlp, x):
    for block in mlp.children():
        x = rows_seq(block, x)
    return x


def run_mlp(rows, parts, pool_ns=0):
    if _chain_ok(rows, parts):
        flat = []
        for conv, bn, slope in parts:
            flat += [conv.weight, bn.weight, bn.bias]
        return _MLPChain.apply(rows, pool_ns, [(bn, slope) for _, bn, slope in parts], getattr(rows, "_tp3d_grad_cols", None),
                               torch.is_grad_enabled(), *flat)
    for i, (conv, bn, slope) in enumerate(parts):
        rows = linear_bn_act(rows, conv, bn, slope, pool_ns if i == len(parts) - 1 else 0)
    return rows


def scatter_table(idx, weight, nbins, div):
    dev = idx.device
    B = idx.shape[0]
    L = idx[0].numel()
    nbytes = _lib.load().tp3d_scatter_workspace_bytes(B, L, nbins, int(weight is not None))
    buf = torch.empty(nbytes, dtype=torch.uint8, device=dev)
    idx = idx.contiguous()
    w = None if weight is None else weight.contiguous()
    with _lib.on_device(dev):
        _lib.call("tp3d_rows_scatter_invert", _lib.ptr(idx), _lib.ptr(w), B, L, div, nbins, _lib.ptr(buf), nbytes,
                  _lib.stream_ptr(dev))
    return buf


class _GroupConcat(torch.autograd.Function):

    @staticmethod
    def forward(ctx, pos, new_pos, x_cl, idx, radius, normalize, table=None):
        dev = pos.device
        B, N, _ = pos.shape
        _, npnt, ns = idx.shape
        C = 0 if x_cl is None else x_cl.shape[2]
        pos, new_pos, idx = pos.contiguous(), new_pos.contiguous(), idx.contiguous()
        xc = None if x_cl is None else x_cl.contiguous()
        ld = _pad4(C + 3)
        out = torch.empty((B * npnt * ns, ld), dtype=torch.float32, device=dev)
        with _lib.on_device(dev):
            _lib.call("tp3d_group_concat_fwd_f32", _lib.ptr(pos), _lib.ptr(new_pos), _lib.ptr(xc), _lib.ptr(idx), B, N,
                      npnt, ns, C, ld, float(radius), int(bool(normalize)), _lib.ptr(out), _lib.stream_ptr(dev))
        ctx.save_for_backward(idx, table)
        ctx.dims = (B, N, npnt, ns, C, ld)
        return out

    @staticmethod
    def backward(ctx, grad_rows):
        idx, table = ctx.saved_tensors
        B, N, npnt, ns, C, ld = ctx.dims
        if C == 0 or not ctx.needs_input_grad[2]:
            return None, None, None, None, None, None, None
        dev = grad_rows.device
        grad_rows = grad_rows.contiguous()
        g = torch.empty((B, N, C), dtype=torch.float32, device=dev)
        L = npnt * ns
        with _lib.on_device(dev):
            if table is not None:
                _lib.call("tp3d_rows_scatter_apply_f32", _lib.ptr(grad_rows), B, L, 1, N, ld, 3, C, 0, _lib.ptr(g),
                          _lib.ptr(table), table.numel(), _lib.stream_ptr(dev))
            else:
                ws, ws_bytes = _lib.scatter_workspace(B, L, N, False, dev)
                _lib.call("tp3d_rows_scatter_bwd_f32", _lib.ptr(grad_rows), _lib.ptr(idx), None, B, L, 1, N, ld, 3, C,
                          _lib.ptr(g), _lib.ptr(ws), ws_bytes, _lib.stream_ptr(dev))
        return None, None, g, None, None, None, None


def group_concat(pos, new_pos, x_cl, idx, radius, normalize, table=None):
    rows = _GroupConcat.apply(pos, new_pos, x_cl, idx, radius, normalize, table)
    if x_cl is not None:
        rows._tp3d_grad_cols = (3, x_cl.shape[2])
    return rows


class _InterpConcat(torch.autograd.Function):

    @staticmethod
    def forward(ctx, feat_cl, idx, weight, skip_cl, table=None):
        dev = feat_cl.device
        B, m, C1 = feat_cl.shape
        n = idx.shape[1]
        C2 = 0 if skip_cl is None else skip_cl.shape[2]
        feat_cl, idx, weight = feat_cl.contiguous(), idx.contiguous(), weight.contiguous()
        sk = None if skip_cl is None else skip_cl.contiguous()
        ld = _pad4(C1 + C2)
        out = torch.empty((B * n, ld), dtype=torch.float32, device=dev)
        with _lib.on_device(dev):
            _lib.call("tp3d_interp_concat_fwd_f32", _lib.ptr(feat_cl), _lib.ptr(idx), _lib.ptr(weight), _lib.ptr(sk), B,
                      m, n, C1, C2, ld, _lib.ptr(out), _lib.stream_ptr(dev))
        ctx.save_for_backward(idx, weight, table)
        ctx.dims = (B, m, n, C1, C2, ld)
        return out

    @staticmethod
    def backward(ctx, grad_rows):
        idx, weight, table = ctx.saved_tensors
        B, m, n, C1, C2, ld = ctx.dims
        dev = grad_rows.device
        grad_rows = grad_rows.contiguous()
        g_feat = None
        if ctx.needs_input_grad[0]:
            g_feat = torch.empty((B, m, C1), dtype=torch.float32, device=dev)
            with _lib.on_device(dev):
                if table is not None:
                    _lib.call("tp3d_rows_scatter_apply_f32", _lib.ptr(grad_rows), B, 3 * n, 3, m, ld, 0, C1, 1,
                              _lib.ptr(g_feat), _lib.ptr(table), table.numel(), _lib.stream_ptr(dev))
                else:
                    ws, ws_bytes = _lib.scatter_workspace(B, 3 * n, m, True, dev)
                    _lib.call("tp3d_rows_scatter_bwd_f32", _lib.ptr(grad_rows), _lib.ptr(idx), _lib.ptr(weight), B, 3 * n,
                              3, m, ld, 0, C1, _lib.ptr(g_feat), _lib.ptr(ws), ws_bytes, _lib.stream_ptr(dev))
        g_skip = None
        if C2 and ctx.needs_input_grad[3]:
            g_skip = grad_rows.view(B, n, ld)[:, :, C1:C1 + C2]
        return g_feat, None, None, g_skip, None


def interp_concat(feat_cl, idx, weight, skip_cl, table=None):
    rows = _InterpConcat.apply(feat_cl, idx, weight, skip_cl, table)
    if skip_cl is not None and not (skip_cl.requires_grad and torch.is_grad_enabled()):
        rows._tp3d_grad_cols = (0, feat_cl.shape[2])
    return rows


def cat_rows(parts):
    B, n = parts[0].shape[0], parts[0].shape[1]
    width = sum(p.shape[2] for p in parts)
    if _pad4(width) != width:
        parts = list(parts) + [parts[0].new_zeros((B, n, _pad4(width) - width))]
    return torch.cat(parts, 2).reshape(B * n, -1)


def idw_weights(dist):
    dev = dist.device
    dist = dist.contiguous()
    w = torch.empty_like(dist)
    with _lib.on_device(dev):
        _lib.call("tp3d_idw_weights_f32", _lib.ptr(dist), dist.numel() // 3, _lib.ptr(w), _lib.stream_ptr(dev))
    return w
```

Baseline: 4248 point-clouds/s.

## Merge BN finalize, wgrad reduce+BN-bwd finalize, and weight packing into single launches

Adds a one-launch BN-stats finalize kernel that folds partial (sum, sumsq, shift, count) chunks per channel with a Chan-style merge. It also adds a combined kernel that does the tn split-reduction and the BN-backward finalize in one grid. A new chain-weights kernel packs padded forward weights and transposed backward weight slices into one buffer in a single launch, replacing the per-layer pad and transpose-contiguous copies. The aim is fewer small kernel launches and fewer graph nodes per MLP chain layer, at the cost of more complex finalize kernels and an extra saved pack tensor. The old two-launch paths stay available behind module flags.

```diff
diff --git a/include/tp3d_hip.h b/include/tp3d_hip.h
--- a/include/tp3d_hip.h
+++ b/include/tp3d_hip.h
@@ -112,6 +112,13 @@
 int tp3d_bn_finalize_f32(float *partial, int chunks, int64_t M, int C, float eps, float momentum, const float *gamma,
                          const float *beta, float *running_mean, float *running_var, int64_t *num_batches_tracked,
                          float *mean, float *invstd, float *scale, float *shift, void *stream);
+int tp3d_bn_finalize_two_launch_f32(float *partial, int chunks, int64_t M, int C, float eps, float momentum,
+                                    const float *gamma, const float *beta, float *running_mean, float *running_var,
+                                    int64_t *num_batches_tracked, float *mean, float *invstd, float *scale, float *shift,
+                                    void *stream);
+
+int tp3d_chain_weights_f32(const void *const *weights, const int64_t *desc, int L, float *workspace,
+                           size_t workspace_floats, void *stream);
 
 int tp3d_gemm_tn_bn_narrow_serves(int64_t M, int N, int K);
 int tp3d_gemm_rows_narrow_chunks(int64_t M);
@@ -137,6 +144,10 @@
                                 const float *beta_k, const float *invstd_k, float slope_k, const float *dA_k, int training,
                                 int64_t M, int N, int K, int terms, float *out, float *workspace, float *red_out,
                                 float *red_workspace, int reverse, void *stream);
+int tp3d_gemm_tn_x3_act_red_two_launch_f32(const float *dY, const float *Yp, const float *mean_k, const float *scale_k,
+                                           const float *beta_k, const float *invstd_k, float slope_k, const float *dA_k,
+                                           int training, int64_t M, int N, int K, int terms, float *out, float *workspace,
+                                           float *red_out, float *red_workspace, int reverse, void *stream);
 
 int tp3d_kpconv_weighted_f32(const float *query, const float *support, const int64_t *neighbors,
                              const float *features, const float *k_points, int64_t Nq, int64_t M, int Mn, int Cin,
diff --git a/torch_points3d_amd/_lib.py b/torch_points3d_amd/_lib.py
--- a/torch_points3d_amd/_lib.py
+++ b/torch_points3d_amd/_lib.py
@@ -35,6 +35,7 @@
     "tp3d_gemm_tn_x3_f32": [_p, _p, _l, _i, _i, _i, _p, _p, _i, _p],
     "tp3d_gemm_tn_x3_act_f32": [_p, _p, _p, _p, _p, _f, _l, _i, _i, _i, _p, _p, _i, _p],
     "tp3d_gemm_tn_x3_act_red_f32": [_p, _p, _p, _p, _p, _p, _f, _p, _i, _l, _i, _i, _i, _p, _p, _p, _p, _i, _p],
+    "tp3d_gemm_tn_x3_act_red_two_launch_f32": [_p, _p, _p, _p, _p, _p, _f, _p, _i, _l, _i, _i, _i, _p, _p, _p, _p, _i, _p],
     "tp3d_gemm_rows_narrow_f32": [_p, _p, _l, _i, _i, _p, _p, _i, _p],
     "tp3d_gemm_tn_bn_narrow_f32": [_p, _p, _p, _p, _p, _p, _p, _f, _p, _l, _i, _i, _p, _p, _i, _p],
     "tp3d_bn_bwd_reduce_f32": [_p, _p, _p, _p, _p, _p, _p, _f, _l, _i, _i, _i, _p, _p, _p, _p, _p, _i, _p],
@@ -44,6 +45,8 @@
     "tp3d_gemm_rows_bnact_x3_f32": [_p, _p, _p, _p, _f, _p, _l, _i, _i, _p, _p, _p, _i, _p],
     "tp3d_gemm_rows_bnbwd_sp_f32": [_p, _p, _p, _p, _p, _p, _p, _f, _p, _l, _i, _i, _p, _i, _i, _i, _p, _p, _i, _i, _p],
     "tp3d_bn_finalize_f32": [_p, _i, _l, _i, _f, _f, _p, _p, _p, _p, _p, _p, _p, _p, _p, _p],
+    "tp3d_bn_finalize_two_launch_f32": [_p, _i, _l, _i, _f, _f, _p, _p, _p, _p, _p, _p, _p, _p, _p, _p],
+    "tp3d_chain_weights_f32": [_p, _p, _i, _p, ctypes.c_size_t, _p],
     "tp3d_kpconv_bwd_features_f32": [_p, _p, _p, _p, _p, _l, _l, _i, _i, _i, _f, _i, _i, _p, _p, ctypes.c_size_t, _i, _p,
                                      ctypes.c_size_t, _p],
     "tp3d_knn_partial_dense_f32": [_p, _p, _p, _p, _i, _i, _l, _l, _i, _f, _p, _p, _p, ctypes.c_size_t, _p],
diff --git a/torch_points3d_amd/csrc/gemm_tn.hip b/torch_points3d_amd/csrc/gemm_tn.hip
--- a/torch_points3d_amd/csrc/gemm_tn.hip
+++ b/torch_points3d_amd/csrc/gemm_tn.hip
@@ -116,24 +116,10 @@
             }
 }
 
-constexpr int RD_E = 64, RD_S = 16;
 __global__ __launch_bounds__(RD_E *RD_S) void gemm_tn_reduce_kernel(const float *__restrict__ partial, int S,
                                                                      int64_t NK, float *__restrict__ out)
 {
-    __shared__ float sm[RD_S][RD_E];
-    const int tx = threadIdx.x % RD_E, ty = threadIdx.x / RD_E;
-    const int64_t e = (int64_t)blockIdx.x * RD_E + tx;
-    float acc = 0.0f;
-    if (e < NK)
-        for (int s = ty; s < S; s += RD_S) acc += partial[(size_t)s * NK + e];
-    sm[ty][tx] = acc;
-    __syncthreads();
-    if (ty == 0 && e < NK) {
-        float t = 0.0f;
-#pragma unroll
-        for (int k = 0; k < RD_S; ++k) t += sm[k][tx];
-        out[e] = t;
-    }
+    tn_reduce_block(partial, S, NK, out, (int)blockIdx.x);
 }
 
 int tn_reduce_splits(const float *partial, int splits, int64_t NK, float *out, hipStream_t s)
diff --git a/torch_points3d_amd/csrc/gemm_tn_x3.hip b/torch_points3d_amd/csrc/gemm_tn_x3.hip
--- a/torch_points3d_amd/csrc/gemm_tn_x3.hip
+++ b/torch_points3d_amd/csrc/gemm_tn_x3.hip
@@ -451,10 +451,10 @@
     return p.tiles_n * p.splits;
 }
 
-TP3D_EXPORT int tp3d_gemm_tn_x3_act_red_f32(const float *dY, const float *Yp, const float *mean_k, const float *scale_k,
-                                            const float *beta_k, const float *invstd_k, float slope_k, const float *dA_k,
-                                            int training, int64_t M, int N, int K, int terms, float *out, float *workspace,
-                                            float *red_out, float *red_workspace, int reverse, void *stream)
+static int x3_act_red_run(const float *dY, const float *Yp, const float *mean_k, const float *scale_k, const float *beta_k,
+                          const float *invstd_k, float slope_k, const float *dA_k, int training, int64_t M, int N, int K,
+                          int terms, float *out, float *workspace, float *red_out, float *red_workspace, int reverse,
+                          void *stream, bool one_launch)
 {
     if (!mean_k || !scale_k || !beta_k || !invstd_k || !dA_k || !red_out || !red_workspace || terms != 6) return TP3D_E_BADARG;
     if (!x3_red_serves(M, N, K) || !dY || !Yp || !out || !workspace) return TP3D_E_BADARG;
@@ -466,7 +466,29 @@
     else if (p.wm == 2) x3_launch<2, 1, false, 32, 6, true>(p, dY, Yp, M, N, K, workspace, pro, s);
     else x3_launch<1, 1, false, 64, 6, true>(p, dY, Yp, M, N, K, workspace, pro, s);
     if (int rc = check_launch()) return rc;
+    if (one_launch)
+        return tn_reduce_bn_bwd_finalize(workspace, p.splits, (int64_t)N * K, out, red_workspace, p.tiles_n * p.splits, K, red_out,
+                                         red_out + K, invstd_k, M, training, red_out + 2 * (size_t)K, red_out + 3 * (size_t)K, s);
     if (int rc = tn_reduce_splits(workspace, p.splits, (int64_t)N * K, out, s)) return rc;
     return bn_bwd_finalize_launch(red_workspace, p.tiles_n * p.splits, K, red_out, red_out + K, invstd_k, M, training,
                                   red_out + 2 * (size_t)K, red_out + 3 * (size_t)K, s);
 }
+
+TP3D_EXPORT int tp3d_gemm_tn_x3_act_red_f32(const float *dY, const float *Yp, const float *mean_k, const float *scale_k,
+                                            const float *beta_k, const float *invstd_k, float slope_k, const float *dA_k,
+                                            int training, int64_t M, int N, int K, int terms, float *out, float *workspace,
+                                            float *red_out, float *red_workspace, int reverse, void *stream)
+{
+    return x3_act_red_run(dY, Yp, mean_k, scale_k, beta_k, invstd_k, slope_k, dA_k, training, M, N, K, terms, out, workspace,
+                          red_out, red_workspace, reverse, stream, true);
+}
+
+TP3D_EXPORT int tp3d_gemm_tn_x3_act_red_two_launch_f32(const float *dY, const float *Yp, const float *mean_k,
+                                                       const float *scale_k, const float *beta_k, const float *invstd_k,
+                                                       float slope_k, const float *dA_k, int training, int64_t M, int N, int K,
+                                                       int terms, float *out, float *workspace, float *red_out,
+                                                       float *red_workspace, int reverse, void *stream)
+{
+    return x3_act_red_run(dY, Yp, mean_k, scale_k, beta_k, invstd_k, slope_k, dA_k, training, M, N, K, terms, out, workspace,
+                          red_out, red_workspace, reverse, stream, false);
+}
diff --git a/torch_points3d_amd/csrc/rows.hip b/torch_points3d_amd/csrc/rows.hip
--- a/torch_points3d_amd/csrc/rows.hip
+++ b/torch_points3d_amd/csrc/rows.hip
@@ -341,13 +341,15 @@
                                              double &q)
 {
     __shared__ double r1[RW_BLOCK], r2[RW_BLOCK];
-    double la = 0.0, lq = 0.0;
-    for (int k = threadIdx.x; k < chunks; k += RW_BLOCK) {
-        la += (double)partial[((size_t)k * 2 + 0) * C + c];
-        lq += (double)partial[((size_t)k * 2 + 1) * C + c];
-    }
-    r1[threadIdx.x] = la;
-    r2[threadIdx.x] = lq;
+    if (threadIdx.x < RW_BLOCK) {
+        double la = 0.0, lq = 0.0;
+        for (int k = threadIdx.x; k < chunks; k += RW_BLOCK) {
+            la += (double)partial[((size_t)k * 2 + 0) * C + c];
+            lq += (double)partial[((size_t)k * 2 + 1) * C + c];
+        }
+        r1[threadIdx.x] = la;
+        r2[threadIdx.x] = lq;
+    }
     __syncthreads();
     for (int off = RW_BLOCK / 2; off > 0; off >>= 1) {
         if ((int)threadIdx.x < off) {
@@ -471,6 +473,111 @@
     invstd_out[c] = invstd;
     scale_out[c] = g * invstd;
     shift_out[c] = beta ? beta[c] : 0.0f;
+}
+
+__device__ __forceinline__ void chan_fold(double &n, double &mu, double &m2, float fS, float fQ, float fK, float fn)
+{
+    const double nb = (double)fn;
+    if (nb > 0.0) {
+        const double S = (double)fS, Q = (double)fQ;
+        const double mb = (double)fK + S / nb, m2b = Q - S * S / nb;
+        const double tot = n + nb, dm = mb - mu;
+        mu += dm * (nb / tot);
+        m2 += m2b + dm * dm * (n * nb / tot);
+        n = tot;
+    }
+}
+__device__ __forceinline__ void chan_merge(double &na_, double &ma, double &m2a, double nb, double mb, double m2b)
+{
+    const double na = na_;
+    const double tot = na + nb;
+    if (nb > 0.0) {
+        const double dm = mb - ma;
+        ma += dm * (nb / tot);
+        m2a += m2b + dm * dm * (na * nb / tot);
+        na_ = tot;
+    }
+}
+
+constexpr int BN_DIRECT_CHUNKS = 64, BN_SLICES = 32;
+static_assert(BN_SLICES * BM_LANES == RW_BLOCK, "one thread per (slice, lane)");
+__global__ __launch_bounds__(RW_BLOCK) void bn_finalize_one_kernel(
+    const float *__restrict__ partial, int chunks, int per, int64_t M, int C, float eps, float momentum,
+    const float *__restrict__ gamma, const float *__restrict__ beta, float *__restrict__ running_mean,
+    float *__restrict__ running_var, int64_t *__restrict__ batches, float *__restrict__ mean_out,
+    float *__restrict__ invstd_out, float *__restrict__ scale_out, float *__restrict__ shift_out)
+{
+    __shared__ double rn[RW_BLOCK][4], rm[RW_BLOCK][4], r2[RW_BLOCK][4];
+    __shared__ double sn[BN_SLICES][4], sm[BN_SLICES][4], s2[BN_SLICES][4];
+    const int tid = threadIdx.x, ry = tid % BM_LANES, sl = tid / BM_LANES;
+    const int c = blockIdx.x * 4;
+    const int k0 = min(sl * per, chunks), k1 = min(k0 + per, chunks);
+    if (batches && blockIdx.x == 0 && tid == 0) *batches += 1;
+    double n[4] = {0.0, 0.0, 0.0, 0.0}, mu[4] = {0.0, 0.0, 0.0, 0.0}, m2[4] = {0.0, 0.0, 0.0, 0.0};
+    for (int k = k0 + ry; k < k1; k += BM_LANES) {
+        const float *pk = partial + (size_t)k * 4 * C + c;
+        const float4 fS = *reinterpret_cast<const float4 *>(pk);
+        const float4 fQ = *reinterpret_cast<const float4 *>(pk + (size_t)C);
+        const float4 fK = *reinterpret_cast<const float4 *>(pk + (size_t)2 * C);
+        const float4 fn = *reinterpret_cast<const float4 *>(pk + (size_t)3 * C);
+        chan_fold(n[0], mu[0], m2[0], fS.x, fQ.x, fK.x, fn.x);
+        chan_fold(n[1], mu[1], m2[1], fS.y, fQ.y, fK.y, fn.y);
+        chan_fold(n[2], mu[2], m2[2], fS.z, fQ.z, fK.z, fn.z);
+        chan_fold(n[3], mu[3], m2[3], fS.w, fQ.w, fK.w, fn.w);
+    }
+#pragma unroll
+    for (int v = 0; v < 4; ++v) {
+        rn[tid][v] = n[v];
+        rm[tid][v] = mu[v];
+        r2[tid][v] = m2[v];
+    }
+    __syncthreads();
+    for (int off = BM_LANES / 2; off > 0; off >>= 1) {
+        if (ry < off) {
+#pragma unroll
+            for (int v = 0; v < 4; ++v) chan_merge(rn[tid][v], rm[tid][v], r2[tid][v], rn[tid + off][v], rm[tid + off][v], r2[tid + off][v]);
+        }
+        __syncthreads();
+    }
+    if (ry == 0) {
+#pragma unroll
+        for (int v = 0; v < 4; ++v) {
+            const double nn = rn[tid][v];
+            const float kf = (float)rm[tid][v];
+            const double sres = nn * (rm[tid][v] - (double)kf);
+            const float fS = (float)sres;
+            const float fQ = (float)(r2[tid][v] + (nn > 0.0 ? sres * sres / nn : 0.0));
+            const float fn = (float)nn;
+            double a = 0.0, b = 0.0, d = 0.0;
+            chan_fold(a, b, d, fS, fQ, kf, fn);
+            sn[sl][v] = a;
+            sm[sl][v] = b;
+            s2[sl][v] = d;
+        }
+    }
+    __syncthreads();
+    for (int off = BN_SLICES / 2; off > 0; off >>= 1) {
+        const int p = tid / 4, v = tid % 4;
+        if (p < off) chan_merge(sn[p][v], sm[p][v], s2[p][v], sn[p + off][v], sm[p + off][v], s2[p + off][v]);
+        __syncthreads();
+    }
+    if (tid >= 4) return;
+    const int cc = c + tid;
+    double vv = s2[0][tid] / (double)M;
+    if (vv < 0.0) vv = 0.0;
+    const float mean = (float)sm[0][tid];
+    const float var = (float)vv;
+    if (running_mean) {
+        const double unb = M > 1 ? vv * ((double)M / (double)(M - 1)) : vv;
+        running_mean[cc] = (1.0f - momentum) * running_mean[cc] + momentum * mean;
+        running_var[cc] = (1.0f - momentum) * running_var[cc] + momentum * (float)unb;
+    }
+    const float invstd = 1.0f / sqrtf(var + eps);
+    const float g = gamma ? gamma[cc] : 1.0f;
+    mean_out[cc] = mean;
+    invstd_out[cc] = invstd;
+    scale_out[cc] = g * invstd;
+    shift_out[cc] = beta ? beta[cc] : 0.0f;
 }
 
 struct ChanWalk {
@@ -597,6 +704,24 @@
     }
 }
 
+__device__ __forceinline__ void bn_bwd_finalize_channel(const float *__restrict__ partial, int chunks, int C, int c,
+                                                        float *__restrict__ dbeta, float *__restrict__ dgamma,
+                                                        const float *__restrict__ invstd, int64_t M, int training,
+                                                        float *__restrict__ c1, float *__restrict__ c2)
+{
+    double a, q;
+    sum_partials(partial, chunks, C, c, a, q);
+    if (threadIdx.x == 0) {
+        dbeta[c] = (float)a;
+        dgamma[c] = (float)q;
+        if (c1) {
+            const float invM = 1.0f / (float)M;
+            c1[c] = training ? (float)a * invM : 0.0f;
+            c2[c] = training ? invstd[c] * ((float)q * invM) : 0.0f;
+        }
+    }
+}
+
 __global__ __launch_bounds__(RW_BLOCK) void bn_bwd_finalize_kernel(const float *__restrict__ partial, int chunks,
                                                                     int C, float *__restrict__ dbeta,
                                                                     float *__restrict__ dgamma,
@@ -604,17 +729,18 @@
                                                                     int training, float *__restrict__ c1,
                                                                     float *__restrict__ c2)
 {
-    double a, q;
-    sum_partials(partial, chunks, C, blockIdx.x, a, q);
-    if (threadIdx.x == 0) {
-        dbeta[blockIdx.x] = (float)a;
-        dgamma[blockIdx.x] = (float)q;
-        if (c1) {
-            const float invM = 1.0f / (float)M;
-            c1[blockIdx.x] = training ? (float)a * invM : 0.0f;
-            c2[blockIdx.x] = training ? invstd[blockIdx.x] * ((float)q * invM) : 0.0f;
-        }
-    }
+    bn_bwd_finalize_channel(partial, chunks, C, blockIdx.x, dbeta, dgamma, invstd, M, training, c1, c2);
+}
+
+__global__ __launch_bounds__(RD_E *RD_S) void tn_reduce_bn_bwd_finalize_kernel(
+    const float *__restrict__ tn_partial, int S, int64_t NK, float *__restrict__ out, int n_reduce,
+    const float *__restrict__ bn_partial, int chunks, int C, float *__restrict__ dbeta, float *__restrict__ dgamma,
+    const float *__restrict__ invstd, int64_t M, int training, float *__restrict__ c1, float *__restrict__ c2)
+{
+    if ((int)blockIdx.x < n_reduce)
+        tn_reduce_block(tn_partial, S, NK, out, (int)blockIdx.x);
+    else
+        bn_bwd_finalize_channel(bn_partial, chunks, C, (int)blockIdx.x - n_reduce, dbeta, dgamma, invstd, M, training, c1, c2);
 }
 
 __device__ __forceinline__ float bn_bwd_elem(float da, float y, float sc, float sh, float mu, float is, float db,
@@ -966,15 +1092,19 @@
     return TP3D_OK;
 }
 
-constexpr int BN_DIRECT_CHUNKS = 64, BN_SLICES = 32;
 static int launch_bn_finalize(float *partial, int chunks, int64_t M, int C, float eps, float momentum, const float *gamma,
                               const float *beta, float *running_mean, float *running_var, int64_t *batches, int training,
-                              float *mean, float *invstd, float *scale, float *shift, hipStream_t s)
+                              float *mean, float *invstd, float *scale, float *shift, hipStream_t s, bool one_launch = false)
 {
     int n = chunks, stride = 1;
     if (training && chunks > BN_DIRECT_CHUNKS) {
         stride = (chunks + BN_SLICES - 1) / BN_SLICES;
         n = (chunks + stride - 1) / stride;
+        if (one_launch && (C & 3) == 0 && (reinterpret_cast<uintptr_t>(partial) & 15) == 0) {
+            hipLaunchKernelGGL(bn_finalize_one_kernel, dim3(C / 4), dim3(RW_BLOCK), 0, s, partial, chunks, stride, M, C, eps,
+                               momentum, gamma, beta, running_mean, running_var, batches, mean, invstd, scale, shift);
+            return check_launch();
+        }
         hipLaunchKernelGGL(bn_merge_slices_kernel, dim3((C + BM_COLS - 1) / BM_COLS, n), dim3(RW_BLOCK), 0, s, partial, chunks,
                            stride, C);
         if (int rc = check_launch()) return rc;
@@ -1021,7 +1151,17 @@
 {
     if (M <= 0 || C <= 0 || chunks <= 0 || !partial || !mean || !invstd || !scale || !shift) return TP3D_E_BADARG;
     return launch_bn_finalize(partial, chunks, M, C, eps, momentum, gamma, beta, running_mean, running_var,
-                              num_batches_tracked, 1, mean, invstd, scale, shift, (hipStream_t)stream);
+                              num_batches_tracked, 1, mean, invstd, scale, shift, (hipStream_t)stream, true);
+}
+
+TP3D_EXPORT int tp3d_bn_finalize_two_launch_f32(float *partial, int chunks, int64_t M, int C, float eps, float momentum,
+                                                const float *gamma, const float *beta, float *running_mean,
+                                                float *running_var, int64_t *num_batches_tracked, float *mean, float *invstd,
+                                                float *scale, float *shift, void *stream)
+{
+    if (M <= 0 || C <= 0 || chunks <= 0 || !partial || !mean || !invstd || !scale || !shift) return TP3D_E_BADARG;
+    return launch_bn_finalize(partial, chunks, M, C, eps, momentum, gamma, beta, running_mean, running_var,
+                              num_batches_tracked, 1, mean, invstd, scale, shift, (hipStream_t)stream, false);
 }
 
 TP3D_EXPORT int tp3d_bn_act_f32(const float *Y, const float *mean, const float *scale, const float *shift, float slope,
@@ -1057,6 +1197,18 @@
 {
     hipLaunchKernelGGL(bn_bwd_finalize_kernel, dim3(C), dim3(RW_BLOCK), 0, s, partial, chunks, C, dbeta, dgamma, invstd, M,
                        training, c1, c2);
+    return check_launch();
+}
+
+static_assert(RD_E * RD_S >= RW_BLOCK, "the finalize workgroups run on the first RW_BLOCK threads of the split sum's");
+int tn_reduce_bn_bwd_finalize(const float *tn_partial, int splits, int64_t NK, float *out, const float *bn_partial, int chunks,
+                              int C, float *dbeta, float *dgamma, const float *invstd, int64_t M, int training, float *c1,
+                              float *c2, hipStream_t s)
+{
+    const int64_t n_reduce = (NK + RD_E - 1) / RD_E;
+    if (n_reduce + C > 0x7fffffff) return TP3D_E_TOOBIG;
+    hipLaunchKernelGGL(tn_reduce_bn_bwd_finalize_kernel, dim3((unsigned)(n_reduce + C)), dim3(RD_E * RD_S), 0, s, tn_partial, splits,
+                       NK, out, (int)n_reduce, bn_partial, chunks, C, dbeta, dgamma, invstd, M, training, c1, c2);
     return check_launch();
 }
 
@@ -1190,3 +1342,70 @@
                        dist, rows, weight);
     return check_launch();
 }
+
+namespace tp3d {
+constexpr int CW_MAX_LAYERS = 8;
+struct ChainWeightJobs {
+    const float *W[CW_MAX_LAYERS];
+    float *W2[CW_MAX_LAYERS], *Wt[CW_MAX_LAYERS];
+    int Cout[CW_MAX_LAYERS], Cin[CW_MAX_LAYERS], Kp[CW_MAX_LAYERS], c0[CW_MAX_LAYERS], ncol[CW_MAX_LAYERS];
+};
+
+__global__ __launch_bounds__(RW_BLOCK) void chain_weights_kernel(ChainWeightJobs jobs)
+{
+    const int l = blockIdx.y >> 1;
+    const float *__restrict__ W = jobs.W[l];
+    const int Cout = jobs.Cout[l], Cin = jobs.Cin[l];
+    const int64_t step = (int64_t)gridDim.x * RW_BLOCK;
+    if ((blockIdx.y & 1) == 0) {
+        float *__restrict__ W2 = jobs.W2[l];
+        if (!W2) return;
+        const int Kp = jobs.Kp[l];
+        const int64_t total = (int64_t)Cout * Kp;
+        for (int64_t e = (int64_t)blockIdx.x * RW_BLOCK + threadIdx.x; e < total; e += step) {
+            const int n = (int)(e / Kp), k = (int)(e - (int64_t)n * Kp);
+            W2[e] = k < Cin ? W[(size_t)n * Cin + k] : 0.0f;
+        }
+    } else {
+        float *__restrict__ Wt = jobs.Wt[l];
+        if (!Wt) return;
+        const int c0 = jobs.c0[l];
+        const int64_t total = (int64_t)jobs.ncol[l] * Cout;
+        for (int64_t e = (int64_t)blockIdx.x * RW_BLOCK + threadIdx.x; e < total; e += step) {
+            const int j = (int)(e / Cout), n = (int)(e - (int64_t)j * Cout);
+            Wt[e] = c0 + j < Cin ? W[(size_t)n * Cin + c0 + j] : 0.0f;
+        }
+    }
+}
+}
+
+TP3D_EXPORT int tp3d_chain_weights_f32(const void *const *weights, const int64_t *desc, int L, float *workspace,
+                                       size_t workspace_floats, void *stream)
+{
+    if (L <= 0 || L > CW_MAX_LAYERS || !weights || !desc || !workspace) return TP3D_E_BADARG;
+    ChainWeightJobs jobs;
+    int64_t most = 0;
+    for (int l = 0; l < L; ++l) {
+        const int64_t *d = desc + 7 * l;
+        const int64_t Cout = d[0], Cin = d[1], Kp = d[2], c0 = d[3], ncol = d[4], o2 = d[5], ot = d[6];
+        if (!weights[l] || Cout <= 0 || Cin <= 0 || Kp < Cin || Kp > (1 << 20) || Cout > (1 << 20)) return TP3D_E_BADARG;
+        if (c0 < 0 || ncol < 0 || c0 + ncol > Kp) return TP3D_E_BADARG;
+        if (o2 >= 0 && (size_t)o2 + (size_t)(Cout * Kp) > workspace_floats) return TP3D_E_BADARG;
+        if (ot >= 0 && (ncol == 0 || (size_t)ot + (size_t)(ncol * Cout) > workspace_floats)) return TP3D_E_BADARG;
+        jobs.W[l] = static_cast<const float *>(weights[l]);
+        jobs.W2[l] = o2 >= 0 ? workspace + o2 : nullptr;
+        jobs.Wt[l] = ot >= 0 ? workspace + ot : nullptr;
+        jobs.Cout[l] = (int)Cout, jobs.Cin[l] = (int)Cin, jobs.Kp[l] = (int)Kp, jobs.c0[l] = (int)c0, jobs.ncol[l] = (int)ncol;
+        if (o2 >= 0 && Cout * Kp > most) most = Cout * Kp;
+        if (ot >= 0 && ncol * Cout > most) most = ncol * Cout;
+    }
+    for (int l = L; l < CW_MAX_LAYERS; ++l) {
+        jobs.W[l] = nullptr, jobs.W2[l] = nullptr, jobs.Wt[l] = nullptr;
+        jobs.Cout[l] = jobs.Cin[l] = jobs.Kp[l] = jobs.c0[l] = jobs.ncol[l] = 0;
+    }
+    if (most == 0) return TP3D_OK;
+    int64_t gx = (most + RW_BLOCK - 1) / RW_BLOCK;
+    if (gx > 256) gx = 256;
+    hipLaunchKernelGGL(chain_weights_kernel, dim3((unsigned)gx, 2 * L), dim3(RW_BLOCK), 0, (hipStream_t)stream, jobs);
+    return check_launch();
+}
diff --git a/torch_points3d_amd/csrc/tp3d_common.h b/torch_points3d_amd/csrc/tp3d_common.h
--- a/torch_points3d_amd/csrc/tp3d_common.h
+++ b/torch_points3d_amd/csrc/tp3d_common.h
@@ -76,6 +76,29 @@
 int bn_bwd_finalize_launch(const float *partial, int chunks, int C, float *dbeta, float *dgamma, const float *invstd, int64_t M,
                            int training, float *c1, float *c2, hipStream_t s);
 int tn_reduce_splits(const float *partial, int splits, int64_t NK, float *out, hipStream_t s);
+int tn_reduce_bn_bwd_finalize(const float *tn_partial, int splits, int64_t NK, float *out, const float *bn_partial, int chunks,
+                              int C, float *dbeta, float *dgamma, const float *invstd, int64_t M, int training, float *c1,
+                              float *c2, hipStream_t s);
+
+constexpr int RD_E = 64, RD_S = 16;
+__device__ __forceinline__ void tn_reduce_block(const float *__restrict__ partial, int S, int64_t NK, float *__restrict__ out,
+                                                int block)
+{
+    __shared__ float sm[RD_S][RD_E];
+    const int tx = threadIdx.x % RD_E, ty = threadIdx.x / RD_E;
+    const int64_t e = (int64_t)block * RD_E + tx;
+    float acc = 0.0f;
+    if (e < NK)
+        for (int s = ty; s < S; s += RD_S) acc += partial[(size_t)s * NK + e];
+    sm[ty][tx] = acc;
+    __syncthreads();
+    if (ty == 0 && e < NK) {
+        float t = 0.0f;
+#pragma unroll
+        for (int k = 0; k < RD_S; ++k) t += sm[k][tx];
+        out[e] = t;
+    }
+}
 
 int grid_ball_query(const float *x, const float *y, const int64_t *seg, const int64_t *batch_y, int num_clouds,
                     int64_t rows, int N, int np, int64_t total_q, int Lmax, float radius, int nsample, int sort,
diff --git a/torch_points3d_amd/fused.py b/torch_points3d_amd/fused.py
--- a/torch_points3d_amd/fused.py
+++ b/torch_points3d_amd/fused.py
@@ -1,4 +1,5 @@
 import collections
+import ctypes
 
 import torch
 import torch.nn as nn
@@ -85,7 +86,7 @@
     ws = _lib.gemm_tn_workspace(M, N, K, dev, x3=True)
     rws = _lib.workspace("gemm_tn_red", 4 * 2 * b.wgrad_chunks * K, dev)
     with _lib.on_device(dev):
-        _lib.call("tp3d_gemm_tn_x3_act_red_f32", _lib.ptr(dY), _lib.ptr(Ys[l - 1]), _lib.ptr(ps[0]), _lib.ptr(ps[2]), _lib.ptr(ps[3]),
+        _lib.call("tp3d_gemm_tn_x3_act_red_f32" if b.red_one_launch else "tp3d_gemm_tn_x3_act_red_two_launch_f32", _lib.ptr(dY), _lib.ptr(Ys[l - 1]), _lib.ptr(ps[0]), _lib.ptr(ps[2]), _lib.ptr(ps[3]),
                   _lib.ptr(ps[1]), float(slopes[l - 1]), _lib.ptr(dA_prev), int(training), M, N, K, 6, _lib.ptr(out), _lib.ptr(ws),
                   _lib.ptr(red), _lib.ptr(rws), int(b.wgrad_rev), _lib.stream_ptr(dev))
     return out, red
@@ -174,11 +175,13 @@
     return C, part
 
 
-def _finalize_stats(part, M, C, gamma, beta, bn, dev, st, chunks=None):
+def _finalize_stats(part, M, C, gamma, beta, bn, dev, st, chunks=None, one_launch=None):
     stats = torch.empty((4, C), dtype=torch.float32, device=dev)
     if chunks is None:
         chunks = _lib.load().tp3d_gemm_rows_stat_chunks(M, C)
-    _lib.call("tp3d_bn_finalize_f32", _lib.ptr(part), chunks, M, C, float(bn.eps),
+    if one_launch is None:
+        one_launch = bool(BN_FINALIZE_ONE_LAUNCH)
+    _lib.call("tp3d_bn_finalize_f32" if one_launch else "tp3d_bn_finalize_two_launch_f32", _lib.ptr(part), chunks, M, C, float(bn.eps),
               float(bn.momentum), _lib.ptr(gamma), _lib.ptr(beta), _lib.ptr(bn.running_mean), _lib.ptr(bn.running_var),
               _lib.ptr(bn.num_batches_tracked), _lib.ptr(stats[0]), _lib.ptr(stats[1]), _lib.ptr(stats[2]), _lib.ptr(stats[3]), st)
     _note_training_pass(bn)
@@ -361,16 +364,19 @@
         need = ctx.needs_input_grad
         first = len(need) - len(params)
         plan = _plan_chain(M, K0, [params[3 * l].shape[0] for l in range(L)], pool_ns, grad_enabled and any(need), need[0],
-                           need[first::3], grad_cols)
+                           need[first::3], grad_cols, params[0][0].numel())
         Ys, stats, W2s, cins, acts = [], [], [], [], [None] * (L - 1)
         with _lib.on_device(dev):
+            pack = _chain_weights(plan, K0, [params[3 * l] for l in range(L)], dev, st)
             for l, ((bn, slope), p) in enumerate(zip(layers, plan)):
                 weight, gamma, beta = params[3 * l], params[3 * l + 1], params[3 * l + 2]
                 Cout = weight.shape[0]
                 W2 = weight.reshape(Cout, -1)
                 Kp = K0 if l == 0 else Ys[-1].shape[1]
                 cins.append(W2.shape[1])
-                if W2.shape[1] != Kp:
+                if pack is not None and p.wpack[0] >= 0:
+                    W2 = pack[p.wpack[0]:p.wpack[0] + Cout * Kp].view(Cout, Kp)
+                elif W2.shape[1] != Kp:
                     W2 = torch.nn.functional.pad(W2, (0, Kp - W2.shape[1]))
                 W2 = W2.contiguous()
                 Y = torch.empty((M, Cout), dtype=torch.float32, device=dev)
@@ -398,13 +404,13 @@
                               _lib.ptr(mean), _lib.ptr(scale), _lib.ptr(shift), pslope, _lib.ptr(W2), M, Cout, Kp, _lib.ptr(Y),
                               _lib.ptr(part), _lib.ptr(acts[l - 1]) if l else None, p.reverse, st)
                 if training:
-                    stats.append(_finalize_stats(part, M, Cout, gamma, beta, bn, dev, st, p.chunks))
+                    stats.append(_finalize_stats(part, M, Cout, gamma, beta, bn, dev, st, p.chunks, p.one_finalize))
                 else:
                     stats.append(_bn_stats(Y, M, Cout, gamma, beta, bn, False, dev, st))
                 Ys.append(Y)
                 W2s.append(W2)
             out, arg = _bn_act_out(Ys[-1], stats[-1], layers[-1][1], pool_ns, st)
-        ctx.save_for_backward(A0, arg, *Ys, *stats, *W2s, *(acts if plan[0].bwd else []))
+        ctx.save_for_backward(A0, arg, *Ys, *stats, *W2s, *(acts if plan[0].bwd else []), *([pack] if pack is not None else []))
         ctx.cfg = (L, pool_ns, training, [s_ for _, s_ in layers], [tuple(params[3 * l].shape) for l in range(L)], cins)
         ctx.plan = plan
         return out
@@ -423,6 +429,7 @@
         if not ctx.plan[0].bwd:
             raise RuntimeError("_MLPChain.backward: the forward pass ran without a gradient request (grad mode off at the call site)")
         acts = saved[2 + 3 * L:2 + 3 * L + (L - 1)]
+        pack = saved[2 + 3 * L + (L - 1)] if ctx.plan[0].wpack is not None else None
         red_next = None
         with _lib.on_device(dev):
             for l in range(L - 1, -1, -1):
@@ -452,7 +459,11 @@
                 dprev = torch.empty((M, Kp), dtype=torch.float32, device=dev)
                 c0, ncol = b.cols if b.cols else (0, Kp)
                 pad_hi = Kp - c0 - ncol
-                Wt = W2.t()[c0:c0 + ncol].contiguous()
+                if pack is not None:
+                    ot = ctx.plan[l].wpack[1]
+                    Wt = pack[ot:ot + ncol * C].view(ncol, C)
+                else:
+                    Wt = W2.t()[c0:c0 + ncol].contiguous()
                 pad_lo_k, pad_hi_k = c0, pad_hi
                 if c0 > 32 or pad_hi > 32:
                     dprev.zero_()
@@ -467,6 +478,24 @@
         return (dcur if ctx.plan[0].bwd.dx else None, None, None, None, None) + tuple(grads)
 
 
+def _chain_weights(plan, K0, weights, dev, st):
+    if plan[0].wpack is None:
+        return None
+    L = len(plan)
+    total = plan[0].wpack[2]
+    pack = torch.empty(total, dtype=torch.float32, device=dev)
+    ws = [w if w.is_contiguous() else w.contiguous() for w in weights]
+    desc = []
+    for l, (p, w) in enumerate(zip(plan, ws)):
+        Cout = w.shape[0]
+        Kp = K0 if l == 0 else weights[l - 1].shape[0]
+        c0, ncol = (p.bwd.cols if (p.bwd is not None and p.bwd.cols) else (0, Kp))
+        desc += [Cout, w[0].numel(), Kp, c0, ncol, p.wpack[0], p.wpack[1]]
+    _lib.call("tp3d_chain_weights_f32", (ctypes.c_void_p * L)(*[w.data_ptr() for w in ws]), (ctypes.c_int64 * len(desc))(*desc),
+              L, _lib.ptr(pack), total, st)
+    return pack
+
+
 def _chain_ok(rows, parts):
     if not USE_MLP_CHAIN or rows.shape[0] < CHAIN_MIN_ROWS or rows.shape[1] % 4:
         return False
@@ -485,11 +514,15 @@
 FWD_NARROW = True
 WGRAD_RED = True
 
-_ChainLayer = collections.namedtuple("_ChainLayer", "kernel chunks reverse keep_act bwd")
-_ChainLayerBwd = collections.namedtuple("_ChainLayerBwd", "kind cols reduce_rev dx dx_rev write_dY wgrad wgrad_rev wgrad_chunks terms")
-
-
-def _plan_chain(M, K0, widths, pool_ns, want_grad, need_in, need_w, grad_cols):
+BN_FINALIZE_ONE_LAUNCH = True
+WGRAD_RED_ONE_LAUNCH = True
+CHAIN_WEIGHTS_ONE_LAUNCH = True
+
+_ChainLayer = collections.namedtuple("_ChainLayer", "kernel chunks reverse keep_act bwd one_finalize wpack")
+_ChainLayerBwd = collections.namedtuple("_ChainLayerBwd", "kind cols reduce_rev dx dx_rev write_dY wgrad wgrad_rev wgrad_chunks terms red_one_launch")
+
+
+def _plan_chain(M, K0, widths, pool_ns, want_grad, need_in, need_w, grad_cols, cin0=None):
     h = _lib.load()
     L = len(widths)
     Ks = [K0] + list(widths[:-1])
@@ -513,8 +546,10 @@
         directed = kernel not in ("rows", "bn_act_rows")
         prev = int(directed and alt and not prev)
         fwd.append((kernel, chunks, prev if directed else None, keep[l]))
+    one_fin, red_one = bool(BN_FINALIZE_ONE_LAUNCH), bool(WGRAD_RED_ONE_LAUNCH)
     if not want_grad:
-        return tuple(_ChainLayer(*f, bwd=None) for f in fwd)
+        wpack = _plan_chain_weights(widths, Ks, cin0, None)
+        return tuple(_ChainLayer(*f, bwd=None, one_finalize=one_fin, wpack=w) for f, w in zip(fwd, wpack))
 
     kinds, cols = [], []
     for l in range(L):
@@ -540,14 +575,14 @@
         if kinds[l] == "passes":
             wgrad = plain if need_w[l] else None
             bwd[l] = _ChainLayerBwd("passes", cols[l], None, l > 0 or need_in, None, True, wgrad, 0 if wgrad in ("x3", "x3_act") else None,
-                                    0, WGRAD_X3)
+                                    0, WGRAD_X3, red_one)
             continue
         reduce_rev = None
         if not red_above:
             reduce_rev, turn = rev[turn % 2], turn + 1
         red_above = False
         if kinds[l] == "narrow":
-            bwd[l] = _ChainLayerBwd("narrow", cols[l], reduce_rev, False, None, False, "narrow", rev[turn % 2], 0, WGRAD_X3)
+            bwd[l] = _ChainLayerBwd("narrow", cols[l], reduce_rev, False, None, False, "narrow", rev[turn % 2], 0, WGRAD_X3, red_one)
             turn += 1
             continue
         dx_rev, turn = rev[turn % 2], turn + 1
@@ -559,8 +594,25 @@
             turn += 1
         if need_w[l] and not chunks:
             wgrad, wgrad_rev, turn = plain, (rev[turn % 2] if plain != "tn" else None), turn + 1
-        bwd[l] = _ChainLayerBwd("loader", cols[l], reduce_rev, True, dx_rev, need_w[l], wgrad, wgrad_rev, chunks, WGRAD_X3)
-    return tuple(_ChainLayer(*f, bwd=b) for f, b in zip(fwd, bwd))
+        bwd[l] = _ChainLayerBwd("loader", cols[l], reduce_rev, True, dx_rev, need_w[l], wgrad, wgrad_rev, chunks, WGRAD_X3, red_one)
+    wpack = _plan_chain_weights(widths, Ks, cin0, bwd)
+    return tuple(_ChainLayer(*f, bwd=b, one_finalize=one_fin, wpack=w) for f, b, w in zip(fwd, bwd, wpack))
+
+
+def _plan_chain_weights(widths, Ks, cin0, bwd):
+    L = len(widths)
+    offs, total = [], 0
+    for l in range(L):
+        o2 = ot = -1
+        if l == 0 and cin0 is not None and cin0 != Ks[0]:
+            o2, total = total, total + _pad4(widths[0] * Ks[0])
+        if bwd is not None and bwd[l].kind == "loader":
+            ncol = bwd[l].cols[1] if bwd[l].cols else Ks[l]
+            ot, total = total, total + _pad4(ncol * widths[l])
+        offs.append((o2, ot))
+    if not CHAIN_WEIGHTS_ONE_LAUNCH or total == 0 or L > 8:
+        return [None] * L
+    return [(o2, ot, total) for o2, ot in offs]
 
 
 class _BNAct(torch.autograd.Function):
```

Measured after the change: 4252 point-clouds/s (median of 2 runs). Within noise of the previous version (+0.1%).
